# rlog58/dags-vae-search

Measured on AMD Instinct MI355X. Metric: DAGs/sec VAE+predictor train step, n=12 batch 4096 per GPU, at 1 MI355X, higher is better.
Workload: dtype f32 (fwd bf16x6, bwd bf16x3 split products, fp32 accumulate); 1 GPU; synthetic_v12 DAGs (n=12, card=12, N=15 tokens), PACE-VAE train step: pack + fwd + bwd + clip_grad_norm_(1.0) + Adam(1e-4), train mode dropout 0.15; per_gpu_batch=4096, global_batch=4096, waves_per_workgroup=8, parallelism=single

## Files before the change

### dags_vae_search_amd/_lib.py

```python
from __future__ import annotations

import ctypes
import os
from ctypes import (POINTER, Structure, c_char, c_char_p, c_float, c_int, c_int32, c_int64, c_size_t, c_uint32,
                    c_uint64, c_void_p)

_HERE = os.path.dirname(os.path.abspath(__file__))
LIB_NAME = "libdvs_hip.so"

D_MODEL, HEADS, LAYERS, LATENT, FC_HIDDEN, EMB = 64, 8, 3, 32, 32, 32
MAX_TOKENS = 48
TILE_TOKENS = 16
DECODE_STATE_BYTES = 440
CLIP_SCRATCH_FLOATS = 4096
RECORD_BYTES = 96
LOSS_FLOATS = 5
ABI_VERSION = 202
GP_ACQ_MAX_INDUCING = 1023
STRUCT_HASH_INVALID = 0x7FFFFFFFFFFFFFFF
GEN_LABELS_CHOICE, GEN_ACCEPT_ISOLATES, GEN_ACCEPT_NO_CONNECTIVITY, GEN_GROUP_SHIFT = 1, 2, 4, 8
SCORE_TYPES = {"loglik": 0, "aic": 1, "bic": 2, "bde": 3, "bds": 4, "k2": 5, "bdj": 6}


class DvsShape(Structure):
    _fields_ = [("batch", c_int32), ("n_tokens", c_int32), ("n_classes", c_int32), ("training", c_int32),
                ("dropout", c_float), ("beta", c_float), ("eps_scale", c_float), ("dag_offset", c_uint32),
                ("seed", c_uint64)]


class DvsParamEntry(Structure):
    _fields_ = [("name", c_char * 64), ("offset", c_int64), ("rows", c_int32), ("cols", c_int32)]


def bind(lib: ctypes.CDLL) -> ctypes.CDLL:
    P = POINTER
    lib.dvs_version.restype = c_int
    lib.dvs_last_error.restype = c_char_p
    lib.dvs_device_cus.restype = c_int
    lib.dvs_param_count.restype = c_int64
    lib.dvs_param_count.argtypes = [P(DvsShape)]
    lib.dvs_param_table.restype = c_int
    lib.dvs_param_table.argtypes = [P(DvsShape), P(DvsParamEntry), c_int]
    lib.dvs_workspace_bytes.restype = c_size_t
    lib.dvs_workspace_bytes.argtypes = [P(DvsShape)]
    lib.dvs_record_bytes.restype = c_size_t
    lib.dvs_record_bytes.argtypes = [P(DvsShape)]
    lib.dvs_pack_features.restype = c_int
    lib.dvs_pack_features.argtypes = [P(DvsShape), c_void_p, c_void_p, c_void_p, c_void_p, c_void_p, c_size_t, c_void_p,
                                      c_void_p]
    lib.dvs_build_records.restype = c_int
    lib.dvs_build_records.argtypes = [P(DvsShape), c_void_p, c_void_p, c_void_p, c_size_t, c_void_p, c_void_p]
    lib.dvs_loss_forward.restype = c_int
    lib.dvs_loss_forward.argtypes = [P(DvsShape), c_void_p, c_size_t, c_void_p, c_int64, c_void_p, c_size_t, c_void_p,
                                     c_void_p, c_void_p, c_void_p, c_void_p, c_void_p]
    lib.dvs_loss_forward_notify.restype = c_int
    lib.dvs_loss_forward_notify.argtypes = [P(DvsShape), c_void_p, c_size_t, c_void_p, c_int64, c_void_p, c_size_t, c_void_p,
                                            c_void_p, c_void_p, c_void_p, c_void_p, c_void_p, ctypes.c_uint32, c_void_p]
    lib.dvs_loss_backward.restype = c_int
    lib.dvs_loss_backward.argtypes = [P(DvsShape), c_void_p, c_size_t, c_void_p, c_int64, c_void_p, c_size_t, c_void_p,
                                      c_void_p, c_void_p]
    lib.dvs_loss_backward_sq.restype = c_int
    lib.dvs_loss_backward_sq.argtypes = [P(DvsShape), c_void_p, c_size_t, c_void_p, c_int64, c_void_p, c_size_t, c_void_p,
                                         c_void_p, c_void_p, c_void_p]
    lib.dvs_encode.restype = c_int
    lib.dvs_encode.argtypes = [P(DvsShape), c_void_p, c_size_t, c_void_p, c_int64, c_void_p, c_size_t, c_void_p, c_void_p,
                               c_void_p]
    lib.dvs_decode.restype = c_int
    lib.dvs_decode.argtypes = [P(DvsShape), c_void_p, c_int64, c_void_p, c_size_t, c_void_p, c_size_t, c_void_p, c_void_p,
                               c_void_p, c_size_t, c_void_p]
    lib.dvs_match_decoded.restype = c_int
    lib.dvs_match_decoded.argtypes = [c_int32, c_int32, c_int32, c_int32, c_int32, c_void_p, c_void_p, c_void_p, c_size_t,
                                      c_int32, c_void_p, c_void_p]
    lib.dvs_decoded_structures.restype = c_int
    lib.dvs_decoded_structures.argtypes = [c_int32, c_int32, c_int32, c_void_p, c_size_t, c_uint64, c_void_p, c_void_p,
                                           c_void_p, c_void_p, c_size_t, c_void_p, c_void_p]
    lib.dvs_structset_filter.restype = c_int
    lib.dvs_structset_filter.argtypes = [c_int32, c_int32, c_void_p, c_void_p, c_void_p, c_size_t, c_void_p, c_int32,
                                         c_void_p, c_void_p, c_size_t, c_void_p, c_void_p]
    lib.dvs_generate_dags.restype = c_int
    lib.dvs_generate_dags.argtypes = [c_int32, c_int32, c_int32, c_int32, c_void_p, c_uint64, c_int64, c_int32, c_int32,
                                      c_void_p, c_void_p, c_size_t, c_void_p, c_void_p]
    lib.dvs_generate_edge_counts.restype = c_int
    lib.dvs_generate_edge_counts.argtypes = [c_int32, c_int32, c_void_p, c_void_p, c_uint64, c_int64, c_void_p, c_void_p]
    lib.dvs_debug_launch.restype = c_int
    lib.dvs_debug_launch.argtypes = [c_size_t, c_void_p]
    lib.dvs_bic_scores.restype = c_int
    lib.dvs_bic_scores.argtypes = [c_int32, c_int32, c_int32, c_void_p, c_void_p, c_void_p, c_void_p, c_void_p, c_void_p,
                                   c_void_p]
    lib.dvs_bn_scores.restype = c_int
    lib.dvs_bn_scores.argtypes = [c_int32, c_int32, c_int32, c_void_p, c_void_p, c_void_p, c_int32, ctypes.c_double, c_void_p,
                                  c_void_p, c_void_p, c_void_p]
    lib.dvs_bic_parent_masks.restype = c_int
    lib.dvs_bic_parent_masks.argtypes = [c_int32, c_int32, c_int32, c_void_p, c_void_p, c_void_p, c_void_p, c_void_p]
    lib.dvs_gp_predict.restype = c_int
    lib.dvs_gp_predict.argtypes = [c_int32, c_int32, c_int32, c_void_p, c_void_p, c_void_p, ctypes.c_double, ctypes.c_double,
                                   ctypes.c_double, c_void_p, c_void_p]
    lib.dvs_gp_kernel.restype = c_int
    lib.dvs_gp_kernel.argtypes = [c_int32, c_int32, c_int32, c_void_p, c_void_p, ctypes.c_double, ctypes.c_double, c_void_p,
                                  c_void_p]
    lib.dvs_gp_kernel_backward.restype = c_int
    lib.dvs_gp_kernel_backward.argtypes = [c_int32, c_int32, c_int32, c_int32, c_void_p, c_void_p, ctypes.c_double,
                                           ctypes.c_double, c_void_p, c_void_p, c_void_p, c_void_p]
    lib.dvs_gp_acquire.restype = c_int
    lib.dvs_gp_acquire.argtypes = [c_int32, c_int32, c_int32, c_int32, c_void_p, c_void_p, c_void_p] + [ctypes.c_double] * 6 + \
        [c_void_p, c_void_p, c_void_p, c_void_p, c_void_p]
    lib.dvs_clip_adam.restype = c_int
    lib.dvs_clip_adam.argtypes = [c_int64, c_void_p, c_void_p, c_void_p, c_void_p, c_float, c_float, c_float, c_float,
                                  c_int64, c_float, c_void_p, c_void_p, c_void_p]
    lib.dvs_clip_adam_from_partials.restype = c_int
    lib.dvs_clip_adam_from_partials.argtypes = lib.dvs_clip_adam.argtypes
    lib.dvs_profile_enable.restype = None
    lib.dvs_profile_enable.argtypes = [c_int]
    lib.dvs_profile_collect.restype = c_int
    lib.dvs_profile_collect.argtypes = [c_void_p, c_int, c_void_p, c_void_p, c_int]
    lib.dvs_debug_activation.restype = c_int
    lib.dvs_debug_activation.argtypes = [P(DvsShape), c_void_p, c_int, c_void_p, c_void_p]
    return lib


EXPORTS = ["dvs_version", "dvs_last_error", "dvs_device_cus", "dvs_param_count", "dvs_param_table",
           "dvs_workspace_bytes", "dvs_record_bytes", "dvs_pack_features", "dvs_build_records", "dvs_loss_forward", "dvs_loss_forward_notify", "dvs_loss_backward", "dvs_loss_backward_sq", "dvs_encode", "dvs_decode", "dvs_match_decoded", "dvs_decoded_structures", "dvs_structset_filter", "dvs_generate_dags", "dvs_generate_edge_counts", "dvs_bic_scores", "dvs_bn_scores", "dvs_bic_parent_masks", "dvs_gp_predict", "dvs_gp_kernel", "dvs_gp_kernel_backward", "dvs_gp_acquire",
           "dvs_clip_adam", "dvs_clip_adam_from_partials", "dvs_debug_activation", "dvs_debug_launch", "dvs_profile_enable", "dvs_profile_collect"]


def profile_collect(lib):
    cap, stride = 64, 64
    names = ctypes.create_string_buffer(cap * stride)
    counts = (c_int * cap)()
    ms = (c_float * cap)()
    n = lib.dvs_profile_collect(names, stride, counts, ms, cap)
    out = {}
    for i in range(min(n, cap)):
        out[names.raw[i * stride:(i + 1) * stride].split(b"\0")[0].decode()] = (int(counts[i]), float(ms[i]))
    return out

_lib = None


def lib_path() -> str:
    return os.path.join(_HERE, LIB_NAME)


def load() -> ctypes.CDLL:
    global _lib
    if _lib is None:
        path = lib_path()
        if not os.path.exists(path):
            raise RuntimeError(
                f"{LIB_NAME} not found at {path}: build it with `python -c 'import __graft_entry__ as g; g.build()'` "
                f"(hipcc --offload-arch=gfx950).  dags_vae_search_amd has no CPU fallback.")
        _lib = bind(ctypes.CDLL(path))
        if _lib.dvs_version() != ABI_VERSION:
            raise RuntimeError(f"{LIB_NAME}: unexpected ABI version {_lib.dvs_version()}")
    return _lib


def check(lib, code: int, what: str):
    if code != 0:
        msg = lib.dvs_last_error()
        raise RuntimeError(f"{what} failed with code {code}: {msg.decode() if msg else ''}")


def make_shape(batch: int, n_tokens: int, n_classes: int, training: bool = False, dropout: float = 0.15,
               beta: float = 0.005, eps_scale: float = 0.01, dag_offset: int = 0, seed: int = 0) -> DvsShape:
    return DvsShape(int(batch), int(n_tokens), int(n_classes), 1 if training else 0, float(dropout), float(beta),
                    float(eps_scale), int(dag_offset) & 0xFFFFFFFF, int(seed) & 0xFFFFFFFFFFFFFFFF)


def record_bytes(lib, shape: DvsShape) -> int:
    n = int(lib.dvs_record_bytes(ctypes.byref(shape)))
    if n == 0:
        check(lib, 1, "dvs_record_bytes")
    return n


def is_wide(n_tokens: int, n_classes: int) -> bool:
    return n_tokens > TILE_TOKENS or n_classes > 16


def param_table(lib, shape: DvsShape):
    entries = (DvsParamEntry * 128)()
    n = lib.dvs_param_table(ctypes.byref(shape), entries, 128)
    if n <= 0:
        check(lib, 1, "dvs_param_table")
    table = []
    for e in entries[:n]:
        shp = (e.rows, e.cols) if e.cols else (e.rows,)
        table.append((e.name.decode(), int(e.offset), shp))
    total = int(lib.dvs_param_count(ctypes.byref(shape)))
    return table, total
```

### dags_vae_search_amd/csrc/dvs_api.hip

```cpp
#include <math.h>
#include <stdarg.h>
#include <stdio.h>
#include <stdlib.h>
#include <string.h>

#include "dvs_kernels.h"
#include "dvs_backward.h"
#include "dvs_wide.h"
#include "dvs_wimg.h"
#include "dvs_decode.h"

static thread_local char g_err[256] = "";

#include <map>
#include <mutex>
#include <string>
#include <utility>
#include <vector>
namespace {
struct ProfRec {
    const char* name;
#ifndef DVS_EMU
    hipEvent_t a, b;
#endif
};
std::mutex g_prof_mu;
bool g_prof_on = false;
std::vector<ProfRec> g_prof;
thread_local int t_prof_slot = -1;
}

void dvs_prof_begin(const char* name, dvs_stream_t st) {
    t_prof_slot = -1;
    std::lock_guard<std::mutex> lock(g_prof_mu);
    if (!g_prof_on) return;
    ProfRec r;
    r.name = name;
#ifndef DVS_EMU
    if (hipEventCreate(&r.a) != hipSuccess) return;
    if (hipEventCreate(&r.b) != hipSuccess) {
        (void)hipEventDestroy(r.a);
        return;
    }
    (void)hipEventRecord(r.a, st);
#endif
    t_prof_slot = (int)g_prof.size();
    g_prof.push_back(r);
}
void dvs_prof_end(dvs_stream_t st) {
    if (t_prof_slot < 0) return;
    std::lock_guard<std::mutex> lock(g_prof_mu);
#ifndef DVS_EMU
    if (t_prof_slot < (int)g_prof.size()) (void)hipEventRecord(g_prof[t_prof_slot].b, st);
#endif
    t_prof_slot = -1;
}
extern "C" void dvs_profile_enable(int on) {
    std::lock_guard<std::mutex> lock(g_prof_mu);
    g_prof_on = on != 0;
}
extern "C" int dvs_profile_collect(char* names, int name_stride, int* counts, float* total_ms, int cap) {
    std::map<std::string, std::pair<int, float>> agg;
    std::lock_guard<std::mutex> lock(g_prof_mu);
    for (auto& r : g_prof) {
        float ms = 0.f;
#ifndef DVS_EMU
        (void)hipEventSynchronize(r.b);
        (void)hipEventElapsedTime(&ms, r.a, r.b);
        (void)hipEventDestroy(r.a);
        (void)hipEventDestroy(r.b);
#endif
        auto& e = agg[r.name];
        e.first += 1;
        e.second += ms;
    }
    g_prof.clear();
    int i = 0;
    for (auto& kv : agg) {
        if (i >= cap) break;
        snprintf(names + (size_t)i * name_stride, name_stride, "%s", kv.first.c_str());
        counts[i] = kv.second.first;
        total_ms[i] = kv.second.second;
        ++i;
    }
    return (int)agg.size();
}

static int fail(int code, const char* msg) {
    snprintf(g_err, sizeof(g_err), "%s", msg);
    return code;
}

static thread_local int t_hip_err = 0;
static thread_local char t_hip_msg[200] = "";
void dvs_note_hip_error(const char* what, int hip_error, const char* hip_message) {
    if (t_hip_err != 0) return;
    t_hip_err = hip_error ? hip_error : -1;
    snprintf(t_hip_msg, sizeof(t_hip_msg), "%s: HIP error %d (%s)", what, hip_error, hip_message ? hip_message : "?");
}
static void call_begin() {
    t_hip_err = 0;
    (void)hipGetLastError();
}
static int call_end(const char* fn) {
    if (t_hip_err == 0) return 0;
    snprintf(g_err, sizeof(g_err), "%s: %s", fn, t_hip_msg);
    t_hip_err = 0;
    return 20;
}
#define DVS_HIP_CALL(expr)                                                             \
    do {                                                                               \
        const hipError_t dvs_ce_ = (expr);                                             \
        if (dvs_ce_ != hipSuccess) dvs_note_hip_error(#expr, (int)dvs_ce_, hipGetErrorString(dvs_ce_)); \
    } while (0)
static void copy_out(void* dst, const void* src, size_t bytes, dvs_stream_t st) {
#ifdef DVS_EMU
    DVS_HIP_CALL(hipMemcpyAsyncD2D(dst, src, bytes, st));
#else
    DVS_HIP_CALL(hipMemcpyAsync(dst, src, bytes, hipMemcpyDeviceToDevice, st));
#endif
}

extern "C" int dvs_version(void) { return DVS_VERSION; }
extern "C" const char* dvs_last_error(void) { return g_err; }

extern "C" int dvs_device_cus(void) {
#ifdef DVS_EMU
    return 2;
#else
    int dev = 0, cus = 0;
    if (hipGetDevice(&dev) != hipSuccess) return 0;
    if (hipDeviceGetAttribute(&cus, hipDeviceAttributeMultiprocessorCount, dev) != hipSuccess) return 0;
    return cus;
#endif
}

namespace {
struct LayoutBuilder {
    int64_t off = 0;
    dvs_param_entry* table;
    int cap, count = 0;
    int64_t add(int rows, int cols, const char* fmt, ...) {
        const int64_t o = off;
        if (table && count < cap) {
            dvs_param_entry& e = table[count];
            memset(&e, 0, sizeof(e));
            va_list ap;
            va_start(ap, fmt);
            vsnprintf(e.name, sizeof(e.name), fmt, ap);
            va_end(ap);
            e.offset = o;
            e.rows = rows;
            e.cols = cols;
        }
        ++count;
        const int64_t n = (int64_t)rows * (cols ? cols : 1);
        off += (n + 3) & ~(int64_t)3;
        return o;
    }
};
}

DvsLayout dvs_make_layout(int N, int C, dvs_param_entry* table, int cap, int* count) {
    LayoutBuilder b;
    b.table = table;
    b.cap = cap;
    DvsLayout l;
    auto attn = [&](const char* stack, int i, const char* which, DvsAttnP& p) {
        p.in_w = b.add(192, 64, "%s.layers.%d.%s.in_proj_weight", stack, i, which);
        p.in_b = b.add(192, 0, "%s.layers.%d.%s.in_proj_bias", stack, i, which);
        p.out_w = b.add(64, 64, "%s.layers.%d.%s.out_proj.weight", stack, i, which);
        p.out_b = b.add(64, 0, "%s.layers.%d.%s.out_proj.bias", stack, i, which);
    };
    auto ffn = [&](const char* stack, int i, DvsFfnP& p) {
        p.l1_w = b.add(64, 64, "%s.layers.%d.linear1.weight", stack, i);
        p.l1_b = b.add(64, 0, "%s.layers.%d.linear1.bias", stack, i);
        p.l2_w = b.add(64, 64, "%s.layers.%d.linear2.weight", stack, i);
        p.l2_b = b.add(64, 0, "%s.layers.%d.linear2.bias", stack, i);
    };
    auto norm = [&](const char* stack, int i, int k, DvsNormP& p) {
        p.w = b.add(64, 0, "%s.layers.%d.norm%d.weight", stack, i, k);
        p.b = b.add(64, 0, "%s.layers.%d.norm%d.bias", stack, i, k);
    };
    l.W1 = b.add(2 * N, 64, "vertex_position_embed.W1");
    l.W2 = b.add(64, 32, "vertex_position_embed.W2");
    l.lab_w = b.add(32, C, "vertex_label_embed.0.weight");
    l.lab_b = b.add(32, 0, "vertex_label_embed.0.bias");
    for (int i = 0; i < DVS_LAYERS; ++i) {
        attn("encoder", i, "self_attn", l.enc[i].sa);
        ffn("encoder", i, l.enc[i].ff);
        norm("encoder", i, 1, l.enc[i].n1);
        norm("encoder", i, 2, l.enc[i].n2);
    }
    l.fc1_w = b.add(32, N * 64, "fc1.weight");
    l.fc1_b = b.add(32, 0, "fc1.bias");
    l.fc2_w = b.add(32, N * 64, "fc2.weight");
    l.fc2_b = b.add(32, 0, "fc2.bias");
    for (int i = 0; i < DVS_LAYERS; ++i) {
        attn("decoder", i, "self_attn", l.dec[i].sa);
        attn("decoder", i, "multihead_attn", l.dec[i].ca);
        ffn("decoder", i, l.dec[i].ff);
        norm("decoder", i, 1, l.dec[i].n1);
        norm("decoder", i, 2, l.dec[i].n2);
        norm("decoder", i, 3, l.dec[i].n3);
    }
    l.node0_w = b.add(32, 64, "add_node.0.weight");
    l.node0_b = b.add(32, 0, "add_node.0.bias");
    l.node2_w = b.add(C, 32, "add_node.2.weight");
    l.node2_b = b.add(C, 0, "add_node.2.bias");
    l.edge0_w = b.add(64, 128, "add_edge.0.weight");
    l.edge0_b = b.add(64, 0, "add_edge.0.bias");
    l.edge2_w = b.add(1, 64, "add_edge.2.weight");
    l.edge2_b = b.add(1, 0, "add_edge.2.bias");
    l.fc3_w = b.add(N * 64, 32, "fc3.weight");
    l.fc3_b = b.add(N * 64, 0, "fc3.bias");
    l.total = b.off;
    if (count) *count = b.count;
    return l;
}

DvsWorkspace dvs_make_workspace(int B, int NT, int64_t P, int nslab, bool wide) {
    DvsWorkspace w;
    size_t off = 0;
    auto take = [&](size_t n) {
        const size_t o = off;
        off += (n + 63) & ~(size_t)63;
        return o;
    };
    const size_t tile = (size_t)B * NT * 1024;
    for (int s = 0; s < DVS_NSLOTS; ++s) {
        w.act[s] = take(tile);
        w.stats[s] = take((size_t)B * NT * 32);
    }
    w.enc_out = take(tile);
    w.mu = take((size_t)B * 32);
    w.logvar = take((size_t)B * 32);
    w.z = take((size_t)B * 32);
    w.epsv = take((size_t)B * 32);
    w.mem = take(tile);
    w.dag_loss = take((size_t)B * 2);
    w.gA = take(tile);
    w.gB = take(tile);
    w.gq = take(tile);
    w.gk = take(tile);
    w.gv = take(tile);
    w.gmem = take(tile);
    w.genc = take(tile);
    w.gz = take((size_t)B * 64);
    w.nslab = nslab;
    w.slabs = take((size_t)nslab * (size_t)P);
    w.fcpart = take((size_t)DVS_FC_PARTS * (size_t)P);
    w.wimg = take((DVS_WIMG_BF16 + 1) / 2);
    w.limg = take(DvsLatImg::floats(NT));
    for (int blk = 0; blk < 9; ++blk) w.qkv[blk] = take(wide ? (size_t)B * NT * 12 * 256 : 0);
    w.total_floats = off;
    return w;
}

static int check_shape(const dvs_shape* s) {
    if (!s) return fail(1, "dvs: null shape");
    if (s->batch <= 0) return fail(2, "dvs: batch must be > 0");
    if (s->n_tokens < 4 || s->n_tokens > DVS_WTOK)
        return fail(3, "dvs: n_tokens (= max_num_vertices + 3) must be in [4, 48] in this build");
    if (s->n_classes < 4 || s->n_classes > DVS_WTOK)
        return fail(4, "dvs: n_classes (= vertex_label_cardinality + 3) must be in [4, 48] in this build");
    if (!(s->dropout >= 0.f && s->dropout < 1.f)) return fail(5, "dvs: dropout must be in [0, 1)");
    return 0;
}

static bool is_wide(const dvs_shape* s) { return s->n_tokens > DVS_MAXTOK || s->n_classes > 16; }
static int tiles_of(const dvs_shape* s) { return (s->n_tokens + 15) / 16; }
static size_t record_size(bool wide) { return wide ? sizeof(DvsRecordW) : sizeof(DvsRecord); }

static DvsDims make_dims(const dvs_shape* s) {
    DvsDims d;
    d.NT = tiles_of(s);
    d.B = s->batch;
    d.N = s->n_tokens;
    d.C = s->n_classes;
    d.training = s->training ? 1 : 0;
    d.drop.thr16 = (uint32_t)lrintf(s->dropout * 65536.0f);
    d.drop.on = (d.training && d.drop.thr16 > 0) ? 1 : 0;
    d.drop.scale = 1.0f / (1.0f - (float)d.drop.thr16 / 65536.0f);
    d.seed_lo = (uint32_t)(s->seed & 0xFFFFFFFFull);
    d.seed_hi = (uint32_t)(s->seed >> 32);
    d.dag_offset = s->dag_offset;
    d.beta = s->beta;
    d.eps_scale = s->eps_scale;
    d.debug = 0;
    return d;
}

static int num_slabs() {
    const int cus = dvs_device_cus();
    return cus > 0 ? cus : 256;
}
static int grid_for(int units, int per_wg, int cap) {
    const int want = (units + per_wg - 1) / per_wg;
    return want < cap ? want : cap;
}

static int waves_per_wg(const DvsDims& d, bool wide, int nslab) {
    const char* env = getenv("DVS_WAVES_PER_WG");
    const int force = env ? atoi(env) : 0;
    if (wide) return 8;
    if (force == 4 || force == 8) return force;
    return d.B <= 4 * nslab ? 4 : 8;
}
static int active_slabs(const DvsDims& d, bool wide, int nslab) {
    if (wide) return nslab;
    const int want = (d.B + 3) / 4;
    return want < nslab ? want : nslab;
}

static bool env_on(const char* name) {
    const char* v = getenv(name);
    return v && atoi(v) != 0;
}
static bool split_stack() {
    static const bool on = env_on("DVS_SPLIT_STACK");
    return on;
}
static bool latent_kernels_off() {
    static const bool on = env_on("DVS_LATENT_KERNELS");
    return on;
}
static bool latent_in_chain(bool chain, int nw) { return chain && !latent_kernels_off() && nw == 8; }

struct FwdGrids {
    int chain;
    int tiles16;
    int tiles8;
    int tiles4;
    int dags;
    int dags2;
    int dec4;
};

struct Step {
    DvsDims d;
    DvsLayout L;
    DvsWorkspace W;
    bool wide;
    const float* P;
    float* ws;
    const DvsRecord* rec;
    dvs_stream_t st;
    int nw;
    FwdGrids g;
    int slabs;
};
static Step make_step(const dvs_shape* s, const void* records, const float* params, void* workspace, void* stream) {
    Step c;
    c.d = make_dims(s);
    c.L = dvs_make_layout(c.d.N, c.d.C, nullptr, 0, nullptr);
    c.wide = is_wide(s);
    const int nslab = num_slabs();
    c.W = dvs_make_workspace(c.d.B, c.d.NT, c.L.total, nslab, c.wide);
    c.P = params;
    c.ws = (float*)workspace;
    c.rec = (const DvsRecord*)records;
    c.st = (dvs_stream_t)stream;
    c.nw = waves_per_wg(c.d, c.wide, nslab);
    const int tiles = c.d.B * c.d.NT;
    c.g.chain = grid_for(tiles, c.nw, nslab);
    c.g.tiles16 = grid_for(tiles, 16, nslab);
    c.g.tiles8 = grid_for(tiles, 8, nslab);
    c.g.tiles4 = grid_for(tiles, 4, nslab);
    c.g.dags = grid_for(c.d.B, 1, nslab);
    c.g.dags2 = c.d.B < 2 * c.g.dags ? c.d.B : 2 * c.g.dags;
    c.g.dec4 = grid_for(c.d.B, 4, nslab);
    c.slabs = active_slabs(c.d, c.wide, nslab);
    return c;
}

static int check_records(const char* fn, size_t records_bytes, int batch, bool wide) {
    const size_t need = (size_t)batch * record_size(wide);
    if (records_bytes >= need) return 0;
    char msg[240];
    snprintf(msg, sizeof(msg), "%s: records_bytes %zu < batch * dvs_record_bytes = %zu", fn, records_bytes, need);
    return fail(14, msg);
}
static int check_buffers(const Step& c, const char* fn, size_t records_bytes, int64_t n_params, size_t workspace_bytes) {
    if (int e = check_records(fn, records_bytes, c.d.B, c.wide)) return e;
    char msg[240];
    if (n_params < c.L.total) {
        snprintf(msg, sizeof(msg), "%s: n_params %lld < dvs_param_count = %lld", fn, (long long)n_params, (long long)c.L.total);
        return fail(14, msg);
    }
    const size_t need = c.W.total_floats * sizeof(float);
    if (workspace_bytes < need) {
        snprintf(msg, sizeof(msg), "%s: workspace_bytes %zu < dvs_workspace_bytes = %zu", fn, workspace_bytes, need);
        return fail(14, msg);
    }
    return 0;
}

extern "C" int64_t dvs_param_count(const dvs_shape* s) {
    if (check_shape(s)) return -1;
    return dvs_make_layout(s->n_tokens, s->n_classes, nullptr, 0, nullptr).total;
}

extern "C" int dvs_param_table(const dvs_shape* s, dvs_param_entry* out, int cap) {
    if (check_shape(s)) return -1;
    int count = 0;
    dvs_make_layout(s->n_tokens, s->n_classes, out, cap, &count);
    return count;
}

extern "C" size_t dvs_workspace_bytes(const dvs_shape* s) {
    if (check_shape(s)) return 0;
    return make_step(s, nullptr, nullptr, nullptr, nullptr).W.total_floats * sizeof(float);
}

extern "C" size_t dvs_record_bytes(const dvs_shape* s) {
    if (check_shape(s)) return 0;
    return record_size(is_wide(s));
}

extern "C" int dvs_pack_features(const dvs_shape* s, const float* label_onehot, const float* pos_onehot,
                                 const float* adjacency, const uint8_t* target_masks, void* records, size_t records_bytes,
                                 int32_t* status, void* stream) {
    if (int e = check_shape(s)) return e;
    if (!label_onehot || !pos_onehot || !adjacency || !target_masks || !records || !status)
        return fail(10, "dvs_pack_features: null pointer");
    if (int e = check_records("dvs_pack_features", records_bytes, s->batch, is_wide(s))) return e;
    call_begin();
    PackArgs a;
    a.B = s->batch;
    a.N = s->n_tokens;
    a.C = s->n_classes;
    a.lab1h = label_onehot;
    a.pos1h = pos_onehot;
    a.adj = adjacency;
    a.tmask = target_masks;
    a.rec = (DvsRecord*)records;
    a.status = status;
    if (is_wide(s)) dvs_launch_pack_w(a, (dvs_stream_t)stream);
    else dvs_launch_pack(a, (dvs_stream_t)stream);
    return call_end("dvs_pack_features");
}

extern "C" int dvs_build_records(const dvs_shape* s, const uint8_t* labels, const void* preds, void* records,
                                 size_t records_bytes, int32_t* status, void* stream) {
    if (int e = check_shape(s)) return e;
    if (!labels || !preds || !records || !status) return fail(10, "dvs_build_records: null pointer");
    if (int e = check_records("dvs_build_records", records_bytes, s->batch, is_wide(s))) return e;
    call_begin();
    if (is_wide(s)) {
        BuildWArgs a;
        a.B = s->batch;
        a.N = s->n_tokens;
        a.C = s->n_classes;
        a.labels = labels;
        a.preds = (const uint64_t*)preds;
        a.rec = (DvsRecordW*)records;
        a.status = status;
        dvs_launch_build_records_w(a, (dvs_stream_t)stream);
        return call_end("dvs_build_records");
    }
    BuildArgs a;
    a.B = s->batch;
    a.N = s->n_tokens;
    a.C = s->n_classes;
    a.labels = labels;
    a.preds = (const uint16_t*)preds;
    a.rec = (DvsRecord*)records;
    a.status = status;
    dvs_launch_build_records(a, (dvs_stream_t)stream);
    return call_end("dvs_build_records");
}

static inline int slot_enc(int layer, int sub) { return 1 + 2 * layer + sub; }
static inline int slot_dec(int layer, int sub) { return 8 + 3 * layer + sub; }
static inline int site_enc(int layer, int k) { return 4 + 4 * layer + k; }
static inline int site_dec(int layer, int k) { return 16 + 6 * layer + k; }

static inline size_t img_attn(int block) { return (size_t)block * DvsAttnImg::SIZE; }
static inline size_t img_ffn(int block) { return DVS_N_ATTN_BLOCKS * DvsAttnImg::SIZE + (size_t)block * DvsFfnImg::SIZE; }
static inline int blk_enc_attn(int layer) { return layer; }
static inline int blk_dec_self(int layer) { return 3 + 2 * layer; }
static inline int blk_dec_cross(int layer) { return 4 + 2 * layer; }
static inline int blk_enc_ffn(int layer) { return layer; }
static inline int blk_dec_ffn(int layer) { return 3 + layer; }

static inline const void* wimg_attn(const Step& c, int block) { return (const dvs_bf16*)(c.ws + c.W.wimg) + img_attn(block); }
static inline const void* wimg_ffn(const Step& c, int block) { return (const dvs_bf16*)(c.ws + c.W.wimg) + img_ffn(block); }

static DvsLN ln_of(const Step& c, int slot, const DvsNormP* n) {
    if (!n) return DvsLN{nullptr, nullptr, nullptr};
    return DvsLN{c.ws + c.W.stats[slot], c.P + n->w, c.P + n->b};
}

static EmbedArgs embed_args(const Step& c, int site) {
    EmbedArgs e;
    memset(&e, 0, sizeof(e));
    e.dims = c.d;
    e.rec = c.rec;
    e.W1 = c.P + c.L.W1;
    e.W2 = c.P + c.L.W2;
    e.lab_w = c.P + c.L.lab_w;
    e.lab_b = c.P + c.L.lab_b;
    e.embimg = (const float*)((const dvs_bf16*)(c.ws + c.W.wimg) + DVS_WIMG_EMB);
    e.site = site;
    return e;
}

static AttnArgs attn_args(const Step& c, const DvsAttnP& p, int block, int in, const DvsNormP* norm, const float* kv, int out,
                          int site0) {
    AttnArgs a;
    memset(&a, 0, sizeof(a));
    a.dims = c.d;
    a.rec = c.rec;
    a.xin = c.ws + c.W.act[in];
    a.ln = ln_of(c, in, norm);
    a.kv = kv;
    a.in_w = c.P + p.in_w;
    a.in_b = c.P + p.in_b;
    a.out_w = c.P + p.out_w;
    a.out_b = c.P + p.out_b;
    a.wimg = wimg_attn(c, block);
    a.qkv = c.wide ? c.ws + c.W.qkv[block] : nullptr;
    a.out_pre = c.ws + c.W.act[out];
    a.out_stats = c.ws + c.W.stats[out];
    a.site_prob = site0;
    a.site_post = site0 + 1;
    return a;
}

static FfnArgs ffn_args(const Step& c, const DvsFfnP& p, int block, int in, const DvsNormP& norm, int out, int site0) {
    FfnArgs f;
    memset(&f, 0, sizeof(f));
    f.dims = c.d;
    f.xin = c.ws + c.W.act[in];
    f.ln = ln_of(c, in, &norm);
    f.l1_w = c.P + p.l1_w;
    f.l1_b = c.P + p.l1_b;
    f.l2_w = c.P + p.l2_w;
    f.l2_b = c.P + p.l2_b;
    f.wimg = wimg_ffn(c, block);
    f.out_pre = c.ws + c.W.act[out];
    f.out_stats = c.ws + c.W.stats[out];
    f.site_hidden = site0;
    f.site_post = site0 + 1;
    return f;
}

static LatentArgs latent_args(const Step& c, const float* eps, bool with_mem) {
    LatentArgs a;
    memset(&a, 0, sizeof(a));
    a.dims = c.d;
    a.xenc = c.ws + c.W.enc_out;
    a.fc1_w = c.P + c.L.fc1_w;
    a.fc1_b = c.P + c.L.fc1_b;
    a.fc2_w = c.P + c.L.fc2_w;
    a.fc2_b = c.P + c.L.fc2_b;
    a.fc3_w = c.P + c.L.fc3_w;
    a.fc3_b = c.P + c.L.fc3_b;
    a.limg = c.ws + c.W.limg;
    a.eps_in = eps;
    a.mu = c.ws + c.W.mu;
    a.logvar = c.ws + c.W.logvar;
    a.z = c.ws + c.W.z;
    a.epsv = c.ws + c.W.epsv;
    a.mem = with_mem ? c.ws + c.W.mem : nullptr;
    a.dag_loss = c.ws + c.W.dag_loss;
    return a;
}

template <class A>
static void head_params(const Step& c, A& a) {
    a.node0_w = c.P + c.L.node0_w;
    a.node0_b = c.P + c.L.node0_b;
    a.node2_w = c.P + c.L.node2_w;
    a.node2_b = c.P + c.L.node2_b;
    a.edge0_b = c.P + c.L.edge0_b;
    a.edge2_w = c.P + c.L.edge2_w;
    a.edge2_b = c.P + c.L.edge2_b;
}
template <class A>
static void head_input(const Step& c, A& a) {
    const int last = slot_dec(DVS_LAYERS - 1, 2);
    a.xin = c.ws + c.W.act[last];
    a.ln = ln_of(c, last, &c.L.dec[DVS_LAYERS - 1].n3);
    a.edge0_w = c.P + c.L.edge0_w;
    head_params(c, a);
}

static LossArgs loss_args(const Step& c) {
    LossArgs a;
    memset(&a, 0, sizeof(a));
    a.dims = c.d;
    a.rec = c.rec;
    head_input(c, a);
    a.wimg = (const dvs_bf16*)(c.ws + c.W.wimg) + DVS_WIMG_LOSS;
    a.dag_loss = c.ws + c.W.dag_loss;
    return a;
}

static void prepare_images(const Step& c) {
    const DvsLayout& L = c.L;
    const bool wide = c.wide;
    DvsImgJobs J;
    J.count = 0;
    auto add = [&](int64_t src, size_t dst, int rows, int flags) {
        DvsImgJob& j = J.job[J.count++];
        j.src = src;
        j.dst = (int64_t)dst;
        j.rows = rows;
        j.flags = flags;
    };
    auto attn = [&](const DvsAttnP& p, int block) {
        const size_t b = img_attn(block);
        add(p.in_w, b + DvsAttnImg::Win, 192, wide ? 0 : 2);
        add(p.out_w, b + DvsAttnImg::Wout, 64, wide ? 0 : 4);
        add(p.out_w, b + DvsAttnImg::WoutT, 64, 1 | (wide ? 0 : 4));
        add(p.in_w, b + DvsAttnImg::WinB, 192, 16 | (wide ? 0 : 2));
        for (int q = 0; q < 3; ++q)
            add(p.in_w + 4096 * q, b + DvsAttnImg::WinT + (size_t)q * 2 * DVS_IMG64, 64, 1 | (wide ? 0 : 2));
    };
    auto ffn = [&](const DvsFfnP& p, int block) {
        const size_t b = img_ffn(block);
        add(p.l1_w, b + DvsFfnImg::W1, 64, 0);
        add(p.l2_w, b + DvsFfnImg::W2, 64, 0);
        add(p.l2_w, b + DvsFfnImg::W2T, 64, 1);
        add(p.l1_w, b + DvsFfnImg::W1T, 64, 1);
    };
    for (int i = 0; i < DVS_LAYERS; ++i) {
        attn(L.enc[i].sa, blk_enc_attn(i));
        ffn(L.enc[i].ff, blk_enc_ffn(i));
        attn(L.dec[i].sa, blk_dec_self(i));
        attn(L.dec[i].ca, blk_dec_cross(i));
        ffn(L.dec[i].ff, blk_dec_ffn(i));
    }
    if (!wide) {
        add(L.edge0_w, DVS_WIMG_LOSS + DvsLossImg::Wa, 64, 8);
        add(L.edge0_w + 64, DVS_WIMG_LOSS + DvsLossImg::Wb, 64, 8);
        add(L.edge0_w, DVS_WIMG_LOSS + DvsLossImg::WaT, 64, 8 | 1);
        add(L.edge0_w + 64, DVS_WIMG_LOSS + DvsLossImg::WbT, 64, 8 | 1);
    }
    dvs_bf16* wimg = (dvs_bf16*)(c.ws + c.W.wimg);
    DvsLatImgArgs lat;
    lat.fc1_w = c.P + L.fc1_w;
    lat.fc2_w = c.P + L.fc2_w;
    lat.fc3_w = c.P + L.fc3_w;
    lat.fc3_b = c.P + L.fc3_b;
    lat.img = c.ws + c.W.limg;
    lat.N = c.d.N;
    lat.NT = c.d.NT;
    DvsLossHeadArgs head;
    memset(&head, 0, sizeof(head));
    if (!wide) {
        head_params(c, head);
        head.ln_g = c.P + L.dec[DVS_LAYERS - 1].n3.w;
        head.ln_b = c.P + L.dec[DVS_LAYERS - 1].n3.b;
        head.dst = (float*)(wimg + DVS_WIMG_LOSS + DvsLossImg::Head);
        head.C = c.d.C;
        head.W1 = c.P + L.W1;
        head.W2 = c.P + L.W2;
        head.lab_w = c.P + L.lab_w;
        head.lab_b = c.P + L.lab_b;
        head.dst_emb = (float*)(wimg + DVS_WIMG_EMB);
        head.N = c.d.N;
    }
    dvs_launch_prepare_images(J, c.P, wimg, lat, head, c.st);
}

static void launch_embed_fwd(const Step& c, const EmbedArgs& e) {
    if (c.wide) dvs_launch_embed_fwd_w(e, c.g.tiles4, c.st);
    else if (c.nw == 4) dvs_launch_embed_fwd(e, c.g.chain, 4, c.st);
    else dvs_launch_embed_fwd(e, c.g.tiles16, 16, c.st);
}
static void launch_attn_fwd(const Step& c, const AttnArgs& a) {
    if (c.wide) dvs_launch_attn_fwd_w(a, c.g.dags, c.st);
    else if (c.nw == 4) dvs_launch_attn_fwd(a, c.g.chain, 4, c.st);
    else dvs_launch_attn_fwd(a, c.g.tiles8, 8, c.st);
}
static void launch_ffn_fwd(const Step& c, const FfnArgs& f) {
    if (c.nw == 4) dvs_launch_ffn_fwd(f, c.g.chain, 4, c.st);
    else dvs_launch_ffn_fwd(f, c.g.tiles16, 16, c.st);
}
static void launch_loss_fwd(const Step& c, const LossArgs& a) {
    if (c.wide) dvs_launch_loss_fwd_w(a, c.g.dags2, c.st);
    else if (c.nw == 4) dvs_launch_loss_fwd(a, c.g.chain, 4, c.st);
    else dvs_launch_loss_fwd(a, c.g.tiles8, 8, c.st);
}
struct FwdChain {
    FwdStackArgs stack;
    const Step& c;
    int tag;
    bool chain;
    FwdChain(const Step& step, int tag_) : c(step), tag(tag_), chain(!step.wide && !split_stack()) { memset(&stack, 0, sizeof(stack)); }
    FwdPhase& next(int kind) {
        if (stack.nphase == DVS_FWD_STACK_PHASES) flush();
        FwdPhase& ph = stack.ph[stack.nphase++];
        ph.kind = kind;
        return ph;
    }
    void attn(const AttnArgs& a) {
        if (chain) next(DVS_FPH_ATTN).u.a = a;
        else launch_attn_fwd(c, a);
    }
    void ffn(const FfnArgs& f) {
        if (chain) next(DVS_FPH_FFN).u.f = f;
        else launch_ffn_fwd(c, f);
    }
    bool latent(const LatentArgs& l) {
        if (!latent_in_chain(chain, c.nw) || stack.nphase == 0 || stack.nphase == DVS_FWD_STACK_PHASES) return false;
        next(DVS_FPH_LATENT).u.l = l;
        return true;
    }
    void flush() {
        if (stack.nphase > 0) dvs_launch_fwd_stack(stack, tag, c.g.chain, c.nw, c.st);
        stack.nphase = 0;
    }
};

static void encoder_forward(const Step& c, const LatentArgs& lat, bool dec_embed = false, bool save_qkv = false) {
    EmbedArgs e = embed_args(c, 0);
    e.out = c.ws + c.W.act[0];
    if (dec_embed) {
        e.out2 = c.ws + c.W.act[7];
        e.site2 = 2;
    }
    launch_embed_fwd(c, e);
    FwdChain chain(c, 0);
    const DvsNormP* norm = nullptr;
    int prev = 0;
    for (int i = 0; i < DVS_LAYERS; ++i) {
        const auto& pl = c.L.enc[i];
        const int sa = slot_enc(i, 0), sf = slot_enc(i, 1);
        AttnArgs a = attn_args(c, pl.sa, blk_enc_attn(i), prev, norm, nullptr, sa, site_enc(i, 0));
        if (!save_qkv) a.qkv = nullptr;
        chain.attn(a);
        FfnArgs f = ffn_args(c, pl.ff, blk_enc_ffn(i), sa, pl.n1, sf, site_enc(i, 2));
        if (i == DVS_LAYERS - 1) {
            f.out_norm = c.ws + c.W.enc_out;
            f.ng = c.P + pl.n2.w;
            f.nb = c.P + pl.n2.b;
        }
        chain.ffn(f);
        norm = &pl.n2;
        prev = sf;
    }
    const bool fused = chain.latent(lat);
    chain.flush();
    if (!fused) dvs_launch_latent_fwd(lat, c.st);
}

static void decoder_forward(const Step& c, int dec_in) {
    FwdChain chain(c, 1);
    const DvsNormP* norm = nullptr;
    int prev = dec_in;
    for (int i = 0; i < DVS_LAYERS; ++i) {
        const auto& pl = c.L.dec[i];
        const int s0 = slot_dec(i, 0), s1 = slot_dec(i, 1), s2 = slot_dec(i, 2);
        chain.attn(attn_args(c, pl.sa, blk_dec_self(i), prev, norm, nullptr, s0, site_dec(i, 0)));
        chain.attn(attn_args(c, pl.ca, blk_dec_cross(i), s0, &pl.n1, c.ws + c.W.mem, s1, site_dec(i, 2)));
        chain.ffn(ffn_args(c, pl.ff, blk_dec_ffn(i), s1, pl.n2, s2, site_dec(i, 4)));
        norm = &pl.n3;
        prev = s2;
    }
    chain.flush();
}

extern "C" int dvs_loss_forward(const dvs_shape* s, const void* records, size_t records_bytes, const float* params,
                                int64_t n_params, void* workspace, size_t workspace_bytes, const float* eps,
                                const int32_t* status, float* losses, float* mu, float* logvar, void* stream) {
    return dvs_loss_forward_notify(s, records, records_bytes, params, n_params, workspace, workspace_bytes, eps,
                                   (int32_t*)status, losses, mu, logvar, nullptr, 0u, stream);
}

extern "C" int dvs_loss_forward_notify(const dvs_shape* s, const void* records, size_t records_bytes, const float* params,
                                       int64_t n_params, void* workspace, size_t workspace_bytes, const float* eps,
                                       int32_t* status, float* losses, float* mu, float* logvar, void* host_tail,
                                       uint32_t host_seq, void* stream) {
    if (int e = check_shape(s)) return e;
    if (!records || !params || !workspace || !losses) return fail(10, "dvs_loss_forward: null pointer");
    const Step c = make_step(s, records, params, workspace, stream);
    if (int e = check_buffers(c, "dvs_loss_forward", records_bytes, n_params, workspace_bytes)) return e;
    call_begin();
    prepare_images(c);
    encoder_forward(c, latent_args(c, eps, true), c.d.drop.on, true);
    decoder_forward(c, c.d.drop.on ? 7 : 0);
    launch_loss_fwd(c, loss_args(c));
    FinalizeArgs fa;
    fa.B = c.d.B;
    fa.beta = c.d.beta;
    fa.dag_loss = c.ws + c.W.dag_loss;
    fa.status = status;
    fa.losses = losses;
    fa.host_tail = (float*)host_tail;
    fa.host_seq = host_seq;
    dvs_launch_finalize(fa, c.st);
    const size_t nb = (size_t)c.d.B * 32 * sizeof(float);
    if (mu) copy_out(mu, c.ws + c.W.mu, nb, c.st);
    if (logvar) copy_out(logvar, c.ws + c.W.logvar, nb, c.st);
    return call_end("dvs_loss_forward");
}

extern "C" int dvs_encode(const dvs_shape* s, const void* records, size_t records_bytes, const float* params,
                          int64_t n_params, void* workspace, size_t workspace_bytes, float* mu, float* logvar,
                          void* stream) {
    if (int e = check_shape(s)) return e;
    if (!records || !params || !workspace || !mu || !logvar) return fail(10, "dvs_encode: null pointer");
    const Step c = make_step(s, records, params, workspace, stream);
    if (int e = check_buffers(c, "dvs_encode", records_bytes, n_params, workspace_bytes)) return e;
    call_begin();
    prepare_images(c);
    LatentArgs la = latent_args(c, nullptr, false);
    la.dims.training = 0;
    encoder_forward(c, la);
    const size_t nb = (size_t)c.d.B * 32 * sizeof(float);
    copy_out(mu, c.ws + c.W.mu, nb, c.st);
    copy_out(logvar, c.ws + c.W.logvar, nb, c.st);
    return call_end("dvs_encode");
}

extern "C" int dvs_decode(const dvs_shape* s, const float* params, int64_t n_params, void* workspace,
                          size_t workspace_bytes, void* records, size_t records_bytes, const float* z,
                          const float* uniforms, void* state_out, size_t state_bytes, void* stream) {
    if (int e = check_shape(s)) return e;
    if (!params || !workspace || !records || !z || !state_out) return fail(10, "dvs_decode: null pointer");
    if (s->training) return fail(13, "dvs_decode: generation runs in eval mode (shape.training must be 0)");
    const Step c = make_step(s, records, params, workspace, stream);
    if (int e = check_buffers(c, "dvs_decode", records_bytes, n_params, workspace_bytes)) return e;
    if (state_bytes < (size_t)s->batch * sizeof(dvs_decode_state))
        return fail(14, "dvs_decode: state_bytes < batch * sizeof(dvs_decode_state)");
    call_begin();
    prepare_images(c);
    dvs_launch_decode_memory(c.d, z, c.P + c.L.fc3_w, c.P + c.L.fc3_b, c.ws + c.W.mem, c.st);
    DecodeArgs a;
    memset(&a, 0, sizeof(a));
    a.dims = c.d;
    a.wide = c.wide ? 1 : 0;
    a.rec = records;
    a.state = (DvsDecodeState*)state_out;
    head_input(c, a);
    a.uniforms = uniforms;
    dvs_launch_decode_init(a, c.st);
    EmbedArgs e = embed_args(c, 2);
    e.out = c.ws + c.W.act[7];
    for (int idx = 2; idx < c.d.N; ++idx) {
        launch_embed_fwd(c, e);
        decoder_forward(c, 7);
        a.idx = idx;
        dvs_launch_decode_step(a, c.g.dec4, c.st);
    }
    return call_end("dvs_decode");
}

extern "C" int dvs_match_decoded_impl(int B, int n, int card, int R, int wide, const uint8_t* labels, const void* preds,
                                      const void* states, int budget, uint8_t* flags, void* stream);
extern "C" int dvs_match_decoded(int32_t batch, int32_t n_vars, int32_t card, int32_t repeats, int32_t preds_are_u64,
                                 const uint8_t* labels, const void* preds, const void* states, size_t state_bytes,
                                 int32_t budget, uint8_t* flags, void* stream) {
    if (batch <= 0 || repeats <= 0) return fail(2, "dvs_match_decoded: batch and repeats must be > 0");
    if ((int64_t)batch * repeats > (int64_t)1 << 30) return fail(2, "dvs_match_decoded: batch * repeats must be <= 2^30");
    if (n_vars < 1 || n_vars > 45) return fail(3, "dvs_match_decoded: n_vars must be in [1, 45]");
    if (card < 1 || card > 45) return fail(3, "dvs_match_decoded: card must be in [1, 45]");
    if (!preds_are_u64 && n_vars > 16) return fail(12, "dvs_match_decoded: 16-bit predecessor rows hold at most 16 vertices");
    if (budget < 1) return fail(12, "dvs_match_decoded: budget must be >= 1");
    if (!labels || !preds || !states || !flags) return fail(10, "dvs_match_decoded: null pointer");
    const size_t need = (size_t)batch * repeats * sizeof(dvs_decode_state);
    if (state_bytes < need) {
        char msg[160];
        snprintf(msg, sizeof(msg), "dvs_match_decoded: state_bytes < batch * repeats * DVS_DECODE_STATE_BYTES = %zu", need);
        return fail(14, msg);
    }
    call_begin();
    if (int e = dvs_match_decoded_impl(batch, n_vars, card, repeats, preds_are_u64 ? 1 : 0, labels, preds, states, budget,
                                       flags, stream))
        return e;
    return call_end("dvs_match_decoded");
}

extern "C" int dvs_decoded_structures_impl(int B, int n, int wide, const void* states, uint64_t hash_mask, uint8_t* flags,
                                           uint8_t* labels, void* preds, uint64_t* keys, uint64_t* hashes, void* stream);
extern "C" int dvs_structset_filter_impl(int B, int n, const uint64_t* sorted_hashes, const int64_t* order,
                                         const uint64_t* keys, const uint8_t* flags, int S, const uint64_t* seen_hashes,
                                         const uint64_t* seen_keys, uint8_t* out, void* stream);
static int fail_size(const char* what, size_t need) {
    char msg[200];
    snprintf(msg, sizeof(msg), "%s = %zu", what, need);
    return fail(14, msg);
}
extern "C" int dvs_decoded_structures(int32_t batch, int32_t n_vars, int32_t preds_are_u64, const void* states,
                                      size_t state_bytes, uint64_t hash_mask, uint8_t* flags, uint8_t* labels, void* preds,
                                      uint64_t* keys, size_t keys_bytes, uint64_t* hashes, void* stream) {
    if (batch <= 0) return fail(2, "dvs_decoded_structures: batch must be > 0");
    if (batch > 1 << 30) return fail(2, "dvs_decoded_structures: batch must be <= 2^30");
    if (n_vars < 1 || n_vars > 45) return fail(3, "dvs_decoded_structures: n_vars must be in [1, 45]");
    if (!preds_are_u64 && n_vars > 16) return fail(12, "dvs_decoded_structures: 16-bit predecessor rows hold at most 16 vertices");
    if (!states || !flags || !labels || !preds || !keys || !hashes) return fail(10, "dvs_decoded_structures: null pointer");
    if (state_bytes < (size_t)batch * sizeof(dvs_decode_state))
        return fail_size("dvs_decoded_structures: state_bytes < batch * DVS_DECODE_STATE_BYTES", (size_t)batch * sizeof(dvs_decode_state));
    if (keys_bytes < (size_t)batch * n_vars * 8)
        return fail_size("dvs_decoded_structures: keys_bytes < batch * n_vars * 8", (size_t)batch * n_vars * 8);
    call_begin();
    if (int e = dvs_decoded_structures_impl(batch, n_vars, preds_are_u64 ? 1 : 0, states, hash_mask, flags, labels, preds, keys,
                                            hashes, stream))
        return e;
    return call_end("dvs_decoded_structures");
}

extern "C" int dvs_structset_filter(int32_t batch, int32_t n_vars, const uint64_t* sorted_hashes, const int64_t* order,
                                    const uint64_t* keys, size_t keys_bytes, const uint8_t* flags, int32_t seen_count,
                                    const uint64_t* seen_hashes, const uint64_t* seen_keys, size_t seen_keys_bytes,
                                    uint8_t* out, void* stream) {
    if (batch < 0 || seen_count < 0) return fail(2, "dvs_structset_filter: batch and seen_count must be >= 0");
    if (batch > 1 << 30) return fail(2, "dvs_structset_filter: batch must be <= 2^30");
    if (n_vars < 1 || n_vars > 45) return fail(3, "dvs_structset_filter: n_vars must be in [1, 45]");
    if (batch == 0) return 0;
    if (!sorted_hashes || !order || !keys || !flags || !out) return fail(10, "dvs_structset_filter: null pointer");
    if (seen_count > 0 && (!seen_hashes || !seen_keys)) return fail(10, "dvs_structset_filter: null pointer (seen set)");
    if (keys_bytes < (size_t)batch * n_vars * 8)
        return fail_size("dvs_structset_filter: keys_bytes < batch * n_vars * 8", (size_t)batch * n_vars * 8);
    if (seen_keys_bytes < (size_t)seen_count * n_vars * 8)
        return fail_size("dvs_structset_filter: seen_keys_bytes < seen_count * n_vars * 8", (size_t)seen_count * n_vars * 8);
    call_begin();
    if (int e = dvs_structset_filter_impl(batch, n_vars, sorted_hashes, order, keys, flags, seen_count, seen_hashes, seen_keys,
                                          out, stream))
        return e;
    return call_end("dvs_structset_filter");
}

extern "C" int dvs_generate_dags_impl(int B, int n, int card, int wide, const int* num_edges, uint64_t seed, uint32_t dag_offset,
                                      int try_limit, int flags, int gshift, uint8_t* labels, void* preds, int* attempts,
                                      void* stream);
extern "C" int dvs_generate_dags(int32_t batch, int32_t n_vars, int32_t card, int32_t preds_are_u64, const int32_t* num_edges,
                                 uint64_t seed, int64_t dag_offset, int32_t try_limit, int32_t flags, uint8_t* labels,
                                 void* preds, size_t preds_bytes, int32_t* attempts, void* stream) {
    if (batch <= 0) return fail(2, "dvs_generate_dags: batch must be > 0");
    if (batch > 1 << 30) return fail(2, "dvs_generate_dags: batch must be <= 2^30");
    if (n_vars < 2 || n_vars > 45) return fail(3, "dvs_generate_dags: n_vars must be in [2, 45]");
    if (card < 1 || card > 45) return fail(3, "dvs_generate_dags: card must be in [1, 45]");
    const int group = (flags >> DVS_GEN_GROUP_SHIFT) & 15;
    if ((flags & ~(7 | 15 << DVS_GEN_GROUP_SHIFT)) || group > 7) return fail(12, "dvs_generate_dags: unknown bits in flags");
    if (!(flags & DVS_GEN_LABELS_CHOICE) && card < n_vars)
        return fail(12, "dvs_generate_dags: labels without replacement ('sample') need card >= n_vars");
    if ((preds_are_u64 != 0) != (n_vars > 13))
        return fail(12, "dvs_generate_dags: predecessor rows are u16 for n_vars <= 13 and u64 above (preds_are_u64 does not match)");
    if (try_limit < 1 || try_limit > 4096) return fail(12, "dvs_generate_dags: try_limit must be in [1, 4096]");
    if (dag_offset < 0) return fail(12, "dvs_generate_dags: dag_offset must be >= 0");
    if (!num_edges || !labels || !preds || !attempts) return fail(10, "dvs_generate_dags: null pointer");
    const size_t need = (size_t)batch * n_vars * (preds_are_u64 ? 8 : 2);
    if (preds_bytes < need) return fail_size("dvs_generate_dags: preds_bytes < batch * n_vars * row bytes", need);
    int gshift = 0;
    if (group) {
        gshift = group - 1;
    } else if (!(flags & DVS_GEN_ACCEPT_NO_CONNECTIVITY)) {
        static const int cus = dvs_device_cus();
        const int64_t lanes = (int64_t)cus * 4 * 64 * 16;
        while (gshift < 6 && ((int64_t)batch << (gshift + 1)) <= lanes && (1 << gshift) < try_limit) ++gshift;
    }
    call_begin();
    if (int e = dvs_generate_dags_impl(batch, n_vars, card, preds_are_u64 ? 1 : 0, num_edges, seed, (uint32_t)dag_offset, try_limit,
                                       flags & 7, gshift, labels, preds, attempts, stream))
        return e;
    return call_end("dvs_generate_dags");
}

extern "C" int dvs_generate_edge_counts_impl(int B, int K, const int* counts, const int* cum, uint64_t seed, uint32_t dag_offset,
                                             int* out, void* stream);
extern "C" int dvs_generate_edge_counts(int32_t batch, int32_t n_entries, const int32_t* edge_counts, const int32_t* cum_weights,
                                        uint64_t seed, int64_t dag_offset, int32_t* num_edges, void* stream) {
    if (batch <= 0 || batch > 1 << 30) return fail(2, "dvs_generate_edge_counts: batch must be in [1, 2^30]");
    if (n_entries < 1 || n_entries > 1024) return fail(12, "dvs_generate_edge_counts: n_entries must be in [1, 1024]");
    if (dag_offset < 0) return fail(12, "dvs_generate_edge_counts: dag_offset must be >= 0");
    if (!edge_counts || !cum_weights || !num_edges) return fail(10, "dvs_generate_edge_counts: null pointer");
    call_begin();
    if (int e = dvs_generate_edge_counts_impl(batch, n_entries, edge_counts, cum_weights, seed, (uint32_t)dag_offset, num_edges,
                                              stream))
        return e;
    return call_end("dvs_generate_edge_counts");
}

extern "C" int dvs_bic_scores_impl(int B, int n, int S, const uint64_t* data, const uint8_t* card, const uint64_t* parents,
                                   double* local, double* out, int* status, void* stream);
extern "C" int dvs_bic_scores(int32_t batch, int32_t n_vars, int32_t n_samples, const uint64_t* data, const uint8_t* card,
                              const uint64_t* parents, double* scratch, double* out, int32_t* status, void* stream) {
    if (batch <= 0 || n_samples <= 0) return fail(2, "dvs_bic_scores: batch and n_samples must be > 0");
    if (n_vars < 1 || n_vars > DVS_WTOK) return fail(3, "dvs_bic_scores: n_vars must be in [1, 48]");
    if (!data || !card || !parents || !scratch || !out || !status) return fail(10, "dvs_bic_scores: null pointer");
    call_begin();
    if (int e = dvs_bic_scores_impl(batch, n_vars, n_samples, data, card, parents, scratch, out, status, stream)) return e;
    return call_end("dvs_bic_scores");
}

extern "C" int dvs_bn_scores_impl(int B, int n, int S, const uint64_t* data, const uint8_t* card, const uint64_t* parents,
                                  int type, double arg, double* local, double* out, int* status, void* stream);
extern "C" int dvs_bn_scores(int32_t batch, int32_t n_vars, int32_t n_samples, const uint64_t* data, const uint8_t* card,
                             const uint64_t* parents, int32_t score_type, double score_arg, double* scratch, double* out,
                             int32_t* status, void* stream) {
    if (batch <= 0 || n_samples <= 0) return fail(2, "dvs_bn_scores: batch and n_samples must be > 0");
    if (n_vars < 1 || n_vars > DVS_WTOK) return fail(3, "dvs_bn_scores: n_vars must be in [1, 48]");
    if (!data || !card || !parents || !scratch || !out || !status) return fail(10, "dvs_bn_scores: null pointer");
    const bool dflt = score_arg != score_arg;
    double arg = score_arg;
    switch (score_type) {
        case DVS_SCORE_LOGLIK:
        case DVS_SCORE_K2:
        case DVS_SCORE_BDJ:
            if (!dflt) return fail(13, "dvs_bn_scores: loglik, k2 and bdj take no argument (score_arg must be NaN)");
            arg = 0.0;
            break;
        case DVS_SCORE_AIC:
        case DVS_SCORE_BIC:
            if (!dflt && !(score_arg >= 0.0 && isfinite(score_arg))) return fail(13, "dvs_bn_scores: k must be finite and >= 0");
            if (dflt && score_type == DVS_SCORE_AIC) arg = 1.0;
            break;
        case DVS_SCORE_BDE:
        case DVS_SCORE_BDS:
            if (!dflt && !(score_arg > 0.0 && isfinite(score_arg))) return fail(13, "dvs_bn_scores: iss must be finite and > 0");
            if (dflt) arg = 1.0;
            break;
        default:
            return fail(12, "dvs_bn_scores: score_type is not a dvs_score_type");
    }
    call_begin();
    if (int e = dvs_bn_scores_impl(batch, n_vars, n_samples, data, card, parents, score_type, arg, scratch, out, status, stream))
        return e;
    return call_end("dvs_bn_scores");
}

extern "C" int dvs_bic_parent_masks_impl(int B, int n, int wide, const uint8_t* labels, const void* preds, uint64_t* parents,
                                         int* status, void* stream);
extern "C" int dvs_bic_parent_masks(int32_t batch, int32_t n_vars, int32_t preds_are_u64, const uint8_t* labels,
                                    const void* preds, uint64_t* parents, int32_t* status, void* stream) {
    if (batch <= 0) return fail(2, "dvs_bic_parent_masks: batch must be > 0");
    if (n_vars < 1 || n_vars > DVS_WTOK) return fail(3, "dvs_bic_parent_masks: n_vars must be in [1, 48]");
    if (!preds_are_u64 && n_vars > 16) return fail(12, "dvs_bic_parent_masks: 16-bit predecessor rows hold at most 16 vertices");
    if (!labels || !preds || !parents || !status) return fail(10, "dvs_bic_parent_masks: null pointer");
    call_begin();
    if (int e = dvs_bic_parent_masks_impl(batch, n_vars, preds_are_u64 ? 1 : 0, labels, preds, parents, status, stream)) return e;
    return call_end("dvs_bic_parent_masks");
}

extern "C" int dvs_gp_predict_impl(int B, int M, int D, const float* x, const float* z, const double* alpha,
                                   double outputscale, double lengthscale, double constant, double* out, void* stream);
extern "C" int dvs_gp_predict(int32_t batch, int32_t n_inducing, int32_t dim, const float* x, const float* inducing,
                              const double* alpha, double outputscale, double lengthscale, double constant, double* out,
                              void* stream) {
    if (batch <= 0 || n_inducing <= 0 || dim <= 0) return fail(2, "dvs_gp_predict: sizes must be > 0");
    if (!(lengthscale > 0.0)) return fail(5, "dvs_gp_predict: lengthscale must be > 0");
    if (!x || !inducing || !alpha || !out) return fail(10, "dvs_gp_predict: null pointer");
    call_begin();
    if (int e = dvs_gp_predict_impl(batch, n_inducing, dim, x, inducing, alpha, outputscale, lengthscale, constant, out, stream)) return e;
    return call_end("dvs_gp_predict");
}

extern "C" int dvs_gp_kernel_impl(int na, int nb, int D, const float* xa, const float* xb, double outputscale, double lengthscale,
                                  double* K, void* stream);
extern "C" int dvs_gp_kernel_backward_impl(int na, int nb, int D, int symmetric, const float* xa, const float* xb,
                                           double outputscale, double lengthscale, const double* G, double* dxa, double* rows,
                                           void* stream);
static int gp_check(const char* fn, int na, int nb, int dim, double outputscale, double lengthscale) {
    char msg[160];
    if (na <= 0 || nb <= 0 || dim <= 0 || dim > 32) {
        snprintf(msg, sizeof(msg), "%s: sizes must be > 0 and dim <= 32", fn);
        return fail(2, msg);
    }
    if (!(lengthscale > 0.0) || !(outputscale > 0.0)) {
        snprintf(msg, sizeof(msg), "%s: lengthscale and outputscale must be > 0", fn);
        return fail(5, msg);
    }
    return 0;
}
extern "C" int dvs_gp_kernel(int32_t na, int32_t nb, int32_t dim, const float* xa, const float* xb, double outputscale,
                             double lengthscale, double* K, void* stream) {
    if (int e = gp_check("dvs_gp_kernel", na, nb, dim, outputscale, lengthscale)) return e;
    if (!xa || !xb || !K) return fail(10, "dvs_gp_kernel: null pointer");
    call_begin();
    if (int e = dvs_gp_kernel_impl(na, nb, dim, xa, xb, outputscale, lengthscale, K, stream)) return e;
    return call_end("dvs_gp_kernel");
}
extern "C" int dvs_gp_kernel_backward(int32_t na, int32_t nb, int32_t dim, int32_t symmetric, const float* xa, const float* xb,
                                      double outputscale, double lengthscale, const double* G, double* dxa, double* row_sums,
                                      void* stream) {
    if (int e = gp_check("dvs_gp_kernel_backward", na, nb, dim, outputscale, lengthscale)) return e;
    if (!xa || !xb || !G || !dxa || !row_sums) return fail(10, "dvs_gp_kernel_backward: null pointer");
    if (symmetric && na != nb) return fail(12, "dvs_gp_kernel_backward: symmetric needs na == nb");
    call_begin();
    if (int e = dvs_gp_kernel_backward_impl(na, nb, dim, symmetric, xa, xb, outputscale, lengthscale, G, dxa, row_sums, stream))
        return e;
    return call_end("dvs_gp_kernel_backward");
}

extern "C" int dvs_gp_acquire_impl(int Q, int M, int D, int ld, const float* x, const float* z, const double* W, double c0,
                                   double outputscale, double lengthscale, double constant, double best, double xi,
                                   double* mean, double* var, double* ei, float* grad, void* stream) __attribute__((weak));
extern "C" int dvs_gp_acquire(int32_t batch, int32_t n_inducing, int32_t dim, int32_t ld, const float* x, const float* inducing,
                              const double* weights, double c0, double outputscale, double lengthscale, double constant,
                              double best, double xi, double* mean, double* var, double* ei, float* grad, void* stream) {
    if (int e = gp_check("dvs_gp_acquire", batch, n_inducing, dim, outputscale, lengthscale)) return e;
    if (n_inducing > DVS_GP_ACQ_MAX_INDUCING) return fail(2, "dvs_gp_acquire: n_inducing must be <= 1023");
    if (ld < n_inducing + 1) return fail(12, "dvs_gp_acquire: ld must be >= n_inducing + 1 (P | alpha)");
    if (!(c0 >= 0.0)) return fail(12, "dvs_gp_acquire: c0 must be >= 0");
    if (!x || !inducing || !weights || !mean || !var || !ei) return fail(10, "dvs_gp_acquire: null pointer");
    if (!dvs_gp_acquire_impl) return fail(20, "dvs_gp_acquire: k_gp_acq.hip is not part of this build");
    call_begin();
    if (int e = dvs_gp_acquire_impl(batch, n_inducing, dim, ld, x, inducing, weights, c0, outputscale, lengthscale, constant,
                                    best, xi, mean, var, ei, grad, stream))
        return e;
    return call_end("dvs_gp_acquire");
}

extern "C" int dvs_debug_activation(const dvs_shape* s, const void* workspace, int slot, float* out, void* stream) {
    if (int e = check_shape(s)) return e;
    const Step c = make_step(s, nullptr, nullptr, (void*)workspace, stream);
    const float* ws = c.ws;
    const DvsWorkspace& W = c.W;
    const float* src = nullptr;
    if (slot >= 0 && slot < DVS_NSLOTS) src = ws + W.act[slot];
    else if (slot == 100) src = ws + W.enc_out;
    else if (slot == 101) src = ws + W.mem;
    else if (slot == 102) src = ws + W.gA;
    else if (slot == 103) src = ws + W.gB;
    else if (slot == 104) src = ws + W.gmem;
    else if (slot == 105) src = ws + W.genc;
    else return fail(11, "dvs_debug_activation: bad slot");
    call_begin();
    dvs_launch_unfrag(src, out, c.d.B * c.d.NT, c.st);
    return call_end("dvs_debug_activation");
}

__global__ void k_debug_empty(int* sink) {
    DVS_DYN_LDS(smem);
    if (sink && threadIdx.x == 1u << 20) *sink = smem[0];
}
extern "C" int dvs_debug_launch(size_t dynamic_lds_bytes, void* stream) {
    call_begin();
    DVS_LAUNCH(k_debug_empty, dim3(1), dim3(64), dynamic_lds_bytes, (dvs_stream_t)stream, (int*)nullptr);
    return call_end("dvs_debug_launch");
}

#include "dvs_api_backward.inc"
```

### dags_vae_search_amd/csrc/dvs_wimg.h

```cpp
#pragma once
#include "dvs_bf16.h"

constexpr size_t DVS_IMG64 = 64 * (size_t)DVS_LDB;
struct DvsAttnImg {
    static constexpr size_t Win = 0;
    static constexpr size_t Wout = 3 * 3 * DVS_IMG64;
    static constexpr size_t WoutT = Wout + 3 * DVS_IMG64;
    static constexpr size_t WinB = WoutT + 2 * DVS_IMG64;
    static constexpr size_t WinT = WinB + 2 * 3 * DVS_IMG64;
    static constexpr size_t SIZE = WinT + 3 * 2 * DVS_IMG64;
};
struct DvsFfnImg {
    static constexpr size_t W2T = 0;
    static constexpr size_t W1T = 2 * DVS_IMG64;
    static constexpr size_t W1 = 4 * DVS_IMG64;
    static constexpr size_t W2 = 7 * DVS_IMG64;
    static constexpr size_t SIZE = 10 * DVS_IMG64;
};
struct DvsLossImg {
    static constexpr size_t Wa = 0;
    static constexpr size_t Wb = 3 * DVS_IMG64;
    static constexpr size_t WaT = 6 * DVS_IMG64;
    static constexpr size_t WbT = 8 * DVS_IMG64;
    static constexpr size_t Head = 10 * DVS_IMG64;
    static constexpr int HEAD_FLOATS = 32 * 68 + 16 * 36 + 32 + 16 + 64 + 64 + 16 + 64 + 64;
    static constexpr size_t SIZE = Head + 2 * (size_t)HEAD_FLOATS;
};
static_assert(DvsLossImg::HEAD_FLOATS % 256 == 0 && DVS_LD == 68, "whole 1 KB chunks (dvs_stage.h)");
struct DvsEmbImg {
    static constexpr int FLOATS = 5120;
};
struct DvsLossHeadArgs {
    const float *node0_w, *node0_b, *node2_w, *node2_b, *edge0_b, *edge2_w, *edge2_b, *ln_g, *ln_b;
    float* dst;
    int C;
    const float *W1, *W2, *lab_w, *lab_b;
    float* dst_emb;
    int N;
};
constexpr int DVS_N_ATTN_BLOCKS = 9, DVS_N_FFN_BLOCKS = 6;
constexpr size_t DVS_WIMG_LOSS = DVS_N_ATTN_BLOCKS * DvsAttnImg::SIZE + DVS_N_FFN_BLOCKS * DvsFfnImg::SIZE;
constexpr size_t DVS_WIMG_EMB = DVS_WIMG_LOSS + DvsLossImg::SIZE;
constexpr size_t DVS_WIMG_BF16 = DVS_WIMG_EMB + 2 * (size_t)DvsEmbImg::FLOATS;

struct DvsLatImg {
    static constexpr size_t LD(int NT) { return (size_t)1024 * NT + 64; }
    static constexpr size_t A(int) { return 0; }
    static constexpr size_t AT(int NT) { return 64 * LD(NT); }
    static constexpr size_t W3(int NT) { return AT(NT) + (size_t)64 * 1024 * NT; }
    static constexpr size_t W3T(int NT) { return W3(NT) + (size_t)32 * 1024 * NT; }
    static constexpr size_t B3(int NT) { return W3T(NT) + 32 * LD(NT); }
    static constexpr size_t floats(int NT) { return B3(NT) + (size_t)1024 * NT; }
};
struct DvsLatImgArgs {
    const float *fc1_w, *fc2_w, *fc3_w, *fc3_b;
    float* img;
    int N, NT;
};

struct DvsImgJob {
    int64_t src;
    int64_t dst;
    int32_t rows;
    int32_t flags;
};
constexpr int DVS_MAX_IMG_JOBS = 96;
struct DvsImgJobs {
    DvsImgJob job[DVS_MAX_IMG_JOBS];
    int count;
};
void dvs_launch_prepare_images(const DvsImgJobs& jobs, const float* params, dvs_bf16* wimg, const DvsLatImgArgs& lat,
                               const DvsLossHeadArgs& head, dvs_stream_t st);

__device__ __forceinline__ void dvs_copy_image(dvs_bf16* dst, const dvs_bf16* __restrict__ src, int n) {
    const f4* s = (const f4*)src;
    f4* d = (f4*)dst;
    const int n16 = n >> 3, step = blockDim.x;
    const int rot = (int)(((unsigned)dvs_bid() * 2654435761u) % (unsigned)n16);
    int i = dvs_tid();
    for (; i + 7 * step < n16; i += 8 * step) {
        f4 v[8];
        int j[8];
#pragma unroll
        for (int u = 0; u < 8; ++u) {
            j[u] = i + u * step + rot;
            j[u] = j[u] >= n16 ? j[u] - n16 : j[u];
            v[u] = s[j[u]];
        }
#pragma unroll
        for (int u = 0; u < 8; ++u) d[j[u]] = v[u];
    }
    if (i < n16) {
        f4 v[7];
        int j[7];
#pragma unroll
        for (int u = 0; u < 7; ++u) {
            const int k = i + u * step;
            j[u] = k + rot;
            j[u] = j[u] >= n16 ? j[u] - n16 : j[u];
            if (k < n16) v[u] = s[j[u]];
        }
#pragma unroll
        for (int u = 0; u < 7; ++u)
            if (i + u * step < n16) d[j[u]] = v[u];
    }
}
```

### dags_vae_search_amd/csrc/k_forward.hip

```cpp
#include "dvs_kernels.h"
#include "dvs_wimg.h"

constexpr int PACK_DAGS = 4;
__device__ __forceinline__ void pack_stream(float* dst, const float* __restrict__ src, size_t nfloats) {
    const size_t n4 = nfloats >> 2;
    size_t i = threadIdx.x;
    for (; i + 3 * blockDim.x < n4; i += 4 * blockDim.x) {
        f4 v[4];
#pragma unroll
        for (int u = 0; u < 4; ++u) v[u] = *(const f4*)(src + 4 * (i + u * blockDim.x));
#pragma unroll
        for (int u = 0; u < 4; ++u) *(f4*)(dst + 4 * (i + u * blockDim.x)) = v[u];
    }
    for (; i < n4; i += blockDim.x) *(f4*)(dst + 4 * i) = *(const f4*)(src + 4 * i);
    for (size_t i = 4 * n4 + threadIdx.x; i < nfloats; i += blockDim.x) dst[i] = src[i];
}
__global__ __launch_bounds__(8 * 16 * PACK_DAGS) void k_pack(PackArgs a) {
    DVS_DYN_LDS(smem);
    const int N = a.N, C = a.C;
    const int dag0 = blockIdx.x * PACK_DAGS;
    const int nd = (a.B - dag0 < PACK_DAGS) ? a.B - dag0 : PACK_DAGS;
    float* s_lab = (float*)smem;
    float* s_pos = s_lab + PACK_DAGS * 16 * 16;
    float* s_adj = s_pos + PACK_DAGS * 16 * 16;
    float* s_msk = s_adj + PACK_DAGS * 16 * 16;
    {
        const float* src[4] = {a.lab1h + (size_t)dag0 * N * C, a.pos1h + (size_t)dag0 * N * N, a.adj + (size_t)dag0 * N * N,
                               (const float*)(a.tmask + (size_t)dag0 * 8 * N * N)};
        float* dst[4] = {s_lab, s_pos, s_adj, s_msk};
        const int nf[4] = {nd * N * C, nd * N * N, nd * N * N, nd * 8 * N * N / 4};
        bool whole = true;
#pragma unroll
        for (int k = 0; k < 4; ++k) whole = whole && (nf[k] & 3) == 0 && (nf[k] >> 2) <= 2 * (int)blockDim.x;
        if (whole) {
            f4 v[4][2];
#pragma unroll
            for (int k = 0; k < 4; ++k)
#pragma unroll
                for (int u = 0; u < 2; ++u) {
                    const int i = (int)threadIdx.x + u * (int)blockDim.x;
                    v[k][u] = *(const f4*)(src[k] + 4 * (i < (nf[k] >> 2) ? i : 0));
                }
#pragma unroll
            for (int k = 0; k < 4; ++k)
#pragma unroll
                for (int u = 0; u < 2; ++u) {
                    const int i = (int)threadIdx.x + u * (int)blockDim.x;
                    if (i < (nf[k] >> 2)) *(f4*)(dst[k] + 4 * i) = v[k][u];
                }
        } else {
#pragma unroll
            for (int k = 0; k < 4; ++k) pack_stream(dst[k], src[k], (size_t)nf[k]);
        }
    }
    __syncthreads();
    const int h = threadIdx.x / (16 * PACK_DAGS), d = (threadIdx.x >> 4) % PACK_DAGS, i = threadIdx.x & 15;
    if (d >= nd) return;
    const uint8_t* msk = (const uint8_t*)s_msk;
    int bad = 0;
    if (h > 0) {
        if (i < N) {
            const uint8_t* m0 = msk + ((size_t)d * 8 * N + i) * N;
            const uint8_t* mh = msk + (((size_t)d * 8 + h) * N + i) * N;
            for (int j = 0; j < N; ++j)
                if ((mh[j] != 0) != (m0[j] != 0)) bad |= 2;
        }
        if (bad) atomicOr(a.status, bad);
        return;
    }
    int label = 0, pos = 0;
    unsigned parents = 0, allowed = 1u << i;
    if (i < N) {
        const float* lr = s_lab + ((size_t)d * N + i) * C;
        int ones = 0;
        for (int c = 0; c < C; ++c) {
            const float v = lr[c];
            if (v == 1.0f) { label = c; ++ones; } else if (v != 0.0f) bad |= 1;
        }
        if (ones != 1) bad |= 1;
        const float* pr = s_pos + ((size_t)d * N + i) * N;
        ones = 0;
        for (int c = 0; c < N; ++c) {
            const float v = pr[c];
            if (v == 1.0f) { pos = c; ++ones; } else if (v != 0.0f) bad |= 1;
        }
        if (ones != 1) bad |= 1;
        const float* ad = s_adj + (size_t)d * N * N;
        for (int j = 0; j < N; ++j)
            if (ad[j * N + i] != 0.0f) parents |= 1u << j;
        allowed = 0;
        const uint8_t* m0 = msk + ((size_t)d * 8 * N + i) * N;
        for (int j = 0; j < N; ++j)
            if (!m0[j]) allowed |= 1u << j;
        if (!((allowed >> i) & 1u)) bad |= 4;
    }
    DvsRecord* r = a.rec + dag0 + d;
    r->label[i] = (uint8_t)label;
    r->pos[i] = (uint8_t)pos;
    r->parents[i] = (uint16_t)parents;
    r->allowed[i] = (uint16_t)allowed;
    if (bad) atomicOr(a.status, bad);
}

void dvs_launch_pack(const PackArgs& a, dvs_stream_t st) {
    const size_t lds = (size_t)PACK_DAGS * (3 * 256 * 4 + 8 * 256);
    DVS_SET_LDS(k_pack, lds);
    DVS_LAUNCH(k_pack, dim3((a.B + PACK_DAGS - 1) / PACK_DAGS), dim3(8 * 16 * PACK_DAGS), lds, st, a);
}

__global__ __launch_bounds__(256) void k_build_records(BuildArgs a) {
    __shared__ unsigned short s_child[16][256];
    __shared__ unsigned short s_reach[16][256];
    __shared__ unsigned char s_indeg[16][256];
    __shared__ unsigned char s_order[16][256];
    const int tid = threadIdx.x;
    const int dag = blockIdx.x * 256 + tid;
    if (dag >= a.B) return;
    const int N = a.N, n = N - 3, out_id = N - 1;
    int bad = 0;
    for (int v = 0; v < 16; ++v) s_child[v][tid] = 0;
    s_child[0][tid] = 1u << 1;
    unsigned haspred = 0;
    for (int v = 0; v < n; ++v) {
        const unsigned p = a.preds[(size_t)dag * n + v];
        if (p >> v) bad |= 8;
        for (int u = 0; u < v; ++u)
            if ((p >> u) & 1u) s_child[u + 2][tid] |= (unsigned short)(1u << (v + 2));
        if (p & ((1u << v) - 1u)) haspred |= 1u << v;
    }
    for (int v = 0; v < n; ++v)
        if (!((haspred >> v) & 1u)) s_child[1][tid] |= (unsigned short)(1u << (v + 2));
    for (int v = 0; v < N - 1; ++v)
        if (s_child[v][tid] == 0) s_child[v][tid] = (unsigned short)(1u << out_id);
    for (int v = 0; v < 16; ++v) s_indeg[v][tid] = 0;
    for (int u = 0; u < N; ++u) {
        unsigned c = s_child[u][tid];
        while (c) {
            const int v = __ffs((int)c) - 1;
            c &= c - 1;
            s_indeg[v][tid]++;
        }
    }
    int tail = 0;
    for (int v = 0; v < N; ++v)
        if (s_indeg[v][tid] == 0) s_order[tail++][tid] = (unsigned char)v;
    for (int head = 0; head < tail && head < N; ++head) {
        unsigned c = s_child[s_order[head][tid]][tid];
        while (c) {
            const int v = __ffs((int)c) - 1;
            c &= c - 1;
            if (--s_indeg[v][tid] == 0 && tail < 16) s_order[tail++][tid] = (unsigned char)v;
        }
    }
    if (tail != N) bad |= 8;
    for (int v = 0; v < N; ++v) s_reach[v][tid] = (unsigned short)(s_child[v][tid] | (1u << v));
    for (int k = 0; k < N; ++k) {
        const unsigned rk = s_reach[k][tid];
        for (int v = 0; v < N; ++v)
            if ((s_reach[v][tid] >> k) & 1u) s_reach[v][tid] |= (unsigned short)rk;
    }
    DvsRecord* r = a.rec + dag;
    for (int i = 0; i < 16; ++i) {
        int label = 0, pos = 0;
        unsigned parents = 0, allowed = 1u << i;
        if (i < N) {
            if (i == 0) label = 2;
            else if (i == 1) label = 0;
            else if (i == out_id) label = 1;
            else {
                label = a.labels[(size_t)dag * n + (i - 2)] + 3;
                if (label >= a.C) { bad |= 1; label = 0; }
            }
            pos = s_order[i][tid];
            allowed = 0;
            for (int j = 0; j < N; ++j) {
                if ((s_child[j][tid] >> i) & 1u) parents |= 1u << j;
                if ((s_reach[j][tid] >> i) & 1u) allowed |= 1u << j;
            }
        }
        r->label[i] = (uint8_t)label;
        r->pos[i] = (uint8_t)pos;
        r->parents[i] = (uint16_t)parents;
        r->allowed[i] = (uint16_t)allowed;
    }
    if (bad) atomicOr(a.status, bad);
}

void dvs_launch_build_records(const BuildArgs& a, dvs_stream_t st) {
    DVS_LAUNCH(k_build_records, dim3((a.B + 255) / 256), dim3(256), 0, st, a);
}

struct EmbLds {
    float *W1, *W2, *labw, *labb, *scr;
};
__device__ __forceinline__ EmbLds emb_lds(char* smem) {
    EmbLds l;
    l.W1 = (float*)smem;
    l.W2 = l.W1 + 2 * DVS_MAXTOK * DVS_LD;
    l.labw = l.W2 + 64 * EMB_LDW2;
    l.labb = l.labw + 32 * 16;
    l.scr = l.labb + 32;
    return l;
}
static size_t emb_lds_floats(int nwaves) {
    const size_t n = 2 * DVS_MAXTOK * DVS_LD + 64 * EMB_LDW2 + 32 * 16 + 32 + (size_t)nwaves * 16;
    return n > (size_t)DvsEmbImg::FLOATS ? n : (size_t)DvsEmbImg::FLOATS;
}

__global__ __launch_bounds__(1024) void k_embed_fwd(EmbedArgs a, DvsStagePlan plan) {
    DVS_DYN_LDS(smem);
    const int N = a.dims.N, C = a.dims.C;
    const EmbLds l = emb_lds(smem);
    if (blockDim.x >= 1024) dvs_stage_now<2>(&plan, smem);
    else dvs_stage_now<5>(&plan, smem);
    __syncthreads();
    const Lane L = dvs_lane();
    const DvsDrop D = dvs_drop_of(a.dims);
    float* scr = l.scr + L.wave * 16;
    for (int dag = blockIdx.x * L.nwaves + L.wave; dag < a.dims.B; dag += gridDim.x * L.nwaves) {
        const DvsRecord* rec = a.rec + dag;
        const bool valid = L.r < N;
        const EmbSel sel = dvs_emb_selectors(rec, N, scr, L);
        f4 eh[4];
        dvs_emb_hidden(eh, l.W1, N, sel, L);
        const uint32_t gdag = a.dims.dag_offset + dag;
        const int label = rec->label[L.r];
        for (int v = 0; v < (a.out2 ? 2 : 1); ++v) {
            const int site = v ? a.site2 : a.site;
            f4 e1[4];
#pragma unroll
            for (int t = 0; t < 4; ++t) e1[t] = eh[t];
            dvs_dropout_tile(e1, dvs_site_key(a.dims.seed_lo, a.dims.seed_hi, site, gdag), D, L);
            f4 x[4];
            f4 e2[2] = {f4_zero(), f4_zero()};
#pragma unroll
            for (int t = 0; t < 4; ++t) {
                const f4 w0 = dvs_wcol(l.W2, EMB_LDW2, 0, t, L), w1 = dvs_wcol(l.W2, EMB_LDW2, 16, t, L);
#pragma unroll
                for (int kk = 0; kk < 4; ++kk) {
                    e2[0] = dvs_mfma(w0[kk], e1[t][kk], e2[0]);
                    e2[1] = dvs_mfma(w1[kk], e1[t][kk], e2[1]);
                }
            }
            {
                f4 tmp[2] = {e2[0], e2[1]};
                dvs_dropout_tile<2>(tmp, dvs_site_key(a.dims.seed_lo, a.dims.seed_hi, site + 1, gdag), D, L);
                x[2] = tmp[0];
                x[3] = tmp[1];
            }
#pragma unroll
            for (int t = 0; t < 2; ++t)
#pragma unroll
                for (int kk = 0; kk < 4; ++kk) {
                    const int f = 16 * t + 4 * L.g + kk;
                    x[t][kk] = valid ? fmaxf(l.labw[f * 16 + label] + l.labb[f], 0.f) : 0.f;
                }
            if (!valid) { x[2] = f4_zero(); x[3] = f4_zero(); }
            dvs_store_tile(v ? a.out2 : a.out, dag, x, L);
        }
    }
}

void dvs_launch_embed_fwd(const EmbedArgs& a, int grid, int nw, dvs_stream_t st) {
    const size_t lds = emb_lds_floats(16) * 4;
    DvsStagePlan plan;
    dvs_plan_clear(plan);
    dvs_plan_seg(plan, DVS_FAKE_LDS, DVS_FAKE_LDS, a.embimg, 2 * DvsEmbImg::FLOATS);
    dvs_plan_seal(plan);
    DVS_SET_LDS(k_embed_fwd, lds);
    DVS_LAUNCH(k_embed_fwd, dim3(grid), dim3(nw == 4 ? 256 : 1024), lds, st, a, plan);
}

#ifdef DVS_STAMPS
DVS_STAMP_DECL(dvs_stamps_fwd);
struct DvsLatTag { int phase; };
__device__ const DvsLatTag dvs_lat_tag = {6};
#define DVS_LAT_STAMP(id) DVS_STAMP(dvs_stamps_fwd, &dvs_lat_tag, id)
DVS_ACC_STAMP_DECL(dvs_stamps_attn);
#endif
#define ASTAMP(k) DVS_ACC_STAMP(dvs_stamps_attn, ast_, k)
#include "dvs_latent.h"
struct AttnLds {
    dvs_bf16 *Win, *Wout;
    float *inb, *outb, *lg, *lb;
};
DVS_HD inline AttnLds attn_lds(char* smem) {
    AttnLds l;
    l.Win = (dvs_bf16*)smem;
    l.Wout = l.Win + 3 * 192 * DVS_LDB;
    l.inb = (float*)(l.Wout + 3 * 64 * DVS_LDB);
    l.outb = l.inb + 192;
    l.lg = l.outb + 64;
    l.lb = l.lg + 64;
    return l;
}
static size_t attn_lds_bytes() { return 3 * 256 * DVS_LDB * sizeof(dvs_bf16) + (192 + 64 + 128) * sizeof(float); }

inline void attn_plan(DvsStagePlan& p, const AttnArgs& a, char* smem) {
    const AttnLds l = attn_lds(smem);
    dvs_plan_clear(p);
    dvs_plan_seg(p, smem, l.Win, (const dvs_bf16*)a.wimg + DvsAttnImg::Win, (int)(DvsAttnImg::WoutT - DvsAttnImg::Win));
    dvs_plan_vec(p, smem, l.inb, a.in_b, 192, true);
    dvs_plan_vec(p, smem, l.outb, a.out_b, 64);
    dvs_plan_vec(p, smem, l.lg, a.ln.g, a.ln.stats ? 64 : 0);
    dvs_plan_vec(p, smem, l.lb, a.ln.b, a.ln.stats ? 64 : 0);
    dvs_plan_seal(p);
}

__device__ __forceinline__ void attn_qkv(f4 (&q)[4], f4 (&k)[4], f4 (&v)[4], const Split3T& x, const Split3T& kv,
                                         const AttnLds& l, const Lane& L) {
#pragma unroll
    for (int t = 0; t < 4; ++t) {
        q[t] = dvs_vecT(l.inb, t, L);
        k[t] = dvs_vecT(l.inb + 64, t, L);
        v[t] = f4_splat(l.inb[128 + 16 * t + L.r]);
    }
    dvs_matb3<4>(q, x, l.Win, 192, 0, L);
    dvs_matb3<4>(k, kv, l.Win, 192, 64, L);
    dvs_matb3<4, true>(v, kv, l.Win, 192, 128, L);
    const float scale = 0.35355339059327373f;
#pragma unroll
    for (int t = 0; t < 4; ++t) q[t] *= scale;
}

__device__ __forceinline__ void attn_scores_T(f4 (&s)[8], const f4 (&q)[4], const f4 (&k)[4], const Lane& L) {
#pragma unroll
    for (int h = 0; h < 8; ++h) s[h] = f4_zero();
#pragma unroll
    for (int kk = 0; kk < 2; ++kk)
#pragma unroll
        for (int t = 0; t < 4; ++t) {
            s[2 * t] = dvs_mfma(k[t][kk], q[t][kk], s[2 * t]);
            s[2 * t + 1] = dvs_mfma(k[t][kk + 2], q[t][kk + 2], s[2 * t + 1]);
        }
}
__device__ __forceinline__ void attn_softmax_T(f4 (&p)[8], float (&m)[8], float (&den)[8], const f4 (&s)[8],
                                               unsigned allowed_r, const Lane& L) {
    bool ok[4];
#pragma unroll
    for (int reg = 0; reg < 4; ++reg) ok[reg] = (allowed_r >> (4 * L.g + reg)) & 1u;
#pragma unroll
    for (int h = 0; h < 8; ++h) {
        float mx = -3.0e38f;
#pragma unroll
        for (int reg = 0; reg < 4; ++reg) mx = ok[reg] ? fmaxf(mx, s[h][reg]) : mx;
        m[h] = mx;
    }
#pragma unroll
    for (int h = 0; h < 8; ++h) m[h] = dvs_max_x16(m[h]);
#pragma unroll
    for (int h = 0; h < 8; ++h) m[h] = dvs_max_x32(m[h]);
#pragma unroll
    for (int h = 0; h < 8; ++h) {
        float sum = 0.f;
#pragma unroll
        for (int reg = 0; reg < 4; ++reg) {
            p[h][reg] = ok[reg] ? __expf(s[h][reg] - m[h]) : 0.f;
            sum += p[h][reg];
        }
        den[h] = sum;
    }
#pragma unroll
    for (int h = 0; h < 8; ++h) den[h] = dvs_add_x16(den[h]);
#pragma unroll
    for (int h = 0; h < 8; ++h) den[h] = dvs_add_x32(den[h]);
#pragma unroll
    for (int h = 0; h < 8; ++h) p[h] *= (1.0f / den[h]);
}

__device__ __forceinline__ f4 attn_drop_T(f4 p, uint32_t key, int h, const DvsDrop& D, const Lane& L) {
    if (!D.on) return p;
    const uint32_t p0 = (uint32_t)((h * 16 + L.r) * 8 + 2 * L.g);
    const uint32_t h0 = dvs_draw(key, p0), h1 = dvs_draw(key, p0 + 1);
    p[0] = ((h0 & 0xFFFFu) >= D.thr16) ? p[0] * D.scale : 0.f;
    p[1] = ((h0 >> 16) >= D.thr16) ? p[1] * D.scale : 0.f;
    p[2] = ((h1 & 0xFFFFu) >= D.thr16) ? p[2] * D.scale : 0.f;
    p[3] = ((h1 >> 16) >= D.thr16) ? p[3] * D.scale : 0.f;
    return p;
}

template <class PP>
__device__ __forceinline__ void dvs_fwd_tail(PP next, bool has_next, char* smem, PP mine) {
    if (has_next) {
        DvsPrefetch<DVS_PF_FWD_TAIL> pf;
        const bool fetcher = dvs_tid() < DVS_PF_THREADS;
        if (fetcher) dvs_prefetch_issue<false>(pf, next, dvs_tid(), DVS_PF_THREADS);
        DVS_STAMP(dvs_stamps_fwd, mine, 3);
        dvs_lds_barrier();
        DVS_STAMP(dvs_stamps_fwd, mine, 4);
        if (fetcher) dvs_prefetch_commit<false>(pf, next, smem, dvs_tid(), DVS_PF_THREADS);
        DVS_STAMP(dvs_stamps_fwd, mine, 6);
    }
}

template <int NW, class PP>
__device__ __forceinline__ void dvs_attn_fwd_phase(const AttnArgs& a, char* smem, PP mine, bool stage_mine, PP next,
                                                   bool has_next) {
    const AttnLds l = attn_lds(smem);
    DVS_STAMP(dvs_stamps_fwd, mine, 0);
    if (stage_mine) {
        dvs_stage_now<(NW >= 8 ? DVS_PF_FWD : DVS_PF_FWD_TAIL)>(mine, smem);
        __syncthreads();
    }
    DVS_STAMP(dvs_stamps_fwd, mine, 1);
    const Lane L = dvs_lane();
    const DvsDrop D = dvs_drop_of(a.dims);
    const int N = a.dims.N;
#ifdef DVS_STAMPS
    unsigned long long ast_ = __builtin_amdgcn_s_memtime();
#endif
    bool gate = !stage_mine;
    for (int base = dvs_bid() * L.nwaves; base < a.dims.B; base += gridDim.x * L.nwaves) {
        const int dag = base + L.wave;
        if (dag >= a.dims.B) {
            DVS_PHASE_GATE(gate);
            continue;
        }
        ASTAMP(7);
        f4 x[4], dummy[4], kvt[4];
        float rstd;
        {
            DvsRawX rx;
            dvs_load_x_issue(rx, a.xin, a.ln, dag, L);
            if (a.kv) dvs_load_tile(kvt, a.kv, dag, L);
            DVS_PHASE_GATE(gate);
            dvs_load_x_finish<false>(x, dummy, rstd, rx, a.ln, l.lg, l.lb, N, L);
        }
#ifdef DVS_STAMPS
        asm volatile("s_waitcnt vmcnt(0)" ::: "memory");
#endif
        ASTAMP(0);
        f4 q[4], k[4], v[4];
        {
            const Split3T xs = dvs_split3_T(x);
            if (a.kv) {
                attn_qkv(q, k, v, xs, dvs_split3_T(kvt), l, L);
            } else {
                attn_qkv(q, k, v, xs, xs, l, L);
            }
        }
        ASTAMP(1);
        const unsigned allowed_r = a.rec[dag].allowed[L.r];
        const uint32_t gdag = a.dims.dag_offset + dag;
        const uint32_t kprob = dvs_site_key(a.dims.seed_lo, a.dims.seed_hi, a.site_prob, gdag);
        f4 s[8], p[8];
        float m[8], den[8];
        attn_scores_T(s, q, k, L);
        attn_softmax_T(p, m, den, s, allowed_r, L);
        ASTAMP(2);
#pragma unroll
        for (int h = 0; h < 8; ++h) p[h] = attn_drop_T(p[h], kprob, h, D, L);
        ASTAMP(3);
        f4 o[4];
        {
            f4 oa[4], ob[4];
#pragma unroll
            for (int t = 0; t < 4; ++t) oa[t] = ob[t] = f4_zero();
#pragma unroll
            for (int kk = 0; kk < 4; ++kk)
#pragma unroll
                for (int t = 0; t < 4; ++t) {
                    oa[t] = dvs_mfma(v[t][kk], p[2 * t][kk], oa[t]);
                    ob[t] = dvs_mfma(v[t][kk], p[2 * t + 1][kk], ob[t]);
                }
#pragma unroll
            for (int t = 0; t < 4; ++t) o[t] = f4{oa[t][0], oa[t][1], ob[t][2], ob[t][3]};
        }
        ASTAMP(4);
        f4 y[4];
#pragma unroll
        for (int t = 0; t < 4; ++t) y[t] = dvs_vecT(l.outb, t, L);
        dvs_matb3<4>(y, dvs_split3_T(o), l.Wout, 64, 0, L);
        ASTAMP(5);
        dvs_dropout_tile(y, dvs_site_key(a.dims.seed_lo, a.dims.seed_hi, a.site_post, gdag), D, L);
        const bool valid = L.r < N;
#pragma unroll
        for (int t = 0; t < 4; ++t)
#pragma unroll
            for (int kk = 0; kk < 4; ++kk) y[t][kk] = valid ? x[t][kk] + y[t][kk] : 0.f;
        dvs_store_pre(a.out_pre, a.out_stats, dag, y, L);
        ASTAMP(6);
    }
    DVS_PHASE_GATE(gate);
    DVS_STAMP(dvs_stamps_fwd, mine, 2);
    dvs_fwd_tail(next, has_next, smem, mine);
}

template <int NW>
__global__ __launch_bounds__(64 * NW) void k_attn_fwd(AttnArgs a, DvsStagePlan plan) {
    DVS_DYN_LDS(smem);
    dvs_attn_fwd_phase<NW>(a, smem, &plan, true, &plan, false);
}

void dvs_launch_attn_fwd(const AttnArgs& a, int grid, int nw, dvs_stream_t st) {
    const size_t lds = attn_lds_bytes();
    DvsStagePlan plan;
    attn_plan(plan, a, DVS_FAKE_LDS);
    if (nw == 4) {
        DVS_SET_LDS(k_attn_fwd<4>, lds);
        DVS_LAUNCH_AS("k_attn_fwd", k_attn_fwd<4>, dim3(grid), dim3(256), lds, st, a, plan);
    } else {
        DVS_SET_LDS(k_attn_fwd<8>, lds);
        DVS_LAUNCH_AS("k_attn_fwd", k_attn_fwd<8>, dim3(grid), dim3(512), lds, st, a, plan);
    }
}

struct FfnLds {
    dvs_bf16 *W1, *W2;
    float *b1, *b2, *lg, *lb, *ng, *nb;
};
DVS_HD inline FfnLds ffn_lds(char* smem) {
    FfnLds l;
    l.W1 = (dvs_bf16*)smem;
    l.W2 = l.W1 + 3 * 64 * DVS_LDB;
    l.b1 = (float*)(l.W2 + 3 * 64 * DVS_LDB);
    l.b2 = l.b1 + 64;
    l.lg = l.b2 + 64;
    l.lb = l.lg + 64;
    l.ng = l.lb + 64;
    l.nb = l.ng + 64;
    return l;
}
static size_t ffn_lds_bytes() { return 6 * 64 * DVS_LDB * sizeof(dvs_bf16) + 6 * 64 * sizeof(float); }

inline void ffn_plan(DvsStagePlan& p, const FfnArgs& a, char* smem) {
    const FfnLds l = ffn_lds(smem);
    dvs_plan_clear(p);
    dvs_plan_seg(p, smem, l.W1, (const dvs_bf16*)a.wimg + DvsFfnImg::W1, (int)(6 * DVS_IMG64));
    dvs_plan_vec(p, smem, l.b1, a.l1_b, 64);
    dvs_plan_vec(p, smem, l.b2, a.l2_b, 64);
    dvs_plan_vec(p, smem, l.lg, a.ln.g, a.ln.stats ? 64 : 0);
    dvs_plan_vec(p, smem, l.lb, a.ln.b, a.ln.stats ? 64 : 0);
    dvs_plan_vec(p, smem, l.ng, a.ng, a.out_norm ? 64 : 0);
    dvs_plan_vec(p, smem, l.nb, a.nb, a.out_norm ? 64 : 0);
    dvs_plan_seal(p);
}

template <class PP>
__device__ __forceinline__ void dvs_ffn_fwd_phase(const FfnArgs& a, char* smem, PP mine, bool stage_mine, PP next,
                                                  bool has_next) {
    const FfnLds l = ffn_lds(smem);
    DVS_STAMP(dvs_stamps_fwd, mine, 0);
    if (stage_mine) {
        dvs_stage_now<DVS_PF_FWD>(mine, smem);
        __syncthreads();
    }
    DVS_STAMP(dvs_stamps_fwd, mine, 1);
    const Lane L = dvs_lane();
    const DvsDrop D = dvs_drop_of(a.dims);
    const int ntiles = a.dims.B * a.dims.NT;
    bool gate = !stage_mine;
    for (int base = dvs_bid() * L.nwaves; base < ntiles; base += gridDim.x * L.nwaves) {
        const int tile = base + L.wave;
        if (tile >= ntiles) {
            DVS_PHASE_GATE(gate);
            continue;
        }
        const DvsTile T = dvs_tile_of(tile, a.dims);
        f4 x[4], dummy[4];
        float rstd;
        {
            DvsRawX rx;
            dvs_load_x_issue(rx, a.xin, a.ln, tile, L);
            DVS_PHASE_GATE(gate);
            dvs_load_x_finish<false>(x, dummy, rstd, rx, a.ln, l.lg, l.lb, T.Nl, L);
        }
        const uint32_t gdag = a.dims.dag_offset + T.dag;
        f4 h[4];
#pragma unroll
        for (int t = 0; t < 4; ++t) h[t] = dvs_vecT(l.b1, t, L);
        dvs_matb3<4>(h, dvs_split3_T(x), l.W1, 64, 0, L);
#pragma unroll
        for (int t = 0; t < 4; ++t)
#pragma unroll
            for (int kk = 0; kk < 4; ++kk) h[t][kk] = fmaxf(h[t][kk], 0.f);
        dvs_dropout_tile(h, dvs_site_key(a.dims.seed_lo, a.dims.seed_hi, a.site_hidden, gdag), D, L, T.tok0);
        f4 y[4];
#pragma unroll
        for (int t = 0; t < 4; ++t) y[t] = dvs_vecT(l.b2, t, L);
        dvs_matb3<4>(y, dvs_split3_T(h), l.W2, 64, 0, L);
        dvs_dropout_tile(y, dvs_site_key(a.dims.seed_lo, a.dims.seed_hi, a.site_post, gdag), D, L, T.tok0);
        const bool valid = L.r < T.Nl;
#pragma unroll
        for (int t = 0; t < 4; ++t)
#pragma unroll
            for (int kk = 0; kk < 4; ++kk) y[t][kk] = valid ? x[t][kk] + y[t][kk] : 0.f;
        float mean, rs;
        dvs_ln_stats(y, mean, rs);
        dvs_store_tile(a.out_pre, tile, y, L);
        if (L.g == 0) {
            a.out_stats[(size_t)tile * 32 + L.r] = mean;
            a.out_stats[(size_t)tile * 32 + 16 + L.r] = rs;
        }
        if (a.out_norm) {
            f4 xn[4];
#pragma unroll
            for (int t = 0; t < 4; ++t) {
                const f4 g = dvs_vecT(l.ng, t, L), b = dvs_vecT(l.nb, t, L);
#pragma unroll
                for (int kk = 0; kk < 4; ++kk) xn[t][kk] = valid ? (y[t][kk] - mean) * rs * g[kk] + b[kk] : 0.f;
            }
            dvs_store_tile(a.out_norm, tile, xn, L);
        }
    }
    DVS_PHASE_GATE(gate);
    DVS_STAMP(dvs_stamps_fwd, mine, 2);
    dvs_fwd_tail(next, has_next, smem, mine);
}

__global__ __launch_bounds__(1024) void k_ffn_fwd(FfnArgs a, DvsStagePlan plan) {
    DVS_DYN_LDS(smem);
    dvs_ffn_fwd_phase(a, smem, &plan, true, &plan, false);
}

void dvs_launch_ffn_fwd(const FfnArgs& a, int grid, int nw, dvs_stream_t st) {
    const size_t lds = ffn_lds_bytes();
    DvsStagePlan plan;
    ffn_plan(plan, a, DVS_FAKE_LDS);
    DVS_SET_LDS(k_ffn_fwd, lds);
    DVS_LAUNCH(k_ffn_fwd, dim3(grid), dim3(nw == 4 ? 256 : 1024), lds, st, a, plan);
}

template <int TAG, int NW>
__global__ __launch_bounds__(64 * NW) void k_fwd_stack(FwdStackArgs s) {
    DVS_DYN_LDS(smem);
#ifndef DVS_EMU
    const DvsPlanK plans =
        ((const __attribute__((address_space(4))) FwdStackArgs*)__builtin_amdgcn_kernarg_segment_ptr())->plan;
#else
    const DvsPlanK plans = s.plan;
#endif
    for (int i = 0; i < s.nphase; ++i) {
        const FwdPhase& ph = s.ph[i];
        const bool first = i == 0, more = i + 1 < s.nphase;
        const DvsPlanK mine = plans + i;
        if (TAG == 0 && NW == 8 && ph.kind == DVS_FPH_LATENT) {
            const int step = (int)gridDim.x * 8, B = ph.u.l.dims.B;
            for (int base = dvs_bid() * 8; base < B; base += 2 * step) {
                __syncthreads();
                dvs_latent_fwd_group(ph.u.l, smem, base, base + step);
            }
            continue;
        }
        const bool more_img = more && s.ph[i + 1].kind != DVS_FPH_LATENT;
        const DvsPlanK next = plans + (more_img ? i + 1 : i);
        if (ph.kind == DVS_FPH_ATTN) dvs_attn_fwd_phase<NW>(ph.u.a, smem, mine, first, next, more_img);
        else dvs_ffn_fwd_phase(ph.u.f, smem, mine, first, next, more_img);
    }
}

void dvs_launch_fwd_stack(const FwdStackArgs& s_in, int tag, int grid, int nw, dvs_stream_t st) {
    FwdStackArgs s = s_in;
    for (int i = 0; i < s.nphase; ++i) {
        if (s.ph[i].kind == DVS_FPH_ATTN) attn_plan(s.plan[i], s.ph[i].u.a, DVS_FAKE_LDS);
        else if (s.ph[i].kind == DVS_FPH_FFN) ffn_plan(s.plan[i], s.ph[i].u.f, DVS_FAKE_LDS);
        else dvs_plan_clear(s.plan[i]);
        s.plan[i].phase = i;
    }
#ifdef DVS_STAMPS
    for (int i = 0; i < s.nphase; ++i) s.plan[i].phase = tag * DVS_FWD_STACK_PHASES + i;
#endif
    const size_t la = attn_lds_bytes(), lf = ffn_lds_bytes();
    const size_t lds = la > lf ? la : lf;
#define DVS_FSTACK_LAUNCH(TG, NWV)                                                             \
    do {                                                                                       \
        DVS_SET_LDS((k_fwd_stack<TG, NWV>), lds);                                              \
        DVS_LAUNCH_AS("k_fwd_stack<" #TG ">", (k_fwd_stack<TG, NWV>), dim3(grid), dim3(64 * NWV), lds, st, s); \
    } while (0)
    if (nw == 4) {
        if (tag == 0) DVS_FSTACK_LAUNCH(0, 4);
        else DVS_FSTACK_LAUNCH(1, 4);
    } else {
        if (tag == 0) DVS_FSTACK_LAUNCH(0, 8);
        else DVS_FSTACK_LAUNCH(1, 8);
    }
}

__global__ void k_unfrag(const float* frag, float* out, int B) {
    const size_t i = (size_t)blockIdx.x * blockDim.x + threadIdx.x;
    if (i >= (size_t)B * 1024) return;
    const size_t dag = i >> 10;
    const int e = (int)(i & 1023);
    const int t = e >> 8, lane = (e >> 2) & 63, kk = e & 3;
    const int r = lane & 15, g = lane >> 4;
    out[dag * 1024 + r * 64 + 16 * t + 4 * g + kk] = frag[i];
}
void dvs_launch_unfrag(const float* frag, float* out, int B, dvs_stream_t st) {
    const size_t n = (size_t)B * 1024;
    DVS_LAUNCH(k_unfrag, dim3((unsigned)((n + 255) / 256)), dim3(256), 0, st, frag, out, B);
}

#ifdef DVS_STAMPS
DVS_STAMP_READER(attn)
DVS_STAMP_READER(fwd)
#endif
```

### dags_vae_search_amd/csrc/k_optim.hip

```cpp
#include "dvs_backward.h"

constexpr int SQ_PARTS = 256;
__global__ __launch_bounds__(256) void k_sqnorm_part(const float* g, int64_t n, float* scratch) {
    __shared__ float part[256];
    float s = 0.f;
    const int64_t n4 = n >> 2;
    for (int64_t i = (int64_t)blockIdx.x * 256 + threadIdx.x; i < n4; i += (int64_t)SQ_PARTS * 256) {
        const f4 v = *(const f4*)(g + 4 * i);
        s += (v[0] * v[0] + v[1] * v[1]) + (v[2] * v[2] + v[3] * v[3]);
    }
    if (blockIdx.x == 0)
        for (int64_t i = 4 * n4 + threadIdx.x; i < n; i += 256) s += g[i] * g[i];
    part[threadIdx.x] = s;
    __syncthreads();
    for (int k = 128; k > 0; k >>= 1) {
        if ((int)threadIdx.x < k) part[threadIdx.x] += part[threadIdx.x + k];
        __syncthreads();
    }
    if (threadIdx.x == 0) scratch[2 + blockIdx.x] = part[0];
}
__global__ __launch_bounds__(256) void k_adam(int64_t n, float* p, float* g, float* m, float* v, float lr, float b1, float b2,
                                              float eps, float bc1, float bc2_sqrt, float max_norm, float* scratch,
                                              const float* guard, int nparts) {
    __shared__ float part[256];
    {
        float s = 0.f;
        for (int i = threadIdx.x; i < nparts; i += 256) s += scratch[2 + i];
        part[threadIdx.x] = s;
    }
    __syncthreads();
    for (int k = 128; k > 0; k >>= 1) {
        if ((int)threadIdx.x < k) part[threadIdx.x] += part[threadIdx.x + k];
        __syncthreads();
    }
    const float ss = part[0];
    float coef = 1.0f;
    if (max_norm > 0.f) {
        coef = max_norm / (sqrtf(ss) + 1e-6f);
        coef = coef < 1.0f ? coef : 1.0f;
    }
    if (blockIdx.x == 0 && threadIdx.x == 0) {
        scratch[0] = ss;
        scratch[1] = coef;
    }
    if (guard && (guard[0] != 0.f || guard[1] != 0.f)) return;
    const int64_t i = (int64_t)blockIdx.x * blockDim.x + threadIdx.x;
    if (i >= n) return;
    const float gi = g[i] * coef;
    g[i] = gi;
    const float mi = b1 * m[i] + (1.0f - b1) * gi;
    const float vi = b2 * v[i] + (1.0f - b2) * gi * gi;
    m[i] = mi;
    v[i] = vi;
    const float denom = sqrtf(vi) / bc2_sqrt + eps;
    p[i] -= (lr / bc1) * (mi / denom);
}

void dvs_launch_clip_adam(int64_t n, float* params, float* grads, float* m, float* v, float lr, float b1, float b2,
                          float eps, int64_t step, float max_norm, float* scratch, const float* guard, bool have_partials,
                          dvs_stream_t st) {
    if (!have_partials) DVS_LAUNCH(k_sqnorm_part, dim3(SQ_PARTS), dim3(256), 0, st, (const float*)grads, n, scratch);
    const float bc1 = 1.0f - powf(b1, (float)step);
    const float bc2 = 1.0f - powf(b2, (float)step);
    DVS_LAUNCH(k_adam, dim3((unsigned)((n + 255) / 256)), dim3(256), 0, st, n, params, grads, m, v, lr, b1, b2, eps,
                       bc1, sqrtf(bc2), max_norm, scratch, guard, have_partials ? dvs_sq_parts(n) : SQ_PARTS);
}

#include "dvs_wimg.h"
__device__ __forceinline__ float dvs_loss_head_value(const DvsLossHeadArgs& h, int i) {
    if (i < 32 * 68) {
        const int r = i / 68, c = i % 68;
        return c < 64 ? h.node0_w[r * 64 + c] : 0.f;
    }
    i -= 32 * 68;
    if (i < 16 * 36) {
        const int c = i / 36, k = i % 36;
        return (c < h.C && k < 32) ? h.node2_w[c * 32 + k] : 0.f;
    }
    i -= 16 * 36;
    if (i < 32) return h.node0_b[i];
    i -= 32;
    if (i < 16) return i < h.C ? h.node2_b[i] : 0.f;
    i -= 16;
    if (i < 64) return h.edge0_b[i];
    i -= 64;
    if (i < 64) return h.edge2_w[i];
    i -= 64;
    if (i < 16) return i == 0 ? h.edge2_b[0] : 0.f;
    i -= 16;
    if (i < 64) return h.ln_g[i];
    return h.ln_b[i - 64];
}
__device__ __forceinline__ float dvs_emb_block_value(const DvsLossHeadArgs& h, int i) {
    if (i < 32 * 68) {
        const int r = i / 68, c = i % 68;
        return (r < 2 * h.N && c < 64) ? h.W1[r * 64 + c] : 0.f;
    }
    i -= 32 * 68;
    if (i < 64 * 36) {
        const int f = i / 36, k = i % 36;
        return k < 32 ? h.W2[f * 32 + k] : 0.f;
    }
    i -= 64 * 36;
    if (i < 512) {
        const int f = i >> 4, c = i & 15;
        return c < h.C ? h.lab_w[f * h.C + c] : 0.f;
    }
    i -= 512;
    return i < 32 ? h.lab_b[i] : 0.f;
}
__global__ __launch_bounds__(256) void k_prepare_images(DvsImgJobs jobs, const float* params, dvs_bf16* wimg, DvsLatImgArgs lat,
                                                        DvsLossHeadArgs head) {
    const int nlat = 1024 * lat.NT / 64;
    const int first_job = nlat + (head.dst ? 2 : 0);
    if (head.dst) {
        if ((int)blockIdx.x == nlat + 1) {
            float v[DvsEmbImg::FLOATS / 256];
#pragma unroll
            for (int u = 0; u < DvsEmbImg::FLOATS / 256; ++u) v[u] = dvs_emb_block_value(head, u * 256 + (int)threadIdx.x);
#pragma unroll
            for (int u = 0; u < DvsEmbImg::FLOATS / 256; ++u) head.dst_emb[u * 256 + threadIdx.x] = v[u];
            return;
        }
        if ((int)blockIdx.x == nlat) {
            float v[DvsLossImg::HEAD_FLOATS / 256];
#pragma unroll
            for (int u = 0; u < DvsLossImg::HEAD_FLOATS / 256; ++u) v[u] = dvs_loss_head_value(head, u * 256 + (int)threadIdx.x);
#pragma unroll
            for (int u = 0; u < DvsLossImg::HEAD_FLOATS / 256; ++u) head.dst[u * 256 + threadIdx.x] = v[u];
            return;
        }
    }
    if ((int)blockIdx.x < nlat) {
        __shared__ float tile[64][65];
        const int K = 1024 * lat.NT, kp0 = (int)blockIdx.x * 64;
        const int l = threadIdx.x & 63, w = threadIdx.x >> 6;
        const size_t ldw = (size_t)lat.N * 64;
        auto col_of = [&](int kp, bool& valid) {
            const int tile_i = kp >> 10, q = (kp & 1023) >> 2, kk = kp & 3, t = q >> 6, ln = q & 63;
            const int tok = 16 * tile_i + (ln & 15), feat = 16 * t + 4 * (ln >> 4) + kk;
            valid = tok < lat.N;
            return (size_t)(valid ? tok : 0) * 64 + feat;
        };
        bool valid;
        const size_t col = col_of(kp0 + l, valid);
        float va[16];
#pragma unroll
        for (int i = 0; i < 16; ++i) {
            const int o = w + 4 * i;
            va[i] = !valid ? 0.f : (o < 32 ? lat.fc1_w[o * ldw + col] : lat.fc2_w[(o - 32) * ldw + col]);
        }
        float v3[8];
#pragma unroll
        for (int i = 0; i < 8; ++i) {
            bool v2;
            const size_t c2 = col_of(kp0 + 2 * (w + 4 * i) + (l >> 5), v2);
            v3[i] = v2 ? lat.fc3_w[c2 * 32 + (l & 31)] : 0.f;
        }
        const float vb3 = valid ? lat.fc3_b[col] : 0.f;
#pragma unroll
        for (int i = 0; i < 16; ++i) {
            const int o = w + 4 * i;
            tile[o][l] = va[i];
            lat.img[DvsLatImg::A(lat.NT) + (size_t)o * DvsLatImg::LD(lat.NT) + kp0 + l] = va[i];
        }
        __syncthreads();
        for (int j = w; j < 64; j += 4) lat.img[DvsLatImg::AT(lat.NT) + (size_t)(kp0 + j) * 64 + l] = tile[l][j];
        __syncthreads();
#pragma unroll
        for (int i = 0; i < 8; ++i) {
            const int jj = 2 * (w + 4 * i) + (l >> 5), o = l & 31;
            tile[o][jj] = v3[i];
            lat.img[DvsLatImg::W3(lat.NT) + (size_t)(kp0 + jj) * 32 + o] = v3[i];
        }
        __syncthreads();
        for (int o = w; o < 32; o += 4) lat.img[DvsLatImg::W3T(lat.NT) + (size_t)o * DvsLatImg::LD(lat.NT) + kp0 + l] = tile[o][l];
        if (w == 0) lat.img[DvsLatImg::B3(lat.NT) + kp0 + l] = vb3;
        return;
    }
    const int jb = ((int)blockIdx.x - first_job) / 12, slice = ((int)blockIdx.x - first_job) % 12;
    const DvsImgJob J = jobs.job[jb];
    const bool transposed = J.flags & 1, rperm = J.flags & 2, cperm = J.flags & 4;
    const float* src = params + J.src;
    dvs_bf16* dst = wimg + J.dst;
    for (int i = threadIdx.x; i < 16 * 64; i += blockDim.x) {
        const int row = 16 * slice + (i >> 6), col = i & 63;
        if (row >= J.rows) break;
        const float v = src[(size_t)(rperm ? dvs_pi(row) : row) * ((J.flags & 8) ? 128 : 64) + (cperm ? dvs_pi(col) : col)];
        if (!transposed) {
            dvs_bf16 h, m, l;
            dvs_split3_1(v, h, m, l);
            const size_t o = (size_t)row * DVS_LDB + dvs_kperm(col), part = (size_t)J.rows * DVS_LDB;
            dst[o] = h;
            dst[part + o] = m;
            if (!(J.flags & 16)) dst[2 * part + o] = l;
        } else {
            dvs_bf16 h, l;
            dvs_split1(v, h, l);
            const size_t o = (size_t)col * DVS_LDB + dvs_kperm(row);
            dst[o] = h;
            dst[DVS_IMG64 + o] = l;
        }
    }
}
void dvs_launch_prepare_images(const DvsImgJobs& jobs, const float* params, dvs_bf16* wimg, const DvsLatImgArgs& lat,
                               const DvsLossHeadArgs& head, dvs_stream_t st) {
    DVS_LAUNCH(k_prepare_images, dim3(jobs.count * 12 + 1024 * lat.NT / 64 + (head.dst ? 2 : 0)), dim3(256), 0, st, jobs, params,
               wimg, lat, head);
}
```

### dags_vae_search_amd/engine.py

```python
from __future__ import annotations

import ctypes
from typing import Dict, Optional

import torch

from . import _lib as dl


def _ptr(t: Optional[torch.Tensor]):
    return None if t is None else ctypes.c_void_p(t.data_ptr())


def _nbytes(t: torch.Tensor) -> int:
    return t.numel() * t.element_size()


def _stream():
    return ctypes.c_void_p(torch.cuda.current_stream().cuda_stream)


def _require_cuda(t: torch.Tensor, what: str):
    if not t.is_cuda:
        raise RuntimeError(f"dags_vae_search_amd: {what} must live on the GPU (got device {t.device}); "
                           f"this package has no CPU path")


class PaceEngine:

    def __init__(self, n_tokens: int, n_classes: int):
        self.lib = dl.load()
        self.n_tokens = int(n_tokens)
        self.n_classes = int(n_classes)
        shape = dl.make_shape(1, n_tokens, n_classes)
        if self.lib.dvs_param_count(ctypes.byref(shape)) < 0:
            dl.check(self.lib, 1, "dvs_param_count")
        self.table, self.param_floats = dl.param_table(self.lib, shape)
        self.record_bytes = dl.record_bytes(self.lib, shape)
        self.wide = dl.is_wide(self.n_tokens, self.n_classes)
        self.tiles = (self.n_tokens + dl.TILE_TOKENS - 1) // dl.TILE_TOKENS
        self._ws: Optional[torch.Tensor] = None
        self._ws_batch = 0
        self._records: Optional[torch.Tensor] = None
        self._status: Optional[torch.Tensor] = None
        self._status_external = False

    def shape(self, batch, training=False, dropout=0.15, beta=0.005, eps_scale=0.01, dag_offset=0, seed=0):
        return dl.make_shape(batch, self.n_tokens, self.n_classes, training, dropout, beta, eps_scale, dag_offset, seed)

    def workspace(self, batch: int, device) -> torch.Tensor:
        if self._ws is None or self._ws_batch != batch or self._ws.device != device:
            shape = self.shape(batch)
            nbytes = self.lib.dvs_workspace_bytes(ctypes.byref(shape))
            if nbytes == 0:
                dl.check(self.lib, 1, "dvs_workspace_bytes")
            self._ws = torch.zeros((nbytes + 3) // 4, dtype=torch.float32, device=device)
            self._ws_batch = batch
            self._records = torch.empty(batch * self.record_bytes, dtype=torch.uint8, device=device)
            if not self._status_external or self._status.device != device:
                self._status = torch.zeros(1, dtype=torch.int32, device=device)
                self._status_external = False
        return self._ws

    def use_status(self, status: torch.Tensor):
        self._status = status
        self._status_external = True

    def _read_status(self) -> int:
        st = int(self._status.item())
        if st:
            self._status.zero_()
        return st

    def pack(self, features: Dict, check: bool = True, zero_status: bool = True) -> torch.Tensor:
        lab = features["vertex_label_features"]
        pos = features["vertex_position_features"]
        adj = features["adjacency_matrices"]
        tm = features["target_masks"]
        for name, t in (("vertex_label_features", lab), ("vertex_position_features", pos),
                        ("adjacency_matrices", adj), ("target_masks", tm)):
            _require_cuda(t, name)
        B, N, C = lab.shape
        if N != self.n_tokens or C != self.n_classes:
            raise AssertionError(f"Expected [B,{self.n_tokens},{self.n_classes}] label features, got {tuple(lab.shape)}")
        if tuple(pos.shape) != (B, N, N) or tuple(adj.shape) != (B, N, N) or tuple(tm.shape) != (8 * B, N, N):
            raise AssertionError("feature tensors have inconsistent shapes")
        def aligned(t, dtype):
            if t.dtype != dtype:
                t = t.to(dtype)
            if not t.is_contiguous():
                t = t.contiguous()
            return t if t.data_ptr() % 16 == 0 else t.clone()
        lab = aligned(lab, torch.float32)
        pos = aligned(pos, torch.float32)
        adj = aligned(adj, torch.float32)
        tm = aligned(tm, tm.dtype)
        tm = tm.view(torch.uint8) if tm.dtype == torch.bool else aligned(tm, torch.uint8)
        self.workspace(B, lab.device)
        if zero_status:
            self._status.zero_()
        shape = self.shape(B)
        dl.check(self.lib, self.lib.dvs_pack_features(ctypes.byref(shape), _ptr(lab), _ptr(pos), _ptr(adj), _ptr(tm),
                                                      _ptr(self._records), _nbytes(self._records), _ptr(self._status),
                                                      _stream()),
                 "dvs_pack_features")
        if check:
            st = self._read_status()
            if st:
                raise ValueError(f"features violate the prepare_features invariants (status bits {st:#x}: "
                                 f"1 = label/position row not one-hot, 2 = per-head masks differ, 4 = self masked)")
        return self._records

    def build_records(self, labels: torch.Tensor, preds: torch.Tensor, check: bool = True,
                      zero_status: bool = True) -> torch.Tensor:
        _require_cuda(labels, "labels")
        _require_cuda(preds, "preds")
        B, n = labels.shape
        if n != self.n_tokens - 3 or tuple(preds.shape) != (B, n):
            raise AssertionError(f"Expected {self.n_tokens - 3}, got instead {n}")
        labels = labels.contiguous().to(torch.uint8)
        preds = preds.contiguous().to(torch.int64 if self.wide else torch.int16)
        self.workspace(B, labels.device)
        if zero_status:
            self._status.zero_()
        shape = self.shape(B)
        dl.check(self.lib, self.lib.dvs_build_records(ctypes.byref(shape), _ptr(labels), _ptr(preds), _ptr(self._records),
                                                      _nbytes(self._records), _ptr(self._status), _stream()),
                 "dvs_build_records")
        if check:
            st = self._read_status()
            if st:
                raise ValueError(f"invalid compact DAG batch (status bits {st:#x}: 1 = label out of range, "
                                 f"8 = edge not from a lower to a higher vertex id)")
        return self._records

    def loss_forward(self, shape, params: torch.Tensor, eps: Optional[torch.Tensor], losses: torch.Tensor,
                     mu: Optional[torch.Tensor] = None, logvar: Optional[torch.Tensor] = None,
                     host_tail: Optional[torch.Tensor] = None, host_seq: int = 0):
        _require_cuda(params, "parameters")
        ws = self.workspace(shape.batch, params.device)
        if losses.numel() < dl.LOSS_FLOATS:
            raise ValueError(f"losses must hold {dl.LOSS_FLOATS} floats")
        if host_tail is None:
            dl.check(self.lib, self.lib.dvs_loss_forward(ctypes.byref(shape), _ptr(self._records), _nbytes(self._records),
                                                         _ptr(params), params.numel(), _ptr(ws), _nbytes(ws), _ptr(eps),
                                                         _ptr(self._status), _ptr(losses), _ptr(mu), _ptr(logvar), _stream()),
                     "dvs_loss_forward")
            return
        if not host_tail.is_pinned() or host_tail.numel() < 4 or host_tail.dtype != torch.float32 or host_tail.data_ptr() % 16:
            raise ValueError("host_tail must be at least 4 pinned float32 words, 16-byte aligned")
        dl.check(self.lib, self.lib.dvs_loss_forward_notify(
            ctypes.byref(shape), _ptr(self._records), _nbytes(self._records), _ptr(params), params.numel(), _ptr(ws), _nbytes(ws),
            _ptr(eps), _ptr(self._status), _ptr(losses), _ptr(mu), _ptr(logvar), host_tail.data_ptr(), int(host_seq) & 0xFFFFFF,
            _stream()), "dvs_loss_forward_notify")

    def loss_backward(self, shape, params: torch.Tensor, gcoef: torch.Tensor, grads: torch.Tensor,
                      clip_scratch: Optional[torch.Tensor] = None):
        ws = self.workspace(shape.batch, params.device)
        if grads.numel() < params.numel():
            raise ValueError("gradient buffer is smaller than the parameter buffer")
        if clip_scratch is not None:
            if clip_scratch.numel() < dl.CLIP_SCRATCH_FLOATS or clip_scratch.dtype != torch.float32:
                raise ValueError(f"clip_scratch must hold {dl.CLIP_SCRATCH_FLOATS} float32 words")
            dl.check(self.lib, self.lib.dvs_loss_backward_sq(
                ctypes.byref(shape), _ptr(self._records), _nbytes(self._records), _ptr(params), params.numel(), _ptr(ws), _nbytes(ws),
                _ptr(gcoef), _ptr(grads), _ptr(clip_scratch), _stream()), "dvs_loss_backward_sq")
            return
        dl.check(self.lib, self.lib.dvs_loss_backward(ctypes.byref(shape), _ptr(self._records), _nbytes(self._records),
                                                      _ptr(params), params.numel(), _ptr(ws), _nbytes(ws), _ptr(gcoef),
                                                      _ptr(grads), _stream()), "dvs_loss_backward")

    def encode(self, shape, params: torch.Tensor, mu: torch.Tensor, logvar: torch.Tensor):
        ws = self.workspace(shape.batch, params.device)
        dl.check(self.lib, self.lib.dvs_encode(ctypes.byref(shape), _ptr(self._records), _nbytes(self._records),
                                               _ptr(params), params.numel(), _ptr(ws), _nbytes(ws), _ptr(mu), _ptr(logvar),
                                               _stream()), "dvs_encode")

    def decode(self, shape, params: torch.Tensor, z: torch.Tensor, uniforms: Optional[torch.Tensor]) -> torch.Tensor:
        _require_cuda(params, "parameters")
        _require_cuda(z, "z")
        B = z.shape[0]
        ws = self.workspace(B, params.device)
        state = torch.empty(B, dl.DECODE_STATE_BYTES, dtype=torch.uint8, device=params.device)
        dl.check(self.lib, self.lib.dvs_decode(ctypes.byref(shape), _ptr(params), params.numel(), _ptr(ws), _nbytes(ws),
                                               _ptr(self._records), _nbytes(self._records), _ptr(z), _ptr(uniforms),
                                               _ptr(state), _nbytes(state), _stream()), "dvs_decode")
        return state

    def clip_adam(self, params, grads, exp_avg, exp_avg_sq, lr, beta1, beta2, eps, step, max_norm, scratch, guard=None,
                  from_partials: bool = False):
        fn = self.lib.dvs_clip_adam_from_partials if from_partials else self.lib.dvs_clip_adam
        dl.check(self.lib, fn(params.numel(), _ptr(params), _ptr(grads), _ptr(exp_avg), _ptr(exp_avg_sq), lr, beta1, beta2, eps,
                              int(step), float(max_norm), _ptr(scratch), _ptr(guard), _stream()),
                 "dvs_clip_adam_from_partials" if from_partials else "dvs_clip_adam")

    def activation(self, batch: int, slot: int) -> torch.Tensor:
        out = torch.empty(batch, 16 * self.tiles, 64, dtype=torch.float32, device=self._ws.device)
        shape = self.shape(batch)
        dl.check(self.lib, self.lib.dvs_debug_activation(ctypes.byref(shape), _ptr(self._ws), slot, _ptr(out), _stream()),
                 "dvs_debug_activation")
        return out

    def flatten(self, params: Dict[str, torch.Tensor], device) -> torch.Tensor:
        flat = torch.zeros(self.param_floats, dtype=torch.float32, device=device)
        for name, off, shp in self.table:
            v = params[name].detach().to(device=device, dtype=torch.float32).reshape(-1)
            flat[off:off + v.numel()] = v
        return flat

    def unflatten(self, flat: torch.Tensor) -> Dict[str, torch.Tensor]:
        out = {}
        for name, off, shp in self.table:
            n = 1
            for s in shp:
                n *= s
            out[name] = flat[off:off + n].view(shp)
        return out
```

### dags_vae_search_amd/pace.py

```python
from __future__ import annotations

import copy
import math
from typing import Dict, List, Optional, Tuple

import os

import torch
from torch import nn

from . import _lib as dl
from . import features as feat
from .engine import PaceEngine
from .records import CompactBatch

LABEL_KEY = feat.LABEL_KEY
POSITION_KEY = feat.POSITION_KEY


class GnnPositionalEncoding(nn.Module):
    def __init__(self, ninp, dropout, max_n):
        super().__init__()
        self.ninp, self.max_n, self.dropout = ninp, max_n, dropout
        self.W1 = nn.Parameter(torch.zeros(2 * max_n, 2 * ninp))
        self.W2 = nn.Parameter(torch.zeros(2 * ninp, ninp))
        nn.init.xavier_uniform_(self.W1.data, gain=1.414)
        nn.init.xavier_uniform_(self.W2.data, gain=1.414)


class _EncoderLayerParams(nn.Module):
    def __init__(self, d_model, nhead, dim_feedforward, dropout):
        super().__init__()
        self.self_attn = nn.MultiheadAttention(d_model, nhead, dropout=dropout)
        self.linear1 = nn.Linear(d_model, dim_feedforward)
        self.linear2 = nn.Linear(dim_feedforward, d_model)
        self.norm1 = nn.LayerNorm(d_model, eps=1e-5)
        self.norm2 = nn.LayerNorm(d_model, eps=1e-5)


class _DecoderLayerParams(nn.Module):
    def __init__(self, d_model, nhead, dim_feedforward, dropout):
        super().__init__()
        self.self_attn = nn.MultiheadAttention(d_model, nhead, dropout=dropout)
        self.multihead_attn = nn.MultiheadAttention(d_model, nhead, dropout=dropout)
        self.linear1 = nn.Linear(d_model, dim_feedforward)
        self.linear2 = nn.Linear(dim_feedforward, d_model)
        self.norm1 = nn.LayerNorm(d_model, eps=1e-5)
        self.norm2 = nn.LayerNorm(d_model, eps=1e-5)
        self.norm3 = nn.LayerNorm(d_model, eps=1e-5)


class _Stack(nn.Module):
    def __init__(self, layer, num_layers):
        super().__init__()
        self.layers = nn.ModuleList([copy.deepcopy(layer) for _ in range(num_layers)])
        self.num_layers = num_layers


class _PaceLoss(torch.autograd.Function):

    @staticmethod
    def forward(ctx, model, shape, eps, *params):
        losses = torch.zeros(dl.LOSS_FLOATS, dtype=torch.float32, device=model.flat_params.device)
        model._engine.loss_forward(shape, model.flat_params, eps, losses)
        model._fwd_generation += 1
        ctx.model, ctx.shape, ctx.generation = model, shape, model._fwd_generation
        model._last_losses = losses
        return losses[0].clone(), losses[1].clone(), losses[2].clone()

    @staticmethod
    def backward(ctx, g_total, g_recon, g_kld):
        model = ctx.model
        if ctx.generation != model._fwd_generation:
            raise RuntimeError("PaceVaeV3: the saved activations of this loss were overwritten by a later forward "
                               "(call backward() before the next loss_direct())")
        dev = model.flat_params.device
        z = torch.zeros((), device=dev)
        g_total = z if g_total is None else g_total
        g_recon = z if g_recon is None else g_recon
        g_kld = z if g_kld is None else g_kld
        gcoef = torch.stack([g_total + g_recon, ctx.shape.beta * g_total + g_kld]).float().contiguous()
        flat = torch.empty_like(model.flat_params)
        model._engine.loss_backward(ctx.shape, model.flat_params, gcoef, flat)
        grads = [flat[off:off + n].view(shp) for (_, off, shp), n in zip(model._engine.table, model._numels)]
        return (None, None, None, *grads)


_EARLY_READ_MODE = os.environ.get("DVS_EARLY_READ", "poll")


class PaceVaeV3(nn.Module):
    def __init__(
            self,
            max_num_vertices: int,
            vertex_label_cardinality: int,
            vertices_embedding_size: int = 256,
            num_heads: int = 8,
            num_layers: int = 6,
            ff_hidden_size: int = 512,
            latent_layer_size: int = 64,
            fc_hidden: int = 256,
            dropout: float = 0.25,
            graph_label_key: str = LABEL_KEY,
            graph_position_key: str = POSITION_KEY,
            graph_label_input: int = 0,
            graph_label_output: int = 1,
            graph_label_start: int = 2,
    ):
        super().__init__()
        built = dict(vertices_embedding_size=dl.EMB, num_heads=dl.HEADS, num_layers=dl.LAYERS,
                     ff_hidden_size=dl.D_MODEL, latent_layer_size=dl.LATENT, fc_hidden=dl.FC_HIDDEN)
        given = dict(vertices_embedding_size=vertices_embedding_size, num_heads=num_heads, num_layers=num_layers,
                     ff_hidden_size=ff_hidden_size, latent_layer_size=latent_layer_size, fc_hidden=fc_hidden)
        if given != built:
            raise NotImplementedError(f"this MI355X build implements the BASELINE architecture {built}; got {given}")
        if max_num_vertices + 3 > dl.MAX_TOKENS or vertex_label_cardinality + 3 > dl.MAX_TOKENS or max_num_vertices < 1:
            raise NotImplementedError("this build supports max_num_vertices <= 45 and vertex_label_cardinality <= 45 "
                                      "(up to three 16-token tiles per DAG)")
        self._max_num_vertices = max_num_vertices + 3
        self._vertex_label_cardinality = vertex_label_cardinality + 3
        self.vertices_embedding_size = vertices_embedding_size
        self.num_heads = num_heads
        self.num_layers = num_layers
        self.ff_hidden_size = ff_hidden_size
        self.latent_layer_size = latent_layer_size
        self.dropout = dropout
        self._graph_label_key = graph_label_key
        self._graph_position_key = graph_position_key
        self._graph_label_input = graph_label_input
        self._graph_label_output = graph_label_output
        self._graph_label_start = graph_label_start

        self.vertex_position_embed = GnnPositionalEncoding(vertices_embedding_size, dropout, self.max_num_vertices)
        self.vertex_label_embed = nn.Sequential(nn.Linear(self._vertex_label_cardinality, vertices_embedding_size),
                                                nn.ReLU())
        self.encoder = _Stack(_EncoderLayerParams(ff_hidden_size, num_heads, ff_hidden_size, dropout), num_layers)
        hidden_size = self.ff_hidden_size * self.max_num_vertices
        self.hidden_size = hidden_size
        self.fc1 = nn.Linear(hidden_size, latent_layer_size)
        self.fc2 = nn.Linear(hidden_size, latent_layer_size)
        self.decoder = _Stack(_DecoderLayerParams(ff_hidden_size, num_heads, ff_hidden_size, dropout), num_layers)
        self.add_node = nn.Sequential(nn.Linear(ff_hidden_size, fc_hidden), nn.ReLU(),
                                      nn.Linear(fc_hidden, self._vertex_label_cardinality))
        self.add_edge = nn.Sequential(nn.Linear(ff_hidden_size * 2, ff_hidden_size), nn.ReLU(),
                                      nn.Linear(ff_hidden_size, 1))
        self.fc3 = nn.Linear(latent_layer_size, hidden_size)

        self._engine: Optional[PaceEngine] = None
        self._table = None
        self._numels: List[int] = []
        self.flat_params: Optional[torch.Tensor] = None
        self.flat_grads: Optional[torch.Tensor] = None
        self._fwd_generation = 0
        self._last_losses = None
        self._side_stream = None
        self._early_pending = False
        self._early_scalars = None
        self._seed = 0
        self._step = 0
        self.dag_offset = 0
        self.nan_check = True
        self._flatten()

    @property
    def max_num_vertices(self) -> int:
        return self._max_num_vertices

    @property
    def vertex_label_cardinality(self) -> int:
        return self._vertex_label_cardinality

    @property
    def graph_label_key(self) -> str:
        return self._graph_label_key

    @property
    def graph_position_key(self) -> str:
        return self._graph_position_key

    @property
    def graph_label_input(self) -> int:
        return self._graph_label_input

    @property
    def graph_label_output(self) -> int:
        return self._graph_label_output

    @property
    def graph_label_start(self) -> int:
        return self._graph_label_start

    def _layout(self):
        if self._table is None:
            lib = dl.load()
            shape = dl.make_shape(1, self._max_num_vertices, self._vertex_label_cardinality)
            self._table, self._total = dl.param_table(lib, shape)
            names = [n for n, _ in self.named_parameters()]
            assert [t[0] for t in self._table] == names, "state-dict order mismatch with the C layout"
        return self._table, self._total

    def _flatten(self):
        table, total = self._layout()
        params = dict(self.named_parameters())
        dev = next(iter(params.values())).device
        flat = torch.zeros(total, dtype=torch.float32, device=dev)
        self._numels = []
        for name, off, shp in table:
            p = params[name]
            n = p.numel()
            self._numels.append(n)
            flat[off:off + n] = p.data.reshape(-1).float()
            p.data = flat[off:off + n].view(shp)
            p.grad = None
        self.flat_params = flat
        self.flat_grads = None
        self._grad_params = None
        self._step_losses = None

    def _apply(self, fn, recurse=True):
        out = super()._apply(fn, recurse)
        self._flatten()
        self._engine = None
        self._side_stream = None
        self._early_pending = False
        return out

    def bind_flat_grads(self) -> torch.Tensor:
        if self.flat_grads is None or self.flat_grads.device != self.flat_params.device:
            P = self.flat_params.numel()
            self._grads_and_losses = torch.zeros(P + 8, dtype=torch.float32, device=self.flat_params.device)
            self.flat_grads = self._grads_and_losses[:P]
            self._step_losses = self._grads_and_losses[P:P + dl.LOSS_FLOATS]
            self._fixed_guard = self._grads_and_losses[P + 3:P + 5]
            self._step_guard = self._fixed_guard
            self._step_tail = self._grads_and_losses[P:P + 8]
            self._step_status = self._grads_and_losses[P + 7:P + 8].view(torch.int32)
            self._host_tail = torch.zeros(8, dtype=torch.float32)
            if self.flat_params.is_cuda:
                self._host_tail = self._host_tail.pin_memory()
            self._grad_params = None
            if self._engine is not None:
                self._engine.use_status(self._step_status)
        if self._grad_params is None:
            params = dict(self.named_parameters())
            self._grad_params = [params[name] for name, _, _ in self._table]
        first, last = self._grad_params[0], self._grad_params[-1]
        base = self.flat_grads.data_ptr()
        if (first.grad is None or last.grad is None or first.grad.data_ptr() != base + 4 * self._table[0][1]
                or last.grad.data_ptr() != base + 4 * self._table[-1][1]):
            for p, (name, off, shp), n in zip(self._grad_params, self._table, self._numels):
                p.grad = self.flat_grads[off:off + n].view(shp)
        return self.flat_grads

    def _eng(self) -> PaceEngine:
        if not self.flat_params.is_cuda:
            raise RuntimeError("dags_vae_search_amd.PaceVaeV3 computes only on the GPU: call model.to('cuda') first "
                               "(there is no CPU fallback)")
        if self._engine is None:
            self._engine = PaceEngine(self._max_num_vertices, self._vertex_label_cardinality)
            assert self._engine.param_floats == self.flat_params.numel()
            if self.flat_grads is not None and self.flat_grads.device == self.flat_params.device:
                self._engine.use_status(self._step_status)
        return self._engine

    def seed(self, seed: int):
        self._seed = int(seed) & 0xFFFFFFFF
        self._step = 0

    def _next_seed(self) -> int:
        self._step += 1
        return (self._seed << 32) | (self._step & 0xFFFFFFFF)

    def prepare_features(self, labeled_graphs_batch, fixed_memory_len: Optional[int] = None):
        device = self.flat_params.device
        return feat.prepare_features(labeled_graphs_batch, self._max_num_vertices, self._vertex_label_cardinality,
                                     self.num_heads, self._graph_label_key, self._graph_label_input,
                                     self._graph_label_output, self._graph_label_start, fixed_memory_len, device)

    def _pack(self, features, check: Optional[bool] = None, zero_status: bool = True):
        eng = self._eng()
        dev = self.flat_params.device
        check = self.nan_check if check is None else check
        if isinstance(features, CompactBatch):
            eng.build_records(features.labels.to(dev), features.preds.to(dev), check=check, zero_status=zero_status)
            return len(features)
        f = {k: features[k].to(dev) for k in ("vertex_label_features", "vertex_position_features",
                                              "adjacency_matrices", "target_masks")}
        eng.pack(f, check=check, zero_status=zero_status)
        return f["vertex_label_features"].shape[0]

    def _early_read(self, exchange=None):
        if self._side_stream is None:
            self._side_stream = torch.cuda.Stream(device=self.flat_params.device, priority=-1)
            self._ev_tail = torch.cuda.Event()
            self._ev_forward = torch.cuda.Event()
        self._ev_forward.record(torch.cuda.current_stream())
        with torch.cuda.stream(self._side_stream):
            self._side_stream.wait_event(self._ev_forward)
            src = self._step_losses
            if exchange is not None:
                src = exchange.scalars(src)
                self._host_tail[:dl.LOSS_FLOATS].copy_(src, non_blocking=True)
                self._host_tail[7:8].copy_(self._step_tail[7:8], non_blocking=True)
            else:
                self._host_tail.copy_(self._step_tail, non_blocking=True)
            self._step_status.zero_()
            self._early_scalars = src.clone()
            self._ev_tail.record(self._side_stream)
        self._early_pending = True

    def read_step(self):
        if self._early_pending == "poll":
            self._early_pending = False
            words = self._host_tail.numpy().view("uint32")
            seq, spins = self._host_seq, 0
            while int(words[3]) >> 8 != seq:
                spins += 1
                if spins > 2_000_000:
                    torch.cuda.current_stream().synchronize()
                    if int(words[3]) >> 8 != seq:
                        raise RuntimeError("the device never signalled the end of the forward (dvs_loss_forward_notify)")
            for _ in range(4):
                word = int(words[3])
                vals = self._host_tail[:3].tolist() + [float((word >> 6) & 1), float((word >> 7) & 1)]
                if int(words[3]) == word and word >> 8 == seq:
                    break
            else:
                raise RuntimeError("dvs_loss_forward_notify: the notification packet kept changing while it was read")
            self._early_scalars = self._notify_losses
            return vals, word & 0x3F
        if self._early_pending:
            self._early_pending = False
            self._ev_tail.synchronize()
        else:
            self._host_tail.copy_(self._step_tail, non_blocking=True)
            self._step_status.zero_()
            torch.cuda.current_stream().synchronize()
        vals = self._host_tail.tolist()
        status = int(self._host_tail.view(torch.int32)[7])
        return vals[:5], status

    def _shape(self, batch: int, beta: float):
        return self._eng().shape(batch, training=self.training, dropout=self.dropout, beta=beta, eps_scale=0.01,
                                 dag_offset=self.dag_offset, seed=self._next_seed() if self.training else 0)

    def encode_direct(self, features: Dict) -> Tuple[torch.Tensor, torch.Tensor]:
        B = self._pack(features)
        dev = self.flat_params.device
        mu = torch.empty(B, self.latent_layer_size, device=dev)
        logvar = torch.empty(B, self.latent_layer_size, device=dev)
        shape = self._shape(B, 0.005)
        self._engine.encode(shape, self.flat_params, mu, logvar)
        self._fwd_generation += 1
        return mu, logvar

    def encode(self, labeled_graphs_batch) -> Tuple[torch.Tensor, torch.Tensor]:
        return self.encode_direct(self.prepare_features(labeled_graphs_batch))

    def reparameterize(self, mu: torch.Tensor, log_var: torch.Tensor, epsilon_scale: float = 0.01) -> torch.Tensor:
        if self.training:
            std = torch.exp(0.5 * log_var)
            return mu + torch.randn_like(std) * epsilon_scale * std
        return mu

    def decode_states(self, z: torch.Tensor, uniforms: Optional[torch.Tensor] = None) -> torch.Tensor:
        eng = self._eng()
        dev = self.flat_params.device
        z = z.to(dev, torch.float32).contiguous()
        B = z.shape[0]
        if z.dim() != 2 or z.shape[1] != self.latent_layer_size:
            raise AssertionError(f"Expected z of shape [B, {self.latent_layer_size}], got {tuple(z.shape)}")
        N = self._max_num_vertices
        if uniforms is not None:
            uniforms = uniforms.to(dev, torch.float32).contiguous()
            if tuple(uniforms.shape) != (B, N, N):
                raise AssertionError(f"Expected uniforms of shape [{B}, {N}, {N}], got {tuple(uniforms.shape)}")
        self._step += 1
        shape = eng.shape(B, training=False, dropout=self.dropout, dag_offset=self.dag_offset,
                          seed=(self._seed << 32) | (self._step & 0xFFFFFFFF))
        state = eng.decode(shape, self.flat_params, z, uniforms)
        self._fwd_generation += 1
        return state

    def decode(self, z: torch.Tensor, uniforms: Optional[torch.Tensor] = None, strict: bool = True):
        raw = self.decode_states(z, uniforms).cpu().numpy()
        return graphs_from_states(raw, self._max_num_vertices, strict)

    def loss_direct(self, features: Dict, beta: float = 0.005, eps: Optional[torch.Tensor] = None):
        B = self._pack(features)
        shape = self._shape(B, beta)
        if eps is not None:
            eps = eps.to(self.flat_params.device, torch.float32).contiguous()
        total, recon, kld = _PaceLoss.apply(self, shape, eps, *self.parameters())
        if self.nan_check and bool(self._last_losses[3].item() != 0.0):
            raise ValueError("NaN detected in the output of the PACE-VAE step")
        return total, recon, kld

    def loss(self, labeled_graphs_batch, beta: float = 0.005):
        return self.loss_direct(self.prepare_features(labeled_graphs_batch), beta)

    def loss_and_grad(self, features: Dict, beta: float = 0.005, eps: Optional[torch.Tensor] = None,
                      packed: bool = False, defer_check: bool = False, early_read: bool = False,
                      exchange=None, clip_scratch: Optional[torch.Tensor] = None) -> torch.Tensor:
        eng = self._eng()
        if self.flat_grads is None or self.flat_grads.device != self.flat_params.device:
            self.bind_flat_grads()
        if self._early_pending:
            pending, self._early_pending = self._early_pending, False
            if pending != "poll":
                self._ev_tail.synchronize()
        if not packed:
            self._pack(features, check=False if defer_check else None, zero_status=not defer_check)
        B = eng._ws_batch
        shape = self._shape(B, beta)
        grads = self.flat_grads
        losses = self._step_losses
        self._step_guard = self._fixed_guard
        notify = early_read and exchange is None and self._host_tail.is_pinned() and _EARLY_READ_MODE != "event"
        if notify:
            self._host_seq = (getattr(self, "_host_seq", 0) + 1) & 0xFFFFFF or 1
            losses = self._notify_losses = torch.empty(8, dtype=torch.float32, device=grads.device)[:dl.LOSS_FLOATS]
            self._step_guard = losses[3:5]
            eng.loss_forward(shape, self.flat_params, eps, losses, host_tail=self._host_tail, host_seq=self._host_seq)
            self._early_pending = "poll"
        else:
            eng.loss_forward(shape, self.flat_params, eps, losses)
        self._fwd_generation += 1
        if early_read and not notify:
            self._early_read(exchange)
        if not hasattr(self, "_gcoef") or self._gcoef.device != grads.device or self._gcoef_beta != beta:
            self._gcoef = torch.tensor([1.0, beta], dtype=torch.float32, device=grads.device)
            self._gcoef_beta = beta
        eng.loss_backward(shape, self.flat_params, self._gcoef, grads, clip_scratch=clip_scratch)
        self.bind_flat_grads()
        return losses


def graphs_from_states(raw, n_tokens: int, strict: bool = False):
    import numpy as np
    N = n_tokens
    B = raw.shape[0]
    labels = raw[:, 384:432].astype(np.int64) - 3
    nv = raw[:, 432:436].copy().view(np.int32)[:, 0]
    if strict and (nv < N).any():
        raise IndexError("vertex index out of range")
    cube = np.unpackbits(raw[:, :384].reshape(B, 48, 8), axis=2, bitorder="little")
    vs = np.arange(3, N - 1)
    us = np.arange(2, N - 2)
    bits = cube[:, 3:N - 1, 2:N - 2] & (us[None, None, :] < vs[None, :, None])
    bb, vi, ui = np.nonzero(bits)
    starts = np.searchsorted(bb, np.arange(B + 1))
    ev = (vs[vi] - 2).tolist()
    eu = (us[ui] - 2).tolist()
    lab_lists = labels[:, 2:N - 1].tolist()
    full = (nv >= N).tolist()
    out = []
    for b in range(B):
        if not full[b]:
            out.append(None)
            continue
        lo, hi = starts[b], starts[b + 1]
        out.append(feat.LabeledGraph(lab_lists[b], list(zip(eu[lo:hi], ev[lo:hi]))))
    return out
```

### include/dvs.h

```cpp
#ifndef DVS_H
#define DVS_H

#include <stddef.h>
#include <stdint.h>

#ifdef __cplusplus
extern "C" {
#endif

#define DVS_VERSION 202
#define DVS_NUM_PARAMS 108
#define DVS_RECORD_BYTES 96
#define DVS_RECORD_BYTES_WIDE 864
#define DVS_CLIP_SCRATCH_FLOATS 4096
#define DVS_DECODE_STATE_BYTES 440

typedef struct dvs_shape {
    int32_t batch;
    int32_t n_tokens;
    int32_t n_classes;
    int32_t training;
    float dropout;
    float beta;
    float eps_scale;
    uint32_t dag_offset;
    uint64_t seed;
} dvs_shape;

typedef struct dvs_param_entry {
    char name[64];
    int64_t offset;
    int32_t rows, cols;
} dvs_param_entry;

int dvs_version(void);
const char* dvs_last_error(void);
int dvs_device_cus(void);

int64_t dvs_param_count(const dvs_shape* s);
int dvs_param_table(const dvs_shape* s, dvs_param_entry* out, int cap);

size_t dvs_workspace_bytes(const dvs_shape* s);

size_t dvs_record_bytes(const dvs_shape* s);

int dvs_pack_features(const dvs_shape* s, const float* label_onehot, const float* pos_onehot,
                      const float* adjacency, const uint8_t* target_masks, void* records, size_t records_bytes,
                      int32_t* status, void* stream);

int dvs_build_records(const dvs_shape* s, const uint8_t* labels, const void* preds, void* records, size_t records_bytes,
                      int32_t* status, void* stream);


#define DVS_LOSS_FLOATS 5
int dvs_loss_forward(const dvs_shape* s, const void* records, size_t records_bytes, const float* params, int64_t n_params,
                     void* workspace, size_t workspace_bytes, const float* eps, const int32_t* status, float* losses,
                     float* mu, float* logvar, void* stream);

int dvs_loss_forward_notify(const dvs_shape* s, const void* records, size_t records_bytes, const float* params,
                            int64_t n_params, void* workspace, size_t workspace_bytes, const float* eps, int32_t* status,
                            float* losses, float* mu, float* logvar, void* host_tail, uint32_t host_seq, void* stream);

int dvs_loss_backward(const dvs_shape* s, const void* records, size_t records_bytes, const float* params, int64_t n_params,
                      void* workspace, size_t workspace_bytes, const float* gcoef, float* grads, void* stream);

int dvs_loss_backward_sq(const dvs_shape* s, const void* records, size_t records_bytes, const float* params, int64_t n_params,
                         void* workspace, size_t workspace_bytes, const float* gcoef, float* grads, float* clip_scratch,
                         void* stream);

int dvs_encode(const dvs_shape* s, const void* records, size_t records_bytes, const float* params, int64_t n_params,
               void* workspace, size_t workspace_bytes, float* mu, float* logvar, void* stream);

int dvs_clip_adam(int64_t n, float* params, float* grads, float* exp_avg, float* exp_avg_sq, float lr,
                  float beta1, float beta2, float adam_eps, int64_t step, float max_norm, float* scratch,
                  const float* guard, void* stream);

int dvs_clip_adam_from_partials(int64_t n, float* params, float* grads, float* exp_avg, float* exp_avg_sq, float lr,
                                float beta1, float beta2, float adam_eps, int64_t step, float max_norm, float* scratch,
                                const float* guard, void* stream);

typedef struct dvs_decode_state {
    uint64_t parents[48];
    uint8_t label[48];
    int32_t nv;
    int32_t finished;
} dvs_decode_state;

int dvs_decode(const dvs_shape* s, const float* params, int64_t n_params, void* workspace, size_t workspace_bytes,
               void* records, size_t records_bytes, const float* z, const float* uniforms, void* state_out,
               size_t state_bytes, void* stream);

int dvs_match_decoded(int32_t batch, int32_t n_vars, int32_t card, int32_t repeats, int32_t preds_are_u64,
                      const uint8_t* labels, const void* preds, const void* states, size_t state_bytes,
                      int32_t budget, uint8_t* flags, void* stream);

#define DVS_STRUCT_HASH_INVALID 0x7fffffffffffffffull
int dvs_decoded_structures(int32_t batch, int32_t n_vars, int32_t preds_are_u64, const void* states, size_t state_bytes,
                           uint64_t hash_mask, uint8_t* flags, uint8_t* labels, void* preds, uint64_t* keys,
                           size_t keys_bytes, uint64_t* hashes, void* stream);

int dvs_structset_filter(int32_t batch, int32_t n_vars, const uint64_t* sorted_hashes, const int64_t* order,
                         const uint64_t* keys, size_t keys_bytes, const uint8_t* flags, int32_t seen_count,
                         const uint64_t* seen_hashes, const uint64_t* seen_keys, size_t seen_keys_bytes, uint8_t* out,
                         void* stream);

#define DVS_GEN_LABELS_CHOICE 1
#define DVS_GEN_ACCEPT_ISOLATES 2
#define DVS_GEN_ACCEPT_NO_CONNECTIVITY 4
#define DVS_GEN_GROUP_SHIFT 8
int dvs_generate_dags(int32_t batch, int32_t n_vars, int32_t card, int32_t preds_are_u64, const int32_t* num_edges,
                      uint64_t seed, int64_t dag_offset, int32_t try_limit, int32_t flags, uint8_t* labels, void* preds,
                      size_t preds_bytes, int32_t* attempts, void* stream);

int dvs_generate_edge_counts(int32_t batch, int32_t n_entries, const int32_t* edge_counts, const int32_t* cum_weights,
                             uint64_t seed, int64_t dag_offset, int32_t* num_edges, void* stream);

int dvs_bic_scores(int32_t batch, int32_t n_vars, int32_t n_samples, const uint64_t* data, const uint8_t* card,
                   const uint64_t* parents, double* scratch, double* out, int32_t* status, void* stream);

typedef enum dvs_score_type {
    DVS_SCORE_LOGLIK = 0,
    DVS_SCORE_AIC = 1,
    DVS_SCORE_BIC = 2,
    DVS_SCORE_BDE = 3,
    DVS_SCORE_BDS = 4,
    DVS_SCORE_K2 = 5,
    DVS_SCORE_BDJ = 6
} dvs_score_type;
int dvs_bn_scores(int32_t batch, int32_t n_vars, int32_t n_samples, const uint64_t* data, const uint8_t* card,
                  const uint64_t* parents, int32_t score_type, double score_arg, double* scratch, double* out,
                  int32_t* status, void* stream);

int dvs_bic_parent_masks(int32_t batch, int32_t n_vars, int32_t preds_are_u64, const uint8_t* labels, const void* preds,
                         uint64_t* parents, int32_t* status, void* stream);

int dvs_gp_predict(int32_t batch, int32_t n_inducing, int32_t dim, const float* x, const float* inducing,
                   const double* alpha, double outputscale, double lengthscale, double constant, double* out,
                   void* stream);

int dvs_gp_kernel(int32_t na, int32_t nb, int32_t dim, const float* xa, const float* xb, double outputscale,
                  double lengthscale, double* K, void* stream);
int dvs_gp_kernel_backward(int32_t na, int32_t nb, int32_t dim, int32_t symmetric, const float* xa, const float* xb,
                           double outputscale, double lengthscale, const double* G, double* dxa, double* row_sums,
                           void* stream);

#define DVS_GP_ACQ_MAX_INDUCING 1023
int dvs_gp_acquire(int32_t batch, int32_t n_inducing, int32_t dim, int32_t ld, const float* x, const float* inducing,
                   const double* weights, double c0, double outputscale, double lengthscale, double constant, double best,
                   double xi, double* mean, double* var, double* ei, float* grad, void* stream);

void dvs_profile_enable(int on);
int dvs_profile_collect(char* names, int name_stride, int* counts, float* total_ms, int cap);

int dvs_debug_launch(size_t dynamic_lds_bytes, void* stream);

int dvs_debug_activation(const dvs_shape* s, const void* workspace, int slot, float* out, void* stream);

#ifdef __cplusplus
}
#endif
#endif
```

Measured before the change: 3.383 million DAGs/s.

## Fuse feature packing with weight-image preparation into one step prologue kernel

Adds a dvs_pack_loss_forward entry point that packs dense DAG features into records inside the same kernel launch that prepares the bf16 weight images, rather than as a separate pack launch. The pack blocks and image blocks share one grid sized for the pack part. This removes one kernel launch and one host API round trip per train step. In exchange, image blocks now run at the larger pack block size and dynamic LDS footprint, and the pace.py path is only taken when deferred checking is used.

```diff
diff --git a/dags_vae_search_amd/_lib.py b/dags_vae_search_amd/_lib.py
--- a/dags_vae_search_amd/_lib.py
+++ b/dags_vae_search_amd/_lib.py
@@ -56,6 +56,10 @@
     lib.dvs_loss_forward_notify.restype = c_int
     lib.dvs_loss_forward_notify.argtypes = [P(DvsShape), c_void_p, c_size_t, c_void_p, c_int64, c_void_p, c_size_t, c_void_p,
                                             c_void_p, c_void_p, c_void_p, c_void_p, c_void_p, ctypes.c_uint32, c_void_p]
+    lib.dvs_pack_loss_forward.restype = c_int
+    lib.dvs_pack_loss_forward.argtypes = [P(DvsShape), c_void_p, c_void_p, c_void_p, c_void_p, c_void_p, c_size_t, c_void_p,
+                                          c_int64, c_void_p, c_size_t, c_void_p, c_void_p, c_void_p, c_void_p, c_void_p,
+                                          c_void_p, ctypes.c_uint32, c_void_p]
     lib.dvs_loss_backward.restype = c_int
     lib.dvs_loss_backward.argtypes = [P(DvsShape), c_void_p, c_size_t, c_void_p, c_int64, c_void_p, c_size_t, c_void_p,
                                       c_void_p, c_void_p]
@@ -119,7 +123,7 @@
 
 
 EXPORTS = ["dvs_version", "dvs_last_error", "dvs_device_cus", "dvs_param_count", "dvs_param_table",
-           "dvs_workspace_bytes", "dvs_record_bytes", "dvs_pack_features", "dvs_build_records", "dvs_loss_forward", "dvs_loss_forward_notify", "dvs_loss_backward", "dvs_loss_backward_sq", "dvs_encode", "dvs_decode", "dvs_match_decoded", "dvs_decoded_structures", "dvs_structset_filter", "dvs_generate_dags", "dvs_generate_edge_counts", "dvs_bic_scores", "dvs_bn_scores", "dvs_bic_parent_masks", "dvs_gp_predict", "dvs_gp_kernel", "dvs_gp_kernel_backward", "dvs_gp_acquire",
+           "dvs_workspace_bytes", "dvs_record_bytes", "dvs_pack_features", "dvs_build_records", "dvs_loss_forward", "dvs_loss_forward_notify", "dvs_pack_loss_forward", "dvs_loss_backward", "dvs_loss_backward_sq", "dvs_encode", "dvs_decode", "dvs_match_decoded", "dvs_decoded_structures", "dvs_structset_filter", "dvs_generate_dags", "dvs_generate_edge_counts", "dvs_bic_scores", "dvs_bn_scores", "dvs_bic_parent_masks", "dvs_gp_predict", "dvs_gp_kernel", "dvs_gp_kernel_backward", "dvs_gp_acquire",
            "dvs_clip_adam", "dvs_clip_adam_from_partials", "dvs_debug_activation", "dvs_debug_launch", "dvs_profile_enable", "dvs_profile_collect"]
 
 
diff --git a/dags_vae_search_amd/csrc/dvs_api.hip b/dags_vae_search_amd/csrc/dvs_api.hip
--- a/dags_vae_search_amd/csrc/dvs_api.hip
+++ b/dags_vae_search_amd/csrc/dvs_api.hip
@@ -418,14 +418,8 @@
     return record_size(is_wide(s));
 }
 
-extern "C" int dvs_pack_features(const dvs_shape* s, const float* label_onehot, const float* pos_onehot,
-                                 const float* adjacency, const uint8_t* target_masks, void* records, size_t records_bytes,
-                                 int32_t* status, void* stream) {
-    if (int e = check_shape(s)) return e;
-    if (!label_onehot || !pos_onehot || !adjacency || !target_masks || !records || !status)
-        return fail(10, "dvs_pack_features: null pointer");
-    if (int e = check_records("dvs_pack_features", records_bytes, s->batch, is_wide(s))) return e;
-    call_begin();
+static PackArgs pack_args(const dvs_shape* s, const float* label_onehot, const float* pos_onehot, const float* adjacency,
+                          const uint8_t* target_masks, void* records, int32_t* status) {
     PackArgs a;
     a.B = s->batch;
     a.N = s->n_tokens;
@@ -436,6 +430,18 @@
     a.tmask = target_masks;
     a.rec = (DvsRecord*)records;
     a.status = status;
+    return a;
+}
+
+extern "C" int dvs_pack_features(const dvs_shape* s, const float* label_onehot, const float* pos_onehot,
+                                 const float* adjacency, const uint8_t* target_masks, void* records, size_t records_bytes,
+                                 int32_t* status, void* stream) {
+    if (int e = check_shape(s)) return e;
+    if (!label_onehot || !pos_onehot || !adjacency || !target_masks || !records || !status)
+        return fail(10, "dvs_pack_features: null pointer");
+    if (int e = check_records("dvs_pack_features", records_bytes, s->batch, is_wide(s))) return e;
+    call_begin();
+    const PackArgs a = pack_args(s, label_onehot, pos_onehot, adjacency, target_masks, records, status);
     if (is_wide(s)) dvs_launch_pack_w(a, (dvs_stream_t)stream);
     else dvs_launch_pack(a, (dvs_stream_t)stream);
     return call_end("dvs_pack_features");
@@ -598,7 +604,7 @@
     return a;
 }
 
-static void prepare_images(const Step& c) {
+static void prepare_images(const Step& c, const PackArgs* pack = nullptr) {
     const DvsLayout& L = c.L;
     const bool wide = c.wide;
     DvsImgJobs J;
@@ -663,6 +669,11 @@
         head.dst_emb = (float*)(wimg + DVS_WIMG_EMB);
         head.N = c.d.N;
     }
+    if (pack && !wide) {
+        dvs_launch_step_prologue(*pack, J, c.P, wimg, lat, head, c.st);
+        return;
+    }
+    if (pack) dvs_launch_pack_w(*pack, c.st);
     dvs_launch_prepare_images(J, c.P, wimg, lat, head, c.st);
 }
 
@@ -771,16 +782,10 @@
                                    (int32_t*)status, losses, mu, logvar, nullptr, 0u, stream);
 }
 
-extern "C" int dvs_loss_forward_notify(const dvs_shape* s, const void* records, size_t records_bytes, const float* params,
-                                       int64_t n_params, void* workspace, size_t workspace_bytes, const float* eps,
-                                       int32_t* status, float* losses, float* mu, float* logvar, void* host_tail,
-                                       uint32_t host_seq, void* stream) {
-    if (int e = check_shape(s)) return e;
-    if (!records || !params || !workspace || !losses) return fail(10, "dvs_loss_forward: null pointer");
-    const Step c = make_step(s, records, params, workspace, stream);
-    if (int e = check_buffers(c, "dvs_loss_forward", records_bytes, n_params, workspace_bytes)) return e;
-    call_begin();
-    prepare_images(c);
+static int loss_forward(const Step& c, const char* fn, const PackArgs* pack, const float* eps, int32_t* status, float* losses,
+                        float* mu, float* logvar, void* host_tail, uint32_t host_seq) {
+    call_begin();
+    prepare_images(c, pack);
     encoder_forward(c, latent_args(c, eps, true), c.d.drop.on, true);
     decoder_forward(c, c.d.drop.on ? 7 : 0);
     launch_loss_fwd(c, loss_args(c));
@@ -796,7 +801,32 @@
     const size_t nb = (size_t)c.d.B * 32 * sizeof(float);
     if (mu) copy_out(mu, c.ws + c.W.mu, nb, c.st);
     if (logvar) copy_out(logvar, c.ws + c.W.logvar, nb, c.st);
-    return call_end("dvs_loss_forward");
+    return call_end(fn);
+}
+
+extern "C" int dvs_loss_forward_notify(const dvs_shape* s, const void* records, size_t records_bytes, const float* params,
+                                       int64_t n_params, void* workspace, size_t workspace_bytes, const float* eps,
+                                       int32_t* status, float* losses, float* mu, float* logvar, void* host_tail,
+                                       uint32_t host_seq, void* stream) {
+    if (int e = check_shape(s)) return e;
+    if (!records || !params || !workspace || !losses) return fail(10, "dvs_loss_forward: null pointer");
+    const Step c = make_step(s, records, params, workspace, stream);
+    if (int e = check_buffers(c, "dvs_loss_forward", records_bytes, n_params, workspace_bytes)) return e;
+    return loss_forward(c, "dvs_loss_forward", nullptr, eps, status, losses, mu, logvar, host_tail, host_seq);
+}
+
+extern "C" int dvs_pack_loss_forward(const dvs_shape* s, const float* label_onehot, const float* pos_onehot,
+                                     const float* adjacency, const uint8_t* target_masks, void* records, size_t records_bytes,
+                                     const float* params, int64_t n_params, void* workspace, size_t workspace_bytes,
+                                     const float* eps, int32_t* status, float* losses, float* mu, float* logvar,
+                                     void* host_tail, uint32_t host_seq, void* stream) {
+    if (int e = check_shape(s)) return e;
+    if (!label_onehot || !pos_onehot || !adjacency || !target_masks || !records || !status || !params || !workspace || !losses)
+        return fail(10, "dvs_pack_loss_forward: null pointer");
+    const Step c = make_step(s, records, params, workspace, stream);
+    if (int e = check_buffers(c, "dvs_pack_loss_forward", records_bytes, n_params, workspace_bytes)) return e;
+    const PackArgs pack = pack_args(s, label_onehot, pos_onehot, adjacency, target_masks, records, status);
+    return loss_forward(c, "dvs_pack_loss_forward", &pack, eps, status, losses, mu, logvar, host_tail, host_seq);
 }
 
 extern "C" int dvs_encode(const dvs_shape* s, const void* records, size_t records_bytes, const float* params,
diff --git a/dags_vae_search_amd/csrc/dvs_prologue.h b/dags_vae_search_amd/csrc/dvs_prologue.h
--- /dev/null
+++ b/dags_vae_search_amd/csrc/dvs_prologue.h
@@ -0,0 +1,258 @@
+#pragma once
+#include "dvs_kernels.h"
+#include "dvs_wimg.h"
+
+constexpr int PACK_DAGS = 4;
+constexpr int PACK_THREADS = 8 * 16 * PACK_DAGS;
+constexpr size_t PACK_LDS = (size_t)PACK_DAGS * (3 * 256 * 4 + 8 * 256);
+__device__ __forceinline__ void pack_stream(float* dst, const float* __restrict__ src, size_t nfloats) {
+    const size_t n4 = nfloats >> 2;
+    size_t i = threadIdx.x;
+    for (; i + 3 * blockDim.x < n4; i += 4 * blockDim.x) {
+        f4 v[4];
+#pragma unroll
+        for (int u = 0; u < 4; ++u) v[u] = *(const f4*)(src + 4 * (i + u * blockDim.x));
+#pragma unroll
+        for (int u = 0; u < 4; ++u) *(f4*)(dst + 4 * (i + u * blockDim.x)) = v[u];
+    }
+    for (; i < n4; i += blockDim.x) *(f4*)(dst + 4 * i) = *(const f4*)(src + 4 * i);
+    for (size_t i = 4 * n4 + threadIdx.x; i < nfloats; i += blockDim.x) dst[i] = src[i];
+}
+__device__ __forceinline__ void dvs_pack_body(const PackArgs& a, char* smem, int blk) {
+    const int N = a.N, C = a.C;
+    const int dag0 = blk * PACK_DAGS;
+    const int nd = (a.B - dag0 < PACK_DAGS) ? a.B - dag0 : PACK_DAGS;
+    float* s_lab = (float*)smem;
+    float* s_pos = s_lab + PACK_DAGS * 16 * 16;
+    float* s_adj = s_pos + PACK_DAGS * 16 * 16;
+    float* s_msk = s_adj + PACK_DAGS * 16 * 16;
+    {
+        const float* src[4] = {a.lab1h + (size_t)dag0 * N * C, a.pos1h + (size_t)dag0 * N * N, a.adj + (size_t)dag0 * N * N,
+                               (const float*)(a.tmask + (size_t)dag0 * 8 * N * N)};
+        float* dst[4] = {s_lab, s_pos, s_adj, s_msk};
+        const int nf[4] = {nd * N * C, nd * N * N, nd * N * N, nd * 8 * N * N / 4};
+        bool whole = true;
+#pragma unroll
+        for (int k = 0; k < 4; ++k) whole = whole && (nf[k] & 3) == 0 && (nf[k] >> 2) <= 2 * (int)blockDim.x;
+        if (whole) {
+            f4 v[4][2];
+#pragma unroll
+            for (int k = 0; k < 4; ++k)
+#pragma unroll
+                for (int u = 0; u < 2; ++u) {
+                    const int i = (int)threadIdx.x + u * (int)blockDim.x;
+                    v[k][u] = *(const f4*)(src[k] + 4 * (i < (nf[k] >> 2) ? i : 0));
+                }
+#pragma unroll
+            for (int k = 0; k < 4; ++k)
+#pragma unroll
+                for (int u = 0; u < 2; ++u) {
+                    const int i = (int)threadIdx.x + u * (int)blockDim.x;
+                    if (i < (nf[k] >> 2)) *(f4*)(dst[k] + 4 * i) = v[k][u];
+                }
+        } else {
+#pragma unroll
+            for (int k = 0; k < 4; ++k) pack_stream(dst[k], src[k], (size_t)nf[k]);
+        }
+    }
+    __syncthreads();
+    const int h = threadIdx.x / (16 * PACK_DAGS), d = (threadIdx.x >> 4) % PACK_DAGS, i = threadIdx.x & 15;
+    if (d >= nd) return;
+    const uint8_t* msk = (const uint8_t*)s_msk;
+    int bad = 0;
+    if (h > 0) {
+        if (i < N) {
+            const uint8_t* m0 = msk + ((size_t)d * 8 * N + i) * N;
+            const uint8_t* mh = msk + (((size_t)d * 8 + h) * N + i) * N;
+            for (int j = 0; j < N; ++j)
+                if ((mh[j] != 0) != (m0[j] != 0)) bad |= 2;
+        }
+        if (bad) atomicOr(a.status, bad);
+        return;
+    }
+    int label = 0, pos = 0;
+    unsigned parents = 0, allowed = 1u << i;
+    if (i < N) {
+        const float* lr = s_lab + ((size_t)d * N + i) * C;
+        int ones = 0;
+        for (int c = 0; c < C; ++c) {
+            const float v = lr[c];
+            if (v == 1.0f) { label = c; ++ones; } else if (v != 0.0f) bad |= 1;
+        }
+        if (ones != 1) bad |= 1;
+        const float* pr = s_pos + ((size_t)d * N + i) * N;
+        ones = 0;
+        for (int c = 0; c < N; ++c) {
+            const float v = pr[c];
+            if (v == 1.0f) { pos = c; ++ones; } else if (v != 0.0f) bad |= 1;
+        }
+        if (ones != 1) bad |= 1;
+        const float* ad = s_adj + (size_t)d * N * N;
+        for (int j = 0; j < N; ++j)
+            if (ad[j * N + i] != 0.0f) parents |= 1u << j;
+        allowed = 0;
+        const uint8_t* m0 = msk + ((size_t)d * 8 * N + i) * N;
+        for (int j = 0; j < N; ++j)
+            if (!m0[j]) allowed |= 1u << j;
+        if (!((allowed >> i) & 1u)) bad |= 4;
+    }
+    DvsRecord* r = a.rec + dag0 + d;
+    r->label[i] = (uint8_t)label;
+    r->pos[i] = (uint8_t)pos;
+    r->parents[i] = (uint16_t)parents;
+    r->allowed[i] = (uint16_t)allowed;
+    if (bad) atomicOr(a.status, bad);
+}
+
+__device__ __forceinline__ float dvs_loss_head_value(const DvsLossHeadArgs& h, int i) {
+    if (i < 32 * 68) {
+        const int r = i / 68, c = i % 68;
+        return c < 64 ? h.node0_w[r * 64 + c] : 0.f;
+    }
+    i -= 32 * 68;
+    if (i < 16 * 36) {
+        const int c = i / 36, k = i % 36;
+        return (c < h.C && k < 32) ? h.node2_w[c * 32 + k] : 0.f;
+    }
+    i -= 16 * 36;
+    if (i < 32) return h.node0_b[i];
+    i -= 32;
+    if (i < 16) return i < h.C ? h.node2_b[i] : 0.f;
+    i -= 16;
+    if (i < 64) return h.edge0_b[i];
+    i -= 64;
+    if (i < 64) return h.edge2_w[i];
+    i -= 64;
+    if (i < 16) return i == 0 ? h.edge2_b[0] : 0.f;
+    i -= 16;
+    if (i < 64) return h.ln_g[i];
+    return h.ln_b[i - 64];
+}
+__device__ __forceinline__ float dvs_emb_block_value(const DvsLossHeadArgs& h, int i) {
+    if (i < 32 * 68) {
+        const int r = i / 68, c = i % 68;
+        return (r < 2 * h.N && c < 64) ? h.W1[r * 64 + c] : 0.f;
+    }
+    i -= 32 * 68;
+    if (i < 64 * 36) {
+        const int f = i / 36, k = i % 36;
+        return k < 32 ? h.W2[f * 32 + k] : 0.f;
+    }
+    i -= 64 * 36;
+    if (i < 512) {
+        const int f = i >> 4, c = i & 15;
+        return c < h.C ? h.lab_w[f * h.C + c] : 0.f;
+    }
+    i -= 512;
+    return i < 32 ? h.lab_b[i] : 0.f;
+}
+constexpr int IMG_THREADS = 256;
+constexpr size_t IMG_LDS = 64 * 65 * sizeof(float);
+inline int dvs_image_blocks(const DvsImgJobs& jobs, const DvsLatImgArgs& lat, const DvsLossHeadArgs& head) {
+    return jobs.count * 12 + 1024 * lat.NT / 64 + (head.dst ? 2 : 0);
+}
+__device__ __forceinline__ void dvs_prepare_images_body(const DvsImgJobs& jobs, const float* params, dvs_bf16* wimg,
+                                                        const DvsLatImgArgs& lat, const DvsLossHeadArgs& head,
+                                                        float (*tile)[65], int blk) {
+    const bool on = (int)threadIdx.x < IMG_THREADS;
+    const int nlat = 1024 * lat.NT / 64;
+    const int first_job = nlat + (head.dst ? 2 : 0);
+    if (head.dst) {
+        if (blk == nlat + 1) {
+            if (!on) return;
+            float v[DvsEmbImg::FLOATS / 256];
+#pragma unroll
+            for (int u = 0; u < DvsEmbImg::FLOATS / 256; ++u) v[u] = dvs_emb_block_value(head, u * 256 + (int)threadIdx.x);
+#pragma unroll
+            for (int u = 0; u < DvsEmbImg::FLOATS / 256; ++u) head.dst_emb[u * 256 + threadIdx.x] = v[u];
+            return;
+        }
+        if (blk == nlat) {
+            if (!on) return;
+            float v[DvsLossImg::HEAD_FLOATS / 256];
+#pragma unroll
+            for (int u = 0; u < DvsLossImg::HEAD_FLOATS / 256; ++u) v[u] = dvs_loss_head_value(head, u * 256 + (int)threadIdx.x);
+#pragma unroll
+            for (int u = 0; u < DvsLossImg::HEAD_FLOATS / 256; ++u) head.dst[u * 256 + threadIdx.x] = v[u];
+            return;
+        }
+    }
+    if (blk < nlat) {
+        const int kp0 = blk * 64;
+        const int l = threadIdx.x & 63, w = (threadIdx.x >> 6) & 3;
+        const size_t ldw = (size_t)lat.N * 64;
+        auto col_of = [&](int kp, bool& valid) {
+            const int tile_i = kp >> 10, q = (kp & 1023) >> 2, kk = kp & 3, t = q >> 6, ln = q & 63;
+            const int tok = 16 * tile_i + (ln & 15), feat = 16 * t + 4 * (ln >> 4) + kk;
+            valid = tok < lat.N;
+            return (size_t)(valid ? tok : 0) * 64 + feat;
+        };
+        bool valid;
+        const size_t col = col_of(kp0 + l, valid);
+        float va[16];
+        float v3[8];
+        float vb3 = 0.f;
+        if (on) {
+#pragma unroll
+            for (int i = 0; i < 16; ++i) {
+                const int o = w + 4 * i;
+                va[i] = !valid ? 0.f : (o < 32 ? lat.fc1_w[o * ldw + col] : lat.fc2_w[(o - 32) * ldw + col]);
+            }
+#pragma unroll
+            for (int i = 0; i < 8; ++i) {
+                bool v2;
+                const size_t c2 = col_of(kp0 + 2 * (w + 4 * i) + (l >> 5), v2);
+                v3[i] = v2 ? lat.fc3_w[c2 * 32 + (l & 31)] : 0.f;
+            }
+            vb3 = valid ? lat.fc3_b[col] : 0.f;
+#pragma unroll
+            for (int i = 0; i < 16; ++i) {
+                const int o = w + 4 * i;
+                tile[o][l] = va[i];
+                lat.img[DvsLatImg::A(lat.NT) + (size_t)o * DvsLatImg::LD(lat.NT) + kp0 + l] = va[i];
+            }
+        }
+        __syncthreads();
+        if (on)
+            for (int j = w; j < 64; j += 4) lat.img[DvsLatImg::AT(lat.NT) + (size_t)(kp0 + j) * 64 + l] = tile[l][j];
+        __syncthreads();
+        if (on) {
+#pragma unroll
+            for (int i = 0; i < 8; ++i) {
+                const int jj = 2 * (w + 4 * i) + (l >> 5), o = l & 31;
+                tile[o][jj] = v3[i];
+                lat.img[DvsLatImg::W3(lat.NT) + (size_t)(kp0 + jj) * 32 + o] = v3[i];
+            }
+        }
+        __syncthreads();
+        if (!on) return;
+        for (int o = w; o < 32; o += 4) lat.img[DvsLatImg::W3T(lat.NT) + (size_t)o * DvsLatImg::LD(lat.NT) + kp0 + l] = tile[o][l];
+        if (w == 0) lat.img[DvsLatImg::B3(lat.NT) + kp0 + l] = vb3;
+        return;
+    }
+    if (!on) return;
+    const int jb = (blk - first_job) / 12, slice = (blk - first_job) % 12;
+    const DvsImgJob J = jobs.job[jb];
+    const bool transposed = J.flags & 1, rperm = J.flags & 2, cperm = J.flags & 4;
+    const float* src = params + J.src;
+    dvs_bf16* dst = wimg + J.dst;
+    for (int i = threadIdx.x; i < 16 * 64; i += IMG_THREADS) {
+        const int row = 16 * slice + (i >> 6), col = i & 63;
+        if (row >= J.rows) break;
+        const float v = src[(size_t)(rperm ? dvs_pi(row) : row) * ((J.flags & 8) ? 128 : 64) + (cperm ? dvs_pi(col) : col)];
+        if (!transposed) {
+            dvs_bf16 h, m, l;
+            dvs_split3_1(v, h, m, l);
+            const size_t o = (size_t)row * DVS_LDB + dvs_kperm(col), part = (size_t)J.rows * DVS_LDB;
+            dst[o] = h;
+            dst[part + o] = m;
+            if (!(J.flags & 16)) dst[2 * part + o] = l;
+        } else {
+            dvs_bf16 h, l;
+            dvs_split1(v, h, l);
+            const size_t o = (size_t)col * DVS_LDB + dvs_kperm(row);
+            dst[o] = h;
+            dst[DVS_IMG64 + o] = l;
+        }
+    }
+}
diff --git a/dags_vae_search_amd/csrc/dvs_wimg.h b/dags_vae_search_amd/csrc/dvs_wimg.h
--- a/dags_vae_search_amd/csrc/dvs_wimg.h
+++ b/dags_vae_search_amd/csrc/dvs_wimg.h
@@ -71,6 +71,9 @@
 };
 void dvs_launch_prepare_images(const DvsImgJobs& jobs, const float* params, dvs_bf16* wimg, const DvsLatImgArgs& lat,
                                const DvsLossHeadArgs& head, dvs_stream_t st);
+struct PackArgs;
+void dvs_launch_step_prologue(const PackArgs& pack, const DvsImgJobs& jobs, const float* params, dvs_bf16* wimg,
+                              const DvsLatImgArgs& lat, const DvsLossHeadArgs& head, dvs_stream_t st);
 
 __device__ __forceinline__ void dvs_copy_image(dvs_bf16* dst, const dvs_bf16* __restrict__ src, int n) {
     const f4* s = (const f4*)src;
diff --git a/dags_vae_search_amd/csrc/k_forward.hip b/dags_vae_search_amd/csrc/k_forward.hip
--- a/dags_vae_search_amd/csrc/k_forward.hip
+++ b/dags_vae_search_amd/csrc/k_forward.hip
@@ -1,111 +1,15 @@
 #include "dvs_kernels.h"
 #include "dvs_wimg.h"
-
-constexpr int PACK_DAGS = 4;
-__device__ __forceinline__ void pack_stream(float* dst, const float* __restrict__ src, size_t nfloats) {
-    const size_t n4 = nfloats >> 2;
-    size_t i = threadIdx.x;
-    for (; i + 3 * blockDim.x < n4; i += 4 * blockDim.x) {
-        f4 v[4];
-#pragma unroll
-        for (int u = 0; u < 4; ++u) v[u] = *(const f4*)(src + 4 * (i + u * blockDim.x));
-#pragma unroll
-        for (int u = 0; u < 4; ++u) *(f4*)(dst + 4 * (i + u * blockDim.x)) = v[u];
-    }
-    for (; i < n4; i += blockDim.x) *(f4*)(dst + 4 * i) = *(const f4*)(src + 4 * i);
-    for (size_t i = 4 * n4 + threadIdx.x; i < nfloats; i += blockDim.x) dst[i] = src[i];
-}
-__global__ __launch_bounds__(8 * 16 * PACK_DAGS) void k_pack(PackArgs a) {
+#include "dvs_prologue.h"
+
+__global__ __launch_bounds__(PACK_THREADS) void k_pack(PackArgs a) {
     DVS_DYN_LDS(smem);
-    const int N = a.N, C = a.C;
-    const int dag0 = blockIdx.x * PACK_DAGS;
-    const int nd = (a.B - dag0 < PACK_DAGS) ? a.B - dag0 : PACK_DAGS;
-    float* s_lab = (float*)smem;
-    float* s_pos = s_lab + PACK_DAGS * 16 * 16;
-    float* s_adj = s_pos + PACK_DAGS * 16 * 16;
-    float* s_msk = s_adj + PACK_DAGS * 16 * 16;
-    {
-        const float* src[4] = {a.lab1h + (size_t)dag0 * N * C, a.pos1h + (size_t)dag0 * N * N, a.adj + (size_t)dag0 * N * N,
-                               (const float*)(a.tmask + (size_t)dag0 * 8 * N * N)};
-        float* dst[4] = {s_lab, s_pos, s_adj, s_msk};
-        const int nf[4] = {nd * N * C, nd * N * N, nd * N * N, nd * 8 * N * N / 4};
-        bool whole = true;
-#pragma unroll
-        for (int k = 0; k < 4; ++k) whole = whole && (nf[k] & 3) == 0 && (nf[k] >> 2) <= 2 * (int)blockDim.x;
-        if (whole) {
-            f4 v[4][2];
-#pragma unroll
-            for (int k = 0; k < 4; ++k)
-#pragma unroll
-                for (int u = 0; u < 2; ++u) {
-                    const int i = (int)threadIdx.x + u * (int)blockDim.x;
-                    v[k][u] = *(const f4*)(src[k] + 4 * (i < (nf[k] >> 2) ? i : 0));
-                }
-#pragma unroll
-            for (int k = 0; k < 4; ++k)
-#pragma unroll
-                for (int u = 0; u < 2; ++u) {
-                    const int i = (int)threadIdx.x + u * (int)blockDim.x;
-                    if (i < (nf[k] >> 2)) *(f4*)(dst[k] + 4 * i) = v[k][u];
-                }
-        } else {
-#pragma unroll
-            for (int k = 0; k < 4; ++k) pack_stream(dst[k], src[k], (size_t)nf[k]);
-        }
-    }
-    __syncthreads();
-    const int h = threadIdx.x / (16 * PACK_DAGS), d = (threadIdx.x >> 4) % PACK_DAGS, i = threadIdx.x & 15;
-    if (d >= nd) return;
-    const uint8_t* msk = (const uint8_t*)s_msk;
-    int bad = 0;
-    if (h > 0) {
-        if (i < N) {
-            const uint8_t* m0 = msk + ((size_t)d * 8 * N + i) * N;
-            const uint8_t* mh = msk + (((size_t)d * 8 + h) * N + i) * N;
-            for (int j = 0; j < N; ++j)
-                if ((mh[j] != 0) != (m0[j] != 0)) bad |= 2;
-        }
-        if (bad) atomicOr(a.status, bad);
-        return;
-    }
-    int label = 0, pos = 0;
-    unsigned parents = 0, allowed = 1u << i;
-    if (i < N) {
-        const float* lr = s_lab + ((size_t)d * N + i) * C;
-        int ones = 0;
-        for (int c = 0; c < C; ++c) {
-            const float v = lr[c];
-            if (v == 1.0f) { label = c; ++ones; } else if (v != 0.0f) bad |= 1;
-        }
-        if (ones != 1) bad |= 1;
-        const float* pr = s_pos + ((size_t)d * N + i) * N;
-        ones = 0;
-        for (int c = 0; c < N; ++c) {
-            const float v = pr[c];
-            if (v == 1.0f) { pos = c; ++ones; } else if (v != 0.0f) bad |= 1;
-        }
-        if (ones != 1) bad |= 1;
-        const float* ad = s_adj + (size_t)d * N * N;
-        for (int j = 0; j < N; ++j)
-            if (ad[j * N + i] != 0.0f) parents |= 1u << j;
-        allowed = 0;
-        const uint8_t* m0 = msk + ((size_t)d * 8 * N + i) * N;
-        for (int j = 0; j < N; ++j)
-            if (!m0[j]) allowed |= 1u << j;
-        if (!((allowed >> i) & 1u)) bad |= 4;
-    }
-    DvsRecord* r = a.rec + dag0 + d;
-    r->label[i] = (uint8_t)label;
-    r->pos[i] = (uint8_t)pos;
-    r->parents[i] = (uint16_t)parents;
-    r->allowed[i] = (uint16_t)allowed;
-    if (bad) atomicOr(a.status, bad);
+    dvs_pack_body(a, smem, (int)blockIdx.x);
 }
 
 void dvs_launch_pack(const PackArgs& a, dvs_stream_t st) {
-    const size_t lds = (size_t)PACK_DAGS * (3 * 256 * 4 + 8 * 256);
-    DVS_SET_LDS(k_pack, lds);
-    DVS_LAUNCH(k_pack, dim3((a.B + PACK_DAGS - 1) / PACK_DAGS), dim3(8 * 16 * PACK_DAGS), lds, st, a);
+    DVS_SET_LDS(k_pack, PACK_LDS);
+    DVS_LAUNCH(k_pack, dim3((a.B + PACK_DAGS - 1) / PACK_DAGS), dim3(PACK_THREADS), PACK_LDS, st, a);
 }
 
 __global__ __launch_bounds__(256) void k_build_records(BuildArgs a) {
diff --git a/dags_vae_search_amd/csrc/k_optim.hip b/dags_vae_search_amd/csrc/k_optim.hip
--- a/dags_vae_search_amd/csrc/k_optim.hip
+++ b/dags_vae_search_amd/csrc/k_optim.hip
@@ -66,145 +66,28 @@
                        bc1, sqrtf(bc2), max_norm, scratch, guard, have_partials ? dvs_sq_parts(n) : SQ_PARTS);
 }
 
-#include "dvs_wimg.h"
-__device__ __forceinline__ float dvs_loss_head_value(const DvsLossHeadArgs& h, int i) {
-    if (i < 32 * 68) {
-        const int r = i / 68, c = i % 68;
-        return c < 64 ? h.node0_w[r * 64 + c] : 0.f;
-    }
-    i -= 32 * 68;
-    if (i < 16 * 36) {
-        const int c = i / 36, k = i % 36;
-        return (c < h.C && k < 32) ? h.node2_w[c * 32 + k] : 0.f;
-    }
-    i -= 16 * 36;
-    if (i < 32) return h.node0_b[i];
-    i -= 32;
-    if (i < 16) return i < h.C ? h.node2_b[i] : 0.f;
-    i -= 16;
-    if (i < 64) return h.edge0_b[i];
-    i -= 64;
-    if (i < 64) return h.edge2_w[i];
-    i -= 64;
-    if (i < 16) return i == 0 ? h.edge2_b[0] : 0.f;
-    i -= 16;
-    if (i < 64) return h.ln_g[i];
-    return h.ln_b[i - 64];
-}
-__device__ __forceinline__ float dvs_emb_block_value(const DvsLossHeadArgs& h, int i) {
-    if (i < 32 * 68) {
-        const int r = i / 68, c = i % 68;
-        return (r < 2 * h.N && c < 64) ? h.W1[r * 64 + c] : 0.f;
-    }
-    i -= 32 * 68;
-    if (i < 64 * 36) {
-        const int f = i / 36, k = i % 36;
-        return k < 32 ? h.W2[f * 32 + k] : 0.f;
-    }
-    i -= 64 * 36;
-    if (i < 512) {
-        const int f = i >> 4, c = i & 15;
-        return c < h.C ? h.lab_w[f * h.C + c] : 0.f;
-    }
-    i -= 512;
-    return i < 32 ? h.lab_b[i] : 0.f;
-}
-__global__ __launch_bounds__(256) void k_prepare_images(DvsImgJobs jobs, const float* params, dvs_bf16* wimg, DvsLatImgArgs lat,
-                                                        DvsLossHeadArgs head) {
-    const int nlat = 1024 * lat.NT / 64;
-    const int first_job = nlat + (head.dst ? 2 : 0);
-    if (head.dst) {
-        if ((int)blockIdx.x == nlat + 1) {
-            float v[DvsEmbImg::FLOATS / 256];
-#pragma unroll
-            for (int u = 0; u < DvsEmbImg::FLOATS / 256; ++u) v[u] = dvs_emb_block_value(head, u * 256 + (int)threadIdx.x);
-#pragma unroll
-            for (int u = 0; u < DvsEmbImg::FLOATS / 256; ++u) head.dst_emb[u * 256 + threadIdx.x] = v[u];
-            return;
-        }
-        if ((int)blockIdx.x == nlat) {
-            float v[DvsLossImg::HEAD_FLOATS / 256];
-#pragma unroll
-            for (int u = 0; u < DvsLossImg::HEAD_FLOATS / 256; ++u) v[u] = dvs_loss_head_value(head, u * 256 + (int)threadIdx.x);
-#pragma unroll
-            for (int u = 0; u < DvsLossImg::HEAD_FLOATS / 256; ++u) head.dst[u * 256 + threadIdx.x] = v[u];
-            return;
-        }
-    }
-    if ((int)blockIdx.x < nlat) {
-        __shared__ float tile[64][65];
-        const int K = 1024 * lat.NT, kp0 = (int)blockIdx.x * 64;
-        const int l = threadIdx.x & 63, w = threadIdx.x >> 6;
-        const size_t ldw = (size_t)lat.N * 64;
-        auto col_of = [&](int kp, bool& valid) {
-            const int tile_i = kp >> 10, q = (kp & 1023) >> 2, kk = kp & 3, t = q >> 6, ln = q & 63;
-            const int tok = 16 * tile_i + (ln & 15), feat = 16 * t + 4 * (ln >> 4) + kk;
-            valid = tok < lat.N;
-            return (size_t)(valid ? tok : 0) * 64 + feat;
-        };
-        bool valid;
-        const size_t col = col_of(kp0 + l, valid);
-        float va[16];
-#pragma unroll
-        for (int i = 0; i < 16; ++i) {
-            const int o = w + 4 * i;
-            va[i] = !valid ? 0.f : (o < 32 ? lat.fc1_w[o * ldw + col] : lat.fc2_w[(o - 32) * ldw + col]);
-        }
-        float v3[8];
-#pragma unroll
-        for (int i = 0; i < 8; ++i) {
-            bool v2;
-            const size_t c2 = col_of(kp0 + 2 * (w + 4 * i) + (l >> 5), v2);
-            v3[i] = v2 ? lat.fc3_w[c2 * 32 + (l & 31)] : 0.f;
-        }
-        const float vb3 = valid ? lat.fc3_b[col] : 0.f;
-#pragma unroll
-        for (int i = 0; i < 16; ++i) {
-            const int o = w + 4 * i;
-            tile[o][l] = va[i];
-            lat.img[DvsLatImg::A(lat.NT) + (size_t)o * DvsLatImg::LD(lat.NT) + kp0 + l] = va[i];
-        }
-        __syncthreads();
-        for (int j = w; j < 64; j += 4) lat.img[DvsLatImg::AT(lat.NT) + (size_t)(kp0 + j) * 64 + l] = tile[l][j];
-        __syncthreads();
-#pragma unroll
-        for (int i = 0; i < 8; ++i) {
-            const int jj = 2 * (w + 4 * i) + (l >> 5), o = l & 31;
-            tile[o][jj] = v3[i];
-            lat.img[DvsLatImg::W3(lat.NT) + (size_t)(kp0 + jj) * 32 + o] = v3[i];
-        }
-        __syncthreads();
-        for (int o = w; o < 32; o += 4) lat.img[DvsLatImg::W3T(lat.NT) + (size_t)o * DvsLatImg::LD(lat.NT) + kp0 + l] = tile[o][l];
-        if (w == 0) lat.img[DvsLatImg::B3(lat.NT) + kp0 + l] = vb3;
-        return;
-    }
-    const int jb = ((int)blockIdx.x - first_job) / 12, slice = ((int)blockIdx.x - first_job) % 12;
-    const DvsImgJob J = jobs.job[jb];
-    const bool transposed = J.flags & 1, rperm = J.flags & 2, cperm = J.flags & 4;
-    const float* src = params + J.src;
-    dvs_bf16* dst = wimg + J.dst;
-    for (int i = threadIdx.x; i < 16 * 64; i += blockDim.x) {
-        const int row = 16 * slice + (i >> 6), col = i & 63;
-        if (row >= J.rows) break;
-        const float v = src[(size_t)(rperm ? dvs_pi(row) : row) * ((J.flags & 8) ? 128 : 64) + (cperm ? dvs_pi(col) : col)];
-        if (!transposed) {
-            dvs_bf16 h, m, l;
-            dvs_split3_1(v, h, m, l);
-            const size_t o = (size_t)row * DVS_LDB + dvs_kperm(col), part = (size_t)J.rows * DVS_LDB;
-            dst[o] = h;
-            dst[part + o] = m;
-            if (!(J.flags & 16)) dst[2 * part + o] = l;
-        } else {
-            dvs_bf16 h, l;
-            dvs_split1(v, h, l);
-            const size_t o = (size_t)col * DVS_LDB + dvs_kperm(row);
-            dst[o] = h;
-            dst[DVS_IMG64 + o] = l;
-        }
-    }
+#include "dvs_prologue.h"
+__global__ __launch_bounds__(IMG_THREADS) void k_prepare_images(DvsImgJobs jobs, const float* params, dvs_bf16* wimg,
+                                                                DvsLatImgArgs lat, DvsLossHeadArgs head) {
+    __shared__ float tile[64][65];
+    dvs_prepare_images_body(jobs, params, wimg, lat, head, tile, (int)blockIdx.x);
 }
 void dvs_launch_prepare_images(const DvsImgJobs& jobs, const float* params, dvs_bf16* wimg, const DvsLatImgArgs& lat,
                                const DvsLossHeadArgs& head, dvs_stream_t st) {
-    DVS_LAUNCH(k_prepare_images, dim3(jobs.count * 12 + 1024 * lat.NT / 64 + (head.dst ? 2 : 0)), dim3(256), 0, st, jobs, params,
-               wimg, lat, head);
+    DVS_LAUNCH(k_prepare_images, dim3(dvs_image_blocks(jobs, lat, head)), dim3(IMG_THREADS), 0, st, jobs, params, wimg, lat, head);
 }
+
+static_assert(PACK_THREADS >= IMG_THREADS && PACK_LDS >= IMG_LDS, "k_step_prologue is sized by the pack part");
+__global__ __launch_bounds__(PACK_THREADS) void k_step_prologue(PackArgs pack, int n_img, DvsImgJobs jobs, const float* params,
+                                                                dvs_bf16* wimg, DvsLatImgArgs lat, DvsLossHeadArgs head) {
+    DVS_DYN_LDS(smem);
+    if ((int)blockIdx.x < n_img) dvs_prepare_images_body(jobs, params, wimg, lat, head, (float(*)[65])smem, (int)blockIdx.x);
+    else dvs_pack_body(pack, smem, (int)blockIdx.x - n_img);
+}
+void dvs_launch_step_prologue(const PackArgs& pack, const DvsImgJobs& jobs, const float* params, dvs_bf16* wimg,
+                              const DvsLatImgArgs& lat, const DvsLossHeadArgs& head, dvs_stream_t st) {
+    const int n_img = dvs_image_blocks(jobs, lat, head);
+    DVS_SET_LDS(k_step_prologue, PACK_LDS);
+    DVS_LAUNCH(k_step_prologue, dim3(n_img + (pack.B + PACK_DAGS - 1) / PACK_DAGS), dim3(PACK_THREADS), PACK_LDS, st, pack, n_img,
+               jobs, params, wimg, lat, head);
+}
diff --git a/dags_vae_search_amd/engine.py b/dags_vae_search_amd/engine.py
--- a/dags_vae_search_amd/engine.py
+++ b/dags_vae_search_amd/engine.py
@@ -72,7 +72,7 @@
             self._status.zero_()
         return st
 
-    def pack(self, features: Dict, check: bool = True, zero_status: bool = True) -> torch.Tensor:
+    def _dense_inputs(self, features: Dict):
         lab = features["vertex_label_features"]
         pos = features["vertex_position_features"]
         adj = features["adjacency_matrices"]
@@ -96,6 +96,10 @@
         adj = aligned(adj, torch.float32)
         tm = aligned(tm, tm.dtype)
         tm = tm.view(torch.uint8) if tm.dtype == torch.bool else aligned(tm, torch.uint8)
+        return lab, pos, adj, tm, B
+
+    def pack(self, features: Dict, check: bool = True, zero_status: bool = True) -> torch.Tensor:
+        lab, pos, adj, tm, B = self._dense_inputs(features)
         self.workspace(B, lab.device)
         if zero_status:
             self._status.zero_()
@@ -136,19 +140,30 @@
 
     def loss_forward(self, shape, params: torch.Tensor, eps: Optional[torch.Tensor], losses: torch.Tensor,
                      mu: Optional[torch.Tensor] = None, logvar: Optional[torch.Tensor] = None,
-                     host_tail: Optional[torch.Tensor] = None, host_seq: int = 0):
+                     host_tail: Optional[torch.Tensor] = None, host_seq: int = 0, features: Optional[Dict] = None):
         _require_cuda(params, "parameters")
         ws = self.workspace(shape.batch, params.device)
         if losses.numel() < dl.LOSS_FLOATS:
             raise ValueError(f"losses must hold {dl.LOSS_FLOATS} floats")
+        if host_tail is not None and (not host_tail.is_pinned() or host_tail.numel() < 4 or host_tail.dtype != torch.float32
+                                      or host_tail.data_ptr() % 16):
+            raise ValueError("host_tail must be at least 4 pinned float32 words, 16-byte aligned")
+        if features is not None:
+            lab, pos, adj, tm, B = self._dense_inputs(features)
+            if B != shape.batch:
+                raise AssertionError(f"Expected features of {shape.batch} graphs, got {B}")
+            dl.check(self.lib, self.lib.dvs_pack_loss_forward(
+                ctypes.byref(shape), _ptr(lab), _ptr(pos), _ptr(adj), _ptr(tm), _ptr(self._records), _nbytes(self._records),
+                _ptr(params), params.numel(), _ptr(ws), _nbytes(ws), _ptr(eps), _ptr(self._status), _ptr(losses), _ptr(mu),
+                _ptr(logvar), None if host_tail is None else host_tail.data_ptr(), int(host_seq) & 0xFFFFFF, _stream()),
+                "dvs_pack_loss_forward")
+            return
         if host_tail is None:
             dl.check(self.lib, self.lib.dvs_loss_forward(ctypes.byref(shape), _ptr(self._records), _nbytes(self._records),
                                                          _ptr(params), params.numel(), _ptr(ws), _nbytes(ws), _ptr(eps),
                                                          _ptr(self._status), _ptr(losses), _ptr(mu), _ptr(logvar), _stream()),
                      "dvs_loss_forward")
             return
-        if not host_tail.is_pinned() or host_tail.numel() < 4 or host_tail.dtype != torch.float32 or host_tail.data_ptr() % 16:
-            raise ValueError("host_tail must be at least 4 pinned float32 words, 16-byte aligned")
         dl.check(self.lib, self.lib.dvs_loss_forward_notify(
             ctypes.byref(shape), _ptr(self._records), _nbytes(self._records), _ptr(params), params.numel(), _ptr(ws), _nbytes(ws),
             _ptr(eps), _ptr(self._status), _ptr(losses), _ptr(mu), _ptr(logvar), host_tail.data_ptr(), int(host_seq) & 0xFFFFFF,
diff --git a/dags_vae_search_amd/pace.py b/dags_vae_search_amd/pace.py
--- a/dags_vae_search_amd/pace.py
+++ b/dags_vae_search_amd/pace.py
@@ -409,7 +409,13 @@
             pending, self._early_pending = self._early_pending, False
             if pending != "poll":
                 self._ev_tail.synchronize()
-        if not packed:
+        dense = None
+        if not packed and defer_check and not isinstance(features, CompactBatch):
+            dev = self.flat_params.device
+            dense = {k: features[k].to(dev) for k in ("vertex_label_features", "vertex_position_features",
+                                                      "adjacency_matrices", "target_masks")}
+            eng.workspace(dense["vertex_label_features"].shape[0], dev)
+        elif not packed:
             self._pack(features, check=False if defer_check else None, zero_status=not defer_check)
         B = eng._ws_batch
         shape = self._shape(B, beta)
@@ -421,10 +427,11 @@
             self._host_seq = (getattr(self, "_host_seq", 0) + 1) & 0xFFFFFF or 1
             losses = self._notify_losses = torch.empty(8, dtype=torch.float32, device=grads.device)[:dl.LOSS_FLOATS]
             self._step_guard = losses[3:5]
-            eng.loss_forward(shape, self.flat_params, eps, losses, host_tail=self._host_tail, host_seq=self._host_seq)
+            eng.loss_forward(shape, self.flat_params, eps, losses, host_tail=self._host_tail, host_seq=self._host_seq,
+                             features=dense)
             self._early_pending = "poll"
         else:
-            eng.loss_forward(shape, self.flat_params, eps, losses)
+            eng.loss_forward(shape, self.flat_params, eps, losses, features=dense)
         self._fwd_generation += 1
         if early_read and not notify:
             self._early_read(exchange)
diff --git a/include/dvs.h b/include/dvs.h
--- a/include/dvs.h
+++ b/include/dvs.h
@@ -60,6 +60,11 @@
 int dvs_loss_forward_notify(const dvs_shape* s, const void* records, size_t records_bytes, const float* params,
                             int64_t n_params, void* workspace, size_t workspace_bytes, const float* eps, int32_t* status,
                             float* losses, float* mu, float* logvar, void* host_tail, uint32_t host_seq, void* stream);
+
+int dvs_pack_loss_forward(const dvs_shape* s, const float* label_onehot, const float* pos_onehot, const float* adjacency,
+                          const uint8_t* target_masks, void* records, size_t records_bytes, const float* params,
+                          int64_t n_params, void* workspace, size_t workspace_bytes, const float* eps, int32_t* status,
+                          float* losses, float* mu, float* logvar, void* host_tail, uint32_t host_seq, void* stream);
 
 int dvs_loss_backward(const dvs_shape* s, const void* records, size_t records_bytes, const float* params, int64_t n_params,
                       void* workspace, size_t workspace_bytes, const float* gcoef, float* grads, void* stream);
```

Measured after the change: 3.387 million DAGs/s (median of 6 runs). No clear change (+0.1%).
